# Jackie-Chou/MC-CNN-python

Measured on AMD Instinct MI355X. Metric: Mdisparities/s (HxWxD / s) end-to-end match.py timed region, images resident in HBM, higher is better.
Workload: dtype f32; 1 GPU; cfg2: 750x500 synthetic stereo pair, D=256, one pair per GPU; weights=converted reference checkpoint

## Files before the change

### include/mccnn.h

```cpp
#ifndef MCCNN_H
#define MCCNN_H

#include <stddef.h>
#include <stdint.h>

#ifdef __cplusplus
extern "C" {
#endif

typedef void *mccnn_stream_t;

#define MCCNN_ABI_VERSION 7

#define MCCNN_E_INVALID (-1)
#define MCCNN_E_UNSUPPORTED (-2)
#define MCCNN_E_SCRATCH (-3)

#define MCCNN_SIDE_LEFT 0
#define MCCNN_SIDE_RIGHT 1

int mccnn_version(void);
const char *mccnn_last_error_string(void);

#define MCCNN_CV_EXACT 0
#define MCCNN_CV_MFMA 1
int mccnn_cost_volume(const float *fl, const float *fr, int H, int W, int C, int D, float *lcv, float *rcv, int mode,
                      mccnn_stream_t stream);

int mccnn_cost_volume_hwd(const float *fl, const float *fr, int H, int W, int C, int D, float *lcv_hwd, float *rcv_hwd,
                          int mode, mccnn_stream_t stream);

size_t mccnn_decision_pack_bytes(int n_fc, int units, int mode);
int mccnn_decision_pack(const float *weights, int n_fc, int units, float weight_scale, int mode, void *packed,
                        mccnn_stream_t stream);
int mccnn_cost_volume_accurate(const float *aL, const float *aR, int H, int W, int C, int units, int n_fc, int D,
                               const void *packed, const float *biases, const float *w_final, float b_final,
                               float weight_scale, float *lcv, float *rcv, int mode, int *saturation_flag,
                               mccnn_stream_t stream);
int mccnn_cost_volume_accurate_hwd(const float *aL, const float *aR, int H, int W, int C, int units, int n_fc, int D,
                                   const void *packed, const float *biases, const float *w_final, float b_final,
                                   float weight_scale, float *lcv_hwd, float *rcv_hwd, int mode, int *saturation_flag,
                                   mccnn_stream_t stream);

int mccnn_cost_volume_fill(float *lcv, float *rcv, int D, int H, int W, int pixel_major, mccnn_stream_t stream);

typedef uint32_t mccnn_support_t;
size_t mccnn_support_bytes(int H, int W);
#define MCCNN_SUPPORT_UP(s) ((s) & 31u)
#define MCCNN_SUPPORT_DOWN(s) (((s) >> 5) & 31u)
#define MCCNN_SUPPORT_LEFT(s) (((s) >> 10) & 31u)
#define MCCNN_SUPPORT_RIGHT(s) (((s) >> 15) & 31u)
#define MCCNN_SUPPORT_COUNT(s) ((s) >> 20)
int mccnn_cross_arms(const float *image, int H, int W, float tau, int L, mccnn_support_t *support,
                     mccnn_stream_t stream);
int mccnn_cross_arms_pair(const float *image_left, const float *image_right, int H, int W, float tau, int L,
                          mccnn_support_t *support_left, mccnn_support_t *support_right, mccnn_stream_t stream);
int mccnn_cross_region_list(const mccnn_support_t *support, int H, int W, int L, int32_t *region,
                            mccnn_stream_t stream);

#define MCCNN_CBCA_SEPARABLE 0
#define MCCNN_CBCA_REFERENCE_ORDER 1
int mccnn_cbca_iter(const float *in, float *out, const mccnn_support_t *support, int D, int H, int W, int L, int order,
                    mccnn_stream_t stream);

int mccnn_cbca_iter_pair(const float *in_left, float *out_left, const mccnn_support_t *support_left,
                         const float *in_right, float *out_right, const mccnn_support_t *support_right, int D, int H,
                         int W, int L, int order, mccnn_stream_t stream);

int mccnn_cbca_iter_both(const float *in, float *out, const mccnn_support_t *support_self,
                         const mccnn_support_t *support_other, int D, int H, int W, int L, int side,
                         mccnn_stream_t stream);

int mccnn_cbca_iter_hwd(const float *in_hwd, float *out_hwd, const mccnn_support_t *support, int D, int H, int W, int L,
                        mccnn_stream_t stream);
int mccnn_cbca_iter_hwd_pair(const float *in_left, float *out_left, const mccnn_support_t *support_left,
                             const float *in_right, float *out_right, const mccnn_support_t *support_right, int D,
                             int H, int W, int L, mccnn_stream_t stream);

int mccnn_cbca_iter_hwd_pair_wta(const float *in_left, float *out_left, const mccnn_support_t *support_left,
                                 const float *in_right, float *out_right, const mccnn_support_t *support_right, int D,
                                 int H, int W, int L, float *disparity_left, float *disparity_right, int store_right,
                                 mccnn_stream_t stream);

int mccnn_cbca_iter_hwd_long(const float *in_hwd, float *out_hwd, const mccnn_support_t *support, int D, int H, int W,
                             int L, mccnn_stream_t stream);
int mccnn_cbca_iter_hwd_long_pair(const float *in_left, float *out_left, const mccnn_support_t *support_left,
                                  const float *in_right, float *out_right, const mccnn_support_t *support_right, int D,
                                  int H, int W, int L, mccnn_stream_t stream);

size_t mccnn_cbca_prog_bytes(int D, int H, int W);
int mccnn_cbca_prog_build_pair(const mccnn_support_t *support_left, const mccnn_support_t *support_right, int D, int H,
                               int W, int L, void *prog_left, void *prog_right, mccnn_stream_t stream);
int mccnn_cbca_iter_prog_pair(const float *in_left, float *out_left, const mccnn_support_t *support_left,
                              const void *prog_left, const float *in_right, float *out_right,
                              const mccnn_support_t *support_right, const void *prog_right, int D, int H, int W, int L,
                              mccnn_stream_t stream);
int mccnn_cbca_iter_prog_pair_wta(const float *in_left, float *out_left, const mccnn_support_t *support_left,
                                  const void *prog_left, const float *in_right, float *out_right,
                                  const mccnn_support_t *support_right, const void *prog_right, int D, int H, int W, int L,
                                  float *disparity_left, float *disparity_right, int store_right, mccnn_stream_t stream);

int mccnn_cbca_prog_build_skip_pair(const mccnn_support_t *support_left, const mccnn_support_t *support_right, int D,
                                    int H, int W, int L, void *prog_left, void *prog_right, mccnn_stream_t stream);
int mccnn_cbca_prog_build_both_pair(const mccnn_support_t *support_left, const mccnn_support_t *support_right, int D,
                                    int H, int W, int L, void *prog_left, void *prog_right, mccnn_stream_t stream);
int mccnn_cbca_iter_prog_pair_skip(const float *in_left, float *out_left, const mccnn_support_t *support_left,
                                   const void *prog_left, const float *in_right, float *out_right,
                                   const mccnn_support_t *support_right, const void *prog_right, int D, int H, int W,
                                   int L, mccnn_stream_t stream);

int mccnn_cbca_iter_prog(const float *in, float *out, const mccnn_support_t *support, const void *prog, int D, int H, int W,
                         int L, mccnn_stream_t stream);
int mccnn_cbca_iter_prog_skip(const float *in, float *out, const mccnn_support_t *support, const void *prog, int D, int H,
                              int W, int L, mccnn_stream_t stream);

int mccnn_cbca_iter_prog_refresh(float *in, float *out, const mccnn_support_t *support, const void *prog, int D, int H, int W,
                                 int L, mccnn_stream_t stream);
int mccnn_cbca_iter_prog_pair_refresh(float *in_left, float *out_left, const mccnn_support_t *support_left,
                                      const void *prog_left, float *in_right, float *out_right,
                                      const mccnn_support_t *support_right, const void *prog_right, int D, int H, int W,
                                      int L, mccnn_stream_t stream);

int mccnn_hwd_pitch(int D);
int mccnn_dhw_to_hwd(const float *dhw, float *hwd, int D, int H, int W, mccnn_stream_t stream);
int mccnn_hwd_to_dhw(const float *hwd, float *dhw, int D, int H, int W, mccnn_stream_t stream);

size_t mccnn_sgm_scratch_bytes(int H, int W, int D);
int mccnn_sgm_pass(const float *image_left, const float *image_right, float *const *vol_hwd, const int *side,
                   int n_jobs, int D, int H, int W, int rh, int rw, float p1, float p2, float q1, float q2, float thr,
                   void *scratch, size_t scratch_bytes, mccnn_stream_t stream);
int mccnn_sgm_flags(const float *image_left, const float *image_right, int D, int H, int W, int rh, int rw, float thr,
                    void *flags, size_t flags_bytes, mccnn_stream_t stream);
int mccnn_sgm_pass_flagged(float *const *vol_hwd, const int *side, int n_jobs, int D, int H, int W, int rh, int rw, float p1,
                           float p2, float q1, float q2, const void *flags, size_t flags_bytes, mccnn_stream_t stream);

#define MCCNN_SGM_ACC_STORE 0
#define MCCNN_SGM_ACC_ADD 1
#define MCCNN_SGM_ACC_ADD_QUARTER 2
int mccnn_sgm_pass_accumulate(const float *const *src_hwd, float *const *acc_hwd, const int *side, int n_jobs, int D, int H,
                              int W, int rh, int rw, float p1, float p2, float q1, float q2, int mode, const void *flags,
                              size_t flags_bytes, mccnn_stream_t stream);

int mccnn_sgm_first_pass(const float *image_left, const float *image_right, const float *const *vol_dhw,
                         float *const *vol_hwd, const int *side, int n_jobs, int D, int H, int W, float p1, float p2,
                         float q1, float q2, float thr, void *scratch, size_t scratch_bytes, mccnn_stream_t stream);

int mccnn_wta(const float *vol_dhw, int D, int H, int W, float *disparity, mccnn_stream_t stream);

int mccnn_wta_hwd(const float *vol_hwd, int D, int H, int W, float *disparity, mccnn_stream_t stream);

int mccnn_lr_status(const float *disp_left, const float *disp_right, int H, int W, int D, int32_t *status,
                    mccnn_stream_t stream);
int mccnn_interpolate(const float *disp_left, const int32_t *status, int H, int W, float *out,
                      mccnn_stream_t stream);
int mccnn_interpolate_ex(const float *disp_left, const int32_t *status, int H, int W, int directions,
                         int occlusion_from_left, float *out, mccnn_stream_t stream);

int mccnn_lr_status_right(const float *disp_right, const float *disp_left, int H, int W, int D, int32_t *status,
                          mccnn_stream_t stream);
int mccnn_interpolate_right(const float *disp_right, const int32_t *status, int H, int W, int directions,
                            int occlusion_from_right, float *out, mccnn_stream_t stream);

int mccnn_subpixel(const float *disp, const float *vol_dhw, int D, int H, int W, float *out, mccnn_stream_t stream);
int mccnn_subpixel_ex(const float *disp, const float *vol_dhw, int D, int H, int W, int numpy1_promotion, float *out,
                      mccnn_stream_t stream);

int mccnn_subpixel_hwd(const float *disp, const float *vol_hwd, int D, int H, int W, int numpy1_promotion, float *out,
                       mccnn_stream_t stream);

#define MCCNN_CONF_MSM 1u
#define MCCNN_CONF_MMN 2u
#define MCCNN_CONF_CUR 4u
#define MCCNN_CONF_LRC 8u
int mccnn_confidence_hwd(const float *vol_hwd , const float *disp_right , int D,
                         int H, int W, unsigned measures, float *out, mccnn_stream_t stream);
int mccnn_confidence(const float *vol_dhw , const float *disp_right , int D, int H,
                     int W, unsigned measures, float *out, mccnn_stream_t stream);

int mccnn_confidence_right_hwd(const float *vol_right_hwd , const float *disp_left ,
                               int D, int H, int W, unsigned measures, float *out, mccnn_stream_t stream);
int mccnn_confidence_right(const float *vol_right_dhw , const float *disp_left , int D,
                           int H, int W, unsigned measures, float *out, mccnn_stream_t stream);

int mccnn_median(const float *disp, int H, int W, int fh, int fw, float *out, mccnn_stream_t stream);

int mccnn_bilateral(const float *image, const float *disp, int H, int W, int fh, int fw, const float *table,
                    float thr, float *out, mccnn_stream_t stream);

size_t mccnn_ingest_scratch_bytes(int H, int W);
int mccnn_ingest_u8(const uint8_t *image_u8, int H, int W, int C, float *out, void *scratch, size_t scratch_bytes,
                    mccnn_stream_t stream);
int mccnn_ingest_u8_pair(const uint8_t *left_u8, const uint8_t *right_u8, int H, int W, int C, float *out_left,
                         float *out_right, void *scratch, size_t scratch_bytes, mccnn_stream_t stream);

typedef struct { int64_t offset; int32_t H, W; } mccnn_sample_image_t;
typedef struct { int32_t image; float cy, cx; float m[4]; float gain, bias; } mccnn_sample_t;
int mccnn_sample_patches(const float *pool, const mccnn_sample_image_t *images, int n_images,
                         const mccnn_sample_t *records, int N, int ps, float *out ,
                         mccnn_stream_t stream);

#define MCCNN_EVAL_MAX_THRESHOLDS 8
typedef struct { uint64_t n_valid, n_invalid, n_bad[MCCNN_EVAL_MAX_THRESHOLDS]; double sum_abs, sum_sq; } mccnn_eval_region_t;
typedef struct { mccnn_eval_region_t all, nonocc; } mccnn_eval_t;
size_t mccnn_evaluate_scratch_bytes(int H, int W);
int mccnn_evaluate(const float *disp, const float *gt, const uint8_t *mask , int H, int W,
                   const float *thresholds , int n_thr, int accumulate,
                   mccnn_eval_t *result , void *scratch, size_t scratch_bytes, mccnn_stream_t stream);

#define MCCNN_EVAL_MAX_QUANTILES 8
typedef struct { uint64_t n_scored; uint64_t rank[MCCNN_EVAL_MAX_QUANTILES]; float value[MCCNN_EVAL_MAX_QUANTILES]; } mccnn_quantile_region_t;
typedef struct { mccnn_quantile_region_t all, nonocc; } mccnn_eval_quantiles_t;
#define MCCNN_EVAL_POOL_BYTES (2 * 65536 * 8)
size_t mccnn_evaluate_quantiles_scratch_bytes(int H, int W);
int mccnn_evaluate_quantiles(const float *disp, const float *gt, const uint8_t *mask , int H, int W,
                             const uint32_t *q_ppm , int n_q,
                             mccnn_eval_quantiles_t *result , uint64_t *pool ,
                             void *scratch, size_t scratch_bytes, mccnn_stream_t stream);
int mccnn_evaluate_quantiles_pooled(const uint64_t *pool, const uint32_t *q_ppm , int n_q,
                                    mccnn_eval_quantiles_t *result , mccnn_stream_t stream);

int mccnn_kitti_encode_u16(const float *disp, int H, int W, uint16_t *out_u16, mccnn_stream_t stream);
int mccnn_kitti_decode_u16(const uint16_t *code_u16, int H, int W, float *out, mccnn_stream_t stream);
int mccnn_kitti_interpolate_background(const float *disp, int H, int W, float *out, mccnn_stream_t stream);
size_t mccnn_evaluate_kitti_scratch_bytes(int H, int W, int interpolate);
int mccnn_evaluate_kitti(const float *disp, const uint16_t *gt_occ_u16, const uint16_t *gt_noc_u16 ,
                         int H, int W, const float *abs_thr , const float *rel_thr , int n_thr,
                         int interpolate, int accumulate, mccnn_eval_t *result , void *scratch,
                         size_t scratch_bytes, mccnn_stream_t stream);

int mccnn_bias_act(float *x, const float *bias, int N, int C, long plane, int relu, mccnn_stream_t stream);
int mccnn_conv1_pad_bias_relu(const float *images, const float *weights, const float *bias, float *out, int N, int H,
                              int W, int pad, int C, mccnn_stream_t stream);
int mccnn_l2norm_chw_to_hwc(const float *chw, const float *bias, float *hwc, int C, int H, int W,
                            mccnn_stream_t stream);

size_t mccnn_conv3x3_split_weights_bytes(void);
int mccnn_conv3x3_split_pack(const float *weights, float weight_scale, void *packed, mccnn_stream_t stream);
int mccnn_conv1_split(const float *images, const float *weights, const float *bias, void *out, int N, int H, int W,
                      int pad, float act_scale, int *saturation_flag, mccnn_stream_t stream);
int mccnn_conv3x3_split(const void *in, const void *packed_weights, const float *bias, void *out, int N, int Hi, int Wi,
                        float weight_scale, float act_scale, int last, int *saturation_flag, mccnn_stream_t stream);

#ifdef __cplusplus
}
#endif
#endif
```

### mc-cnn-python_amd/csrc/conv_mfma.hip

```cpp
#include "common.h"

namespace mccnn {

typedef _Float16 h8 __attribute__((ext_vector_type(8)));
typedef _Float16 h4 __attribute__((ext_vector_type(4)));
typedef float f16x __attribute__((ext_vector_type(16)));
typedef uint32_t w4 __attribute__((ext_vector_type(4)));
typedef uint32_t w2 __attribute__((ext_vector_type(2)));

#ifndef CONV_STAGE_TAP
#define CONV_STAGE_TAP 0
#endif
#ifndef CONV_NBW
#define CONV_NBW 4
#endif
namespace cs {
constexpr int NBW = CONV_NBW;
constexpr int TH = 4 * NBW, TW = 32;
constexpr int IH = TH + 2, IW = TW + 2;
constexpr int NPIX = IH * IW;
constexpr int SLOT = 80;
constexpr int QBUF = NPIX * SLOT;
constexpr int NITEM = NPIX * 4;
constexpr int NST = (NITEM + 255) / 256;
constexpr int EPITCH = 272;
constexpr int EPX = NBW >= 4 ? 32 : 16;
constexpr int EPI = EPX * EPITCH;
constexpr int LDS_BYTES = 2 * QBUF + 4 * EPI;
constexpr int REC = 256;
constexpr int WFRAG = 1024;
constexpr int WLAYER = 36 * 4 * WFRAG;
}

__device__ __forceinline__ void split4(const float y[4], float scale, w2 &hi, w2 &lo)
{
    h4 a, b;
#pragma unroll
    for (int j = 0; j < 4; ++j) {
        const float v = fminf(fmaxf(y[j] * scale, -65504.f), 65504.f);
        const _Float16 h = (_Float16)v;
        a[j] = h;
        b[j] = (_Float16)(v - (float)h);
    }
    hi = __builtin_bit_cast(w2, a);
    lo = __builtin_bit_cast(w2, b);
}

__device__ __forceinline__ void split4_scaled(const float v[4], w2 &hi, w2 &lo)
{
    h4 a, b;
#pragma unroll
    for (int j = 0; j < 4; ++j) {
        const _Float16 h = (_Float16)v[j];
        a[j] = h;
        b[j] = (_Float16)(v[j] - (float)h);
    }
    hi = __builtin_bit_cast(w2, a);
    lo = __builtin_bit_cast(w2, b);
}

__global__ __launch_bounds__(256) void conv3x3_split_pack_kernel(const float *__restrict__ w, float scale,
                                                                 _Float16 *__restrict__ packed)
{
    const int i = blockIdx.x * 256 + threadIdx.x;
    if (i >= 36 * 2 * 64) return;
    const int lane = i & 63, mb = (i >> 6) & 1, ks = i >> 7;
    const int q = ks / 9, tap = ks - q * 9;
    const int oc = 32 * mb + (lane & 31), ic0 = 16 * q + 8 * (lane >> 5);
    h8 hi, lo;
#pragma unroll
    for (int j = 0; j < 8; ++j) {
        const float v = w[((size_t)oc * 64 + ic0 + j) * 9 + tap] * scale;
        const _Float16 h = (_Float16)v;
        hi[j] = h;
        lo[j] = (_Float16)(v - (float)h);
    }
    h8 *p = reinterpret_cast<h8 *>(packed);
    p[((ks * 2 + 0) * 2 + mb) * 64 + lane] = hi;
    p[((ks * 2 + 1) * 2 + mb) * 64 + lane] = lo;
}

__global__ __launch_bounds__(256) void conv1_split_kernel(const float *__restrict__ img, const float *__restrict__ w,
                                                          const float *__restrict__ bias, char *__restrict__ out, int H,
                                                          int W, int pad, int Ho, int Wo, float act_scale,
                                                          int *__restrict__ sat_flag)
{
    const int xo = blockIdx.x * 256 + threadIdx.x;
    const int yo = blockIdx.y, n = blockIdx.z;
    if (xo >= Wo) return;
    float v[9];
#pragma unroll
    for (int i = 0; i < 3; ++i)
#pragma unroll
        for (int j = 0; j < 3; ++j) {
            const int y = yo + i - pad, x = xo + j - pad;
            v[i * 3 + j] = (y >= 0 && y < H && x >= 0 && x < W) ? img[((size_t)n * H + y) * W + x] : 0.f;
        }
    char *rec = out + (((size_t)n * Ho + yo) * Wo + xo) * cs::REC;
    bool sat = false;
#pragma unroll
    for (int q = 0; q < 4; ++q) {
        w2 hi[4], lo[4];
#pragma unroll
        for (int g = 0; g < 4; ++g) {
            float y[4];
#pragma unroll
            for (int j = 0; j < 4; ++j) {
                const int c = 16 * q + 4 * g + j;
                float acc = 0.f;
#pragma unroll
                for (int k = 0; k < 9; ++k) acc += w[c * 9 + k] * v[k];
                acc += bias[c];
                y[j] = fmaxf(acc, 0.f);
                sat |= !(acc * act_scale <= 65504.f);
            }
            split4(y, act_scale, hi[g], lo[g]);
        }
        w4 *p = reinterpret_cast<w4 *>(rec + q * 64);
        p[0] = w4{hi[0].x, hi[0].y, hi[1].x, hi[1].y};
        p[1] = w4{hi[2].x, hi[2].y, hi[3].x, hi[3].y};
        p[2] = w4{lo[0].x, lo[0].y, lo[1].x, lo[1].y};
        p[3] = w4{lo[2].x, lo[2].y, lo[3].x, lo[3].y};
    }
    if (sat_flag && sat) atomicOr(sat_flag, 1);
}

__device__ __forceinline__ void pin_loads()
{
    asm volatile("" ::: "memory");
    __builtin_amdgcn_sched_barrier(0x78f);
}

template <int MODE>
__global__ __launch_bounds__(256) void conv3x3_split_kernel(const char *__restrict__ in, const char *__restrict__ wpk,
                                                            const float *__restrict__ bias, char *__restrict__ out,
                                                            int N, int Hi, int Wi, float inv_scale, float act_scale,
                                                            int tiles_x, int tiles_y, int total,
                                                            int *__restrict__ sat_flag)
{
    using namespace cs;
    extern __shared__ __attribute__((aligned(16))) char lds[];
    const int tid = threadIdx.x, lane = tid & 63;
    const int wave = __builtin_amdgcn_readfirstlane(tid >> 6);
    const int Ho = Hi - 2, Wo = Wi - 2;
    const size_t in_bytes = (size_t)N * Hi * Wi * REC, out_bytes = (size_t)N * Ho * Wo * REC;
    const __amdgpu_buffer_rsrc_t rs_in = __builtin_amdgcn_make_buffer_rsrc(
        const_cast<char *>(in), 0, (int)in_bytes, 0x00020000);
    const __amdgpu_buffer_rsrc_t rs_w =
        __builtin_amdgcn_make_buffer_rsrc(const_cast<char *>(wpk), 0, WLAYER, 0x00020000);
    const __amdgpu_buffer_rsrc_t rs_out = __builtin_amdgcn_make_buffer_rsrc(
        out, 0, (int)out_bytes, 0x00020000);

    int goff[NST], loff[NST];
#pragma unroll
    for (int r = 0; r < NST; ++r) {
        const int i = r * 256 + tid, p = min(i >> 2, NPIX - 1), part = i & 3;
        const int py = p / IW, px = p - py * IW;
        goff[r] = (py * Wi + px) * REC + part * 16;
        loff[r] = p * SLOT + part * 16;
    }
    const bool last_piece = (NST - 1) * 256 + tid < NITEM;

    auto xcd_order = [](int b, int n) {
        const int q = n >> 3, r = n & 7, x = b & 7;
        return (x < r ? x * (q + 1) : r * (q + 1) + (x - r) * q) + (b >> 3);
    };
    auto tile_base = [&](int v, int &n, int &ty0, int &tx0) {
        const int t = xcd_order(v, total);
        const int tx = t % tiles_x, r = t / tiles_x;
        const int ty = r % tiles_y;
        n = r / tiles_y;
        ty0 = ty * TH;
        tx0 = tx * TW;
    };

    w4 st[NST];
    auto fetch = [&](int n, int ty0, int tx0, int q) {
        const int so = ((n * Hi + ty0) * Wi + tx0) * REC + q * 64;
#ifdef CONV_ABL_NOSTAGE
        if (so == 0x7fffffff)
#endif
#pragma unroll
        for (int r = 0; r < NST; ++r) st[r] = __builtin_amdgcn_raw_buffer_load_b128(rs_in, goff[r], so, 0);
    };
    auto commit = [&](int buf) {
        char *b = lds + buf * QBUF;
#pragma unroll
        for (int r = 0; r < NST; ++r)
            if (r < NST - 1 || last_piece) *reinterpret_cast<w4 *>(b + loff[r]) = st[r];
    };

    int v = blockIdx.x;
    if (v >= total) return;
    int n, ty0, tx0;
    tile_base(v, n, ty0, tx0);
    fetch(n, ty0, tx0, 0);
    commit(0);
    __syncthreads();

    constexpr int NSLOT = MODE == 0 ? 3 : 4;
    w4 af[NSLOT][4];
    auto fetch_a = [&](int slot, int ks) {
#pragma unroll
        for (int f = 0; f < 4; ++f)
            af[slot][f] = __builtin_amdgcn_raw_buffer_load_b128(rs_w, lane * 16, (ks * 4 + f) * WFRAG, 0);
    };
#pragma unroll
    for (int i = 0; i < NSLOT - 1; ++i) fetch_a(i, i);

    const int bfrag = (wave * NBW * IW + (lane & 31)) * SLOT + 16 * (lane >> 5);
    char *const epi = lds + 2 * QBUF + wave * EPI;

    while (true) {
        f16x acc[NBW][2], accx[NBW][2];
#pragma unroll
        for (int nb = 0; nb < NBW; ++nb)
#pragma unroll
            for (int mb = 0; mb < 2; ++mb)
#pragma unroll
                for (int i = 0; i < 16; ++i) acc[nb][mb][i] = accx[nb][mb][i] = 0.f;
        const int vn = v + gridDim.x;
        int nn = 0, nty0 = 0, ntx0 = 0;
        if (vn < total) tile_base(vn, nn, nty0, ntx0);
        if (vn >= total) {
            nn = n;
            nty0 = ty0;
            ntx0 = tx0;
        }
#pragma unroll
        for (int q = 0; q < 4; ++q) {
            auto stage_next = [&]() {
                if (q < 3)
                    fetch(n, ty0, tx0, q + 1);
                else
                    fetch(nn, nty0, ntx0, 0);
                pin_loads();
            };
            if (CONV_STAGE_TAP < 0) stage_next();
            const char *bq = lds + (q & 1) * QBUF + bfrag;
            char *const other = lds + ((q + 1) & 1) * QBUF;
            w4 bf[2][2];
            auto read_b = [&](int slot, int step) {
                const int tap = step / NBW, nb = step % NBW;
                const int dy = tap / 3, dx = tap - dy * 3;
                const char *pb = bq + ((nb + dy) * IW + dx) * SLOT;
                bf[slot][0] = *reinterpret_cast<const w4 *>(pb);
                bf[slot][1] = *reinterpret_cast<const w4 *>(pb + 32);
            };
            read_b(0, 0);
#pragma unroll
            for (int tap = 0; tap < 9; ++tap) {
                const int ks = q * 9 + tap;
                fetch_a((ks + NSLOT - 1) % NSLOT, (ks + NSLOT - 1) % 36);
                pin_loads();
                if (tap == CONV_STAGE_TAP) stage_next();
                const int slot = ks % NSLOT;
                const h8 a_hi0 = __builtin_bit_cast(h8, af[slot][0]), a_hi1 = __builtin_bit_cast(h8, af[slot][1]);
                const h8 a_lo0 = __builtin_bit_cast(h8, af[slot][2]), a_lo1 = __builtin_bit_cast(h8, af[slot][3]);
#pragma unroll
                for (int nb = 0; nb < NBW; ++nb) {
                    const int step = tap * NBW + nb;
                    if (step + 1 < 9 * NBW) read_b((step + 1) & 1, step + 1);
                    __builtin_amdgcn_sched_barrier(0);
                    const h8 b_hi = __builtin_bit_cast(h8, bf[step & 1][0]);
                    const h8 b_lo = __builtin_bit_cast(h8, bf[step & 1][1]);
                    accx[nb][0] = __builtin_amdgcn_mfma_f32_32x32x16_f16(a_lo0, b_hi, accx[nb][0], 0, 0, 0);
                    accx[nb][1] = __builtin_amdgcn_mfma_f32_32x32x16_f16(a_lo1, b_hi, accx[nb][1], 0, 0, 0);
                    accx[nb][0] = __builtin_amdgcn_mfma_f32_32x32x16_f16(a_hi0, b_lo, accx[nb][0], 0, 0, 0);
                    accx[nb][1] = __builtin_amdgcn_mfma_f32_32x32x16_f16(a_hi1, b_lo, accx[nb][1], 0, 0, 0);
                    acc[nb][0] = __builtin_amdgcn_mfma_f32_32x32x16_f16(a_hi0, b_hi, acc[nb][0], 0, 0, 0);
                    acc[nb][1] = __builtin_amdgcn_mfma_f32_32x32x16_f16(a_hi1, b_hi, acc[nb][1], 0, 0, 0);
                }
                if (tap >= 9 - (NST + 1) / 2) {
#pragma unroll
                    for (int j = 0; j < 2; ++j) {
                        const int r = 2 * (tap - (9 - (NST + 1) / 2)) + j;
                        if (r < NST && (r < NST - 1 || last_piece)) *reinterpret_cast<w4 *>(other + loff[r]) = st[r];
                    }
                }
            }
            __syncthreads();
        }

        const int px = lane & 31, half = lane >> 5;
        bool sat = false;
#ifdef CONV_ABL_NOEPI
        {
            float t = 0.f;
#pragma unroll
            for (int nb = 0; nb < NBW; ++nb)
#pragma unroll
                for (int mb = 0; mb < 2; ++mb)
#pragma unroll
                    for (int r = 0; r < 16; ++r) t += acc[nb][mb][r] + accx[nb][mb][r];
            if (t == 123.456f) __builtin_amdgcn_raw_buffer_store_b32(__float_as_uint(t), rs_out, lane * 4, 0, 0);
        }
#else
#pragma unroll
        for (int nb = 0; nb < NBW; ++nb) {
            float y[2][16];
            float ss = 0.f;
#pragma unroll
            for (int mb = 0; mb < 2; ++mb)
#pragma unroll
                for (int r = 0; r < 16; ++r) {
                    const int ch = 32 * mb + (r & 3) + 8 * (r >> 2) + 4 * half;
                    if (MODE == 0) {
                    } else {
                        const float t = fmaf(acc[nb][mb][r] + accx[nb][mb][r], inv_scale, bias[ch]);
                        y[mb][r] = t;
                        ss = fmaf(t, t, ss);
                    }
                }
            float nrm = 1.f;
            if (MODE == 1) {
                ss += __shfl_xor(ss, 32);
                nrm = 1.f / sqrtf(fmaxf(ss, 1e-12f));
            }
            const int row = ty0 + wave * NBW + nb;
            const int so = ((n * Ho + min(row, Ho - 1)) * Wo + tx0) * REC;
            const bool stored = row < Ho && tx0 + px < Wo;
            bool over = false;
#pragma unroll
            for (int hf = 0; hf < 32 / EPX; ++hf) {
                __builtin_amdgcn_wave_barrier();
                if (EPX == 32 || (px >> 4) == hf) {
                    const int pl = px & (EPX - 1);
#pragma unroll
                    for (int mb = 0; mb < 2; ++mb)
#pragma unroll
                        for (int g = 0; g < 4; ++g) {
                            const int ch = 32 * mb + 8 * g + 4 * half;
                            if (MODE == 0) {
                                w2 hi, lo;
                                float y4[4];
#pragma unroll
                                for (int q = 0; q < 4; ++q) {
                                    const int r = 4 * g + q;
                                    const float t = fmaf(acc[nb][mb][r] + accx[nb][mb][r], inv_scale * act_scale,
                                                         bias[ch + q] * act_scale);
                                    over |= !(t <= 65504.f);
                                    y4[q] = __builtin_amdgcn_fmed3f(t, 0.f, 65504.f);
                                }
                                split4_scaled(y4, hi, lo);
                                char *p = epi + pl * EPITCH + (ch >> 4) * 64 + (ch & 15) * 2;
                                *reinterpret_cast<w2 *>(p) = hi;
                                *reinterpret_cast<w2 *>(p + 32) = lo;
                            } else {
                                w4 o;
                                o.x = __float_as_uint(y[mb][4 * g + 0] * nrm);
                                o.y = __float_as_uint(y[mb][4 * g + 1] * nrm);
                                o.z = __float_as_uint(y[mb][4 * g + 2] * nrm);
                                o.w = __float_as_uint(y[mb][4 * g + 3] * nrm);
                                *reinterpret_cast<w4 *>(epi + pl * EPITCH + ch * 4) = o;
                            }
                        }
                }
                __builtin_amdgcn_wave_barrier();
#pragma unroll
                for (int it = 0; it < EPX / 4; ++it) {
                    const int i = it * 64 + lane, pl = i >> 4, part = i & 15, p = hf * EPX + pl;
                    const w4 o = *reinterpret_cast<const w4 *>(epi + pl * EPITCH + part * 16);
                    const bool ok = row < Ho && tx0 + p < Wo;
                    buffer_store_b128<0>(o, rs_out, ok ? p * REC + part * 16 : 0x7ffffff0, so);
                }
            }
            __builtin_amdgcn_wave_barrier();
            sat |= over && stored;
        }
        if (MODE == 0 && sat_flag && __builtin_amdgcn_ballot_w64(sat) != 0 && lane == 0)
            atomicOr(sat_flag, 1);
#endif
        if (vn >= total) break;
        v = vn;
        n = nn;
        ty0 = nty0;
        tx0 = ntx0;
    }
}

}

extern "C" size_t mccnn_conv3x3_split_weights_bytes(void) { return (size_t)mccnn::cs::WLAYER; }

extern "C" int mccnn_conv3x3_split_pack(const float *weights, float weight_scale, void *packed, mccnn_stream_t stream)
{
    using namespace mccnn;
    MCCNN_REQUIRE(weights && packed, MCCNN_E_INVALID, "mccnn_conv3x3_split_pack: null pointer");
    MCCNN_REQUIRE(weight_scale > 0.f, MCCNN_E_INVALID, "mccnn_conv3x3_split_pack: scale must be positive");
    hipLaunchKernelGGL(conv3x3_split_pack_kernel, dim3(cdiv(36 * 2 * 64, 256)), dim3(256), 0, (hipStream_t)stream,
                       weights, weight_scale, reinterpret_cast<_Float16 *>(packed));
    return check_launch("mccnn_conv3x3_split_pack");
}

extern "C" int mccnn_conv1_split(const float *images, const float *weights, const float *bias, void *out, int N, int H,
                                 int W, int pad, float act_scale, int *saturation_flag, mccnn_stream_t stream)
{
    using namespace mccnn;
    MCCNN_REQUIRE(images && weights && bias && out, MCCNN_E_INVALID, "mccnn_conv1_split: null pointer");
    MCCNN_REQUIRE(N > 0 && H > 0 && W > 0 && pad >= 0, MCCNN_E_INVALID, "mccnn_conv1_split: bad size");
    MCCNN_REQUIRE(act_scale > 0.f, MCCNN_E_INVALID, "mccnn_conv1_split: scale must be positive");
    const int Ho = H + 2 * pad - 2, Wo = W + 2 * pad - 2;
    MCCNN_REQUIRE(Ho > 0 && Wo > 0 && Ho <= 65535 && N <= 65535, MCCNN_E_UNSUPPORTED,
                  "mccnn_conv1_split: output %dx%d outside the grid", Wo, Ho);
    hipLaunchKernelGGL(conv1_split_kernel, dim3(cdiv(Wo, 256), Ho, N), dim3(256), 0, (hipStream_t)stream, images,
                       weights, bias, reinterpret_cast<char *>(out), H, W, pad, Ho, Wo, act_scale, saturation_flag);
    return check_launch("mccnn_conv1_split");
}

extern "C" int mccnn_conv3x3_split(const void *in, const void *packed_weights, const float *bias, void *out, int N,
                                   int Hi, int Wi, float weight_scale, float act_scale, int last,
                                   int *saturation_flag, mccnn_stream_t stream)
{
    using namespace mccnn;
    using namespace cs;
    MCCNN_REQUIRE(in && packed_weights && bias && out, MCCNN_E_INVALID, "mccnn_conv3x3_split: null pointer");
    MCCNN_REQUIRE(N > 0 && Hi > 2 && Wi > 2, MCCNN_E_INVALID, "mccnn_conv3x3_split: input %dx%d too small", Wi, Hi);
    MCCNN_REQUIRE(weight_scale > 0.f && act_scale > 0.f, MCCNN_E_INVALID, "mccnn_conv3x3_split: scales must be positive");
    MCCNN_REQUIRE((size_t)N * Hi * Wi * REC <= 0x7ffffff0u, MCCNN_E_UNSUPPORTED,
                  "mccnn_conv3x3_split: %d x %dx%d records exceed 32-bit buffer offsets", N, Wi, Hi);
    const int Ho = Hi - 2, Wo = Wi - 2;
    const int tiles_x = cdiv(Wo, TW), tiles_y = cdiv(Ho, TH);
    const long total = (long)tiles_x * tiles_y * N;
    MCCNN_REQUIRE(total <= 0x7fffffffL, MCCNN_E_UNSUPPORTED, "mccnn_conv3x3_split: too many tiles");
    const int cus = device_cus8();
    const long slots = (long)cus * (LDS_BYTES <= 80 * 1024 ? 2 : 1);
    const int grid = (int)(total < slots ? total : slots);
    const float inv = 1.f / (weight_scale * act_scale);
    hipStream_t s = (hipStream_t)stream;
    if (last) {
        static const hipError_t attr = hipFuncSetAttribute(reinterpret_cast<const void *>(conv3x3_split_kernel<1>),
                                                           hipFuncAttributeMaxDynamicSharedMemorySize, LDS_BYTES);
        MCCNN_REQUIRE(attr == hipSuccess, MCCNN_E_UNSUPPORTED, "mccnn_conv3x3_split: %d bytes of LDS refused", LDS_BYTES);
        hipLaunchKernelGGL(conv3x3_split_kernel<1>, dim3(grid), dim3(256), LDS_BYTES, s,
                           reinterpret_cast<const char *>(in), reinterpret_cast<const char *>(packed_weights), bias,
                           reinterpret_cast<char *>(out), N, Hi, Wi, inv, act_scale, tiles_x, tiles_y, (int)total,
                           saturation_flag);
    } else {
        static const hipError_t attr = hipFuncSetAttribute(reinterpret_cast<const void *>(conv3x3_split_kernel<0>),
                                                           hipFuncAttributeMaxDynamicSharedMemorySize, LDS_BYTES);
        MCCNN_REQUIRE(attr == hipSuccess, MCCNN_E_UNSUPPORTED, "mccnn_conv3x3_split: %d bytes of LDS refused", LDS_BYTES);
        hipLaunchKernelGGL(conv3x3_split_kernel<0>, dim3(grid), dim3(256), LDS_BYTES, s,
                           reinterpret_cast<const char *>(in), reinterpret_cast<const char *>(packed_weights), bias,
                           reinterpret_cast<char *>(out), N, Hi, Wi, inv, act_scale, tiles_x, tiles_y, (int)total,
                           saturation_flag);
    }
    return check_launch("mccnn_conv3x3_split");
}
```

### mc-cnn-python_amd/src/_hipabi.py

```python
import ctypes
import os

import torch

_HERE = os.path.dirname(os.path.abspath(__file__))
LIB_PATH = os.environ.get("MCCNN_HIP_LIB") or os.path.join(os.path.dirname(_HERE), "lib", "libmccnn_hip.so")

MCCNN_ABI_VERSION = 7
MCCNN_CV_EXACT = 0
MCCNN_CV_MFMA = 1
MCCNN_CBCA_SEPARABLE = 0
MCCNN_CBCA_REFERENCE_ORDER = 1
MCCNN_SIDE_LEFT = 0
MCCNN_SIDE_RIGHT = 1
MCCNN_SGM_ACC_STORE = 0
MCCNN_SGM_ACC_ADD = 1
MCCNN_SGM_ACC_ADD_QUARTER = 2
MCCNN_E_INVALID = -1
MCCNN_E_UNSUPPORTED = -2
MCCNN_E_SCRATCH = -3

MCCNN_EVAL_MAX_THRESHOLDS = 8
MCCNN_EVAL_MAX_QUANTILES = 8
MCCNN_EVAL_POOL_BYTES = 2 * 65536 * 8
MCCNN_CONF_MSM = 1
MCCNN_CONF_MMN = 2
MCCNN_CONF_CUR = 4
MCCNN_CONF_LRC = 8

_vp = ctypes.c_void_p
_i = ctypes.c_int
_f = ctypes.c_float
_sz = ctypes.c_size_t

SIGNATURES = {
    "mccnn_version": (_i, []),
    "mccnn_last_error_string": (ctypes.c_char_p, []),
    "mccnn_cost_volume": (_i, [_vp, _vp, _i, _i, _i, _i, _vp, _vp, _i, _vp]),
    "mccnn_cost_volume_hwd": (_i, [_vp, _vp, _i, _i, _i, _i, _vp, _vp, _i, _vp]),
    "mccnn_cost_volume_fill": (_i, [_vp, _vp, _i, _i, _i, _i, _vp]),
    "mccnn_decision_pack_bytes": (_sz, [_i, _i, _i]),
    "mccnn_decision_pack": (_i, [_vp, _i, _i, _f, _i, _vp, _vp]),
    "mccnn_cost_volume_accurate": (_i, [_vp, _vp, _i, _i, _i, _i, _i, _i, _vp, _vp, _vp, _f, _f, _vp, _vp, _i, _vp, _vp]),
    "mccnn_cost_volume_accurate_hwd": (_i, [_vp, _vp, _i, _i, _i, _i, _i, _i, _vp, _vp, _vp, _f, _f, _vp, _vp, _i, _vp,
                                            _vp]),
    "mccnn_support_bytes": (_sz, [_i, _i]),
    "mccnn_cross_arms": (_i, [_vp, _i, _i, _f, _i, _vp, _vp]),
    "mccnn_cross_arms_pair": (_i, [_vp, _vp, _i, _i, _f, _i, _vp, _vp, _vp]),
    "mccnn_cross_region_list": (_i, [_vp, _i, _i, _i, _vp, _vp]),
    "mccnn_cbca_iter": (_i, [_vp, _vp, _vp, _i, _i, _i, _i, _i, _vp]),
    "mccnn_cbca_iter_pair": (_i, [_vp, _vp, _vp, _vp, _vp, _vp, _i, _i, _i, _i, _i, _vp]),
    "mccnn_cbca_iter_both": (_i, [_vp, _vp, _vp, _vp, _i, _i, _i, _i, _i, _vp]),
    "mccnn_cbca_iter_hwd": (_i, [_vp, _vp, _vp, _i, _i, _i, _i, _vp]),
    "mccnn_cbca_iter_hwd_pair": (_i, [_vp, _vp, _vp, _vp, _vp, _vp, _i, _i, _i, _i, _vp]),
    "mccnn_cbca_iter_hwd_pair_wta": (_i, [_vp, _vp, _vp, _vp, _vp, _vp, _i, _i, _i, _i, _vp, _vp, _i, _vp]),
    "mccnn_cbca_iter_hwd_long": (_i, [_vp, _vp, _vp, _i, _i, _i, _i, _vp]),
    "mccnn_cbca_iter_hwd_long_pair": (_i, [_vp, _vp, _vp, _vp, _vp, _vp, _i, _i, _i, _i, _vp]),
    "mccnn_cbca_prog_bytes": (_sz, [_i, _i, _i]),
    "mccnn_cbca_prog_build_pair": (_i, [_vp, _vp, _i, _i, _i, _i, _vp, _vp, _vp]),
    "mccnn_cbca_iter_prog_pair": (_i, [_vp, _vp, _vp, _vp, _vp, _vp, _vp, _vp, _i, _i, _i, _i, _vp]),
    "mccnn_cbca_prog_build_skip_pair": (_i, [_vp, _vp, _i, _i, _i, _i, _vp, _vp, _vp]),
    "mccnn_cbca_prog_build_both_pair": (_i, [_vp, _vp, _i, _i, _i, _i, _vp, _vp, _vp]),
    "mccnn_cbca_iter_prog_pair_skip": (_i, [_vp, _vp, _vp, _vp, _vp, _vp, _vp, _vp, _i, _i, _i, _i, _vp]),
    "mccnn_cbca_iter_prog": (_i, [_vp, _vp, _vp, _vp, _i, _i, _i, _i, _vp]),
    "mccnn_cbca_iter_prog_skip": (_i, [_vp, _vp, _vp, _vp, _i, _i, _i, _i, _vp]),
    "mccnn_cbca_iter_prog_refresh": (_i, [_vp, _vp, _vp, _vp, _i, _i, _i, _i, _vp]),
    "mccnn_cbca_iter_prog_pair_refresh": (_i, [_vp, _vp, _vp, _vp, _vp, _vp, _vp, _vp, _i, _i, _i, _i, _vp]),
    "mccnn_cbca_iter_prog_pair_wta": (_i, [_vp, _vp, _vp, _vp, _vp, _vp, _vp, _vp, _i, _i, _i, _i, _vp, _vp, _i, _vp]),
    "mccnn_wta_hwd": (_i, [_vp, _i, _i, _i, _vp, _vp]),
    "mccnn_subpixel_hwd": (_i, [_vp, _vp, _i, _i, _i, _i, _vp, _vp]),
    "mccnn_confidence_hwd": (_i, [_vp, _vp, _i, _i, _i, ctypes.c_uint, _vp, _vp]),
    "mccnn_confidence": (_i, [_vp, _vp, _i, _i, _i, ctypes.c_uint, _vp, _vp]),
    "mccnn_confidence_right_hwd": (_i, [_vp, _vp, _i, _i, _i, ctypes.c_uint, _vp, _vp]),
    "mccnn_confidence_right": (_i, [_vp, _vp, _i, _i, _i, ctypes.c_uint, _vp, _vp]),
    "mccnn_hwd_pitch": (_i, [_i]),
    "mccnn_dhw_to_hwd": (_i, [_vp, _vp, _i, _i, _i, _vp]),
    "mccnn_hwd_to_dhw": (_i, [_vp, _vp, _i, _i, _i, _vp]),
    "mccnn_sgm_scratch_bytes": (_sz, [_i, _i, _i]),
    "mccnn_sgm_pass": (_i, [_vp, _vp, ctypes.POINTER(_vp), ctypes.POINTER(_i), _i, _i, _i, _i, _i, _i,
                            _f, _f, _f, _f, _f, _vp, _sz, _vp]),
    "mccnn_sgm_flags": (_i, [_vp, _vp, _i, _i, _i, _i, _i, _f, _vp, _sz, _vp]),
    "mccnn_sgm_pass_flagged": (_i, [ctypes.POINTER(_vp), ctypes.POINTER(_i), _i, _i, _i, _i, _i, _i, _f, _f, _f, _f, _vp, _sz,
                                    _vp]),
    "mccnn_sgm_pass_accumulate": (_i, [ctypes.POINTER(_vp), ctypes.POINTER(_vp), ctypes.POINTER(_i), _i, _i, _i, _i, _i, _i,
                                       _f, _f, _f, _f, _i, _vp, _sz, _vp]),
    "mccnn_sgm_first_pass": (_i, [_vp, _vp, ctypes.POINTER(_vp), ctypes.POINTER(_vp), ctypes.POINTER(_i), _i, _i, _i,
                                  _i, _f, _f, _f, _f, _f, _vp, _sz, _vp]),
    "mccnn_wta": (_i, [_vp, _i, _i, _i, _vp, _vp]),
    "mccnn_lr_status": (_i, [_vp, _vp, _i, _i, _i, _vp, _vp]),
    "mccnn_interpolate": (_i, [_vp, _vp, _i, _i, _vp, _vp]),
    "mccnn_interpolate_ex": (_i, [_vp, _vp, _i, _i, _i, _i, _vp, _vp]),
    "mccnn_lr_status_right": (_i, [_vp, _vp, _i, _i, _i, _vp, _vp]),
    "mccnn_interpolate_right": (_i, [_vp, _vp, _i, _i, _i, _i, _vp, _vp]),
    "mccnn_subpixel": (_i, [_vp, _vp, _i, _i, _i, _vp, _vp]),
    "mccnn_subpixel_ex": (_i, [_vp, _vp, _i, _i, _i, _i, _vp, _vp]),
    "mccnn_median": (_i, [_vp, _i, _i, _i, _i, _vp, _vp]),
    "mccnn_bilateral": (_i, [_vp, _vp, _i, _i, _i, _i, _vp, _f, _vp, _vp]),
    "mccnn_bias_act": (_i, [_vp, _vp, _i, _i, ctypes.c_long, _i, _vp]),
    "mccnn_conv1_pad_bias_relu": (_i, [_vp, _vp, _vp, _vp, _i, _i, _i, _i, _i, _vp]),
    "mccnn_conv3x3_split_weights_bytes": (_sz, []),
    "mccnn_conv3x3_split_pack": (_i, [_vp, _f, _vp, _vp]),
    "mccnn_conv1_split": (_i, [_vp, _vp, _vp, _vp, _i, _i, _i, _i, _f, _vp, _vp]),
    "mccnn_conv3x3_split": (_i, [_vp, _vp, _vp, _vp, _i, _i, _i, _f, _f, _i, _vp, _vp]),
    "mccnn_l2norm_chw_to_hwc": (_i, [_vp, _vp, _vp, _i, _i, _i, _vp]),
    "mccnn_ingest_scratch_bytes": (_sz, [_i, _i]),
    "mccnn_ingest_u8": (_i, [_vp, _i, _i, _i, _vp, _vp, _sz, _vp]),
    "mccnn_ingest_u8_pair": (_i, [_vp, _vp, _i, _i, _i, _vp, _vp, _vp, _sz, _vp]),
    "mccnn_sample_patches": (_i, [_vp, _vp, _i, _vp, _i, _i, _vp, _vp]),
    "mccnn_evaluate_scratch_bytes": (_sz, [_i, _i]),
    "mccnn_evaluate": (_i, [_vp, _vp, _vp, _i, _i, ctypes.POINTER(_f), _i, _i, _vp, _vp, _sz, _vp]),
    "mccnn_evaluate_quantiles_scratch_bytes": (_sz, [_i, _i]),
    "mccnn_evaluate_quantiles": (_i, [_vp, _vp, _vp, _i, _i, ctypes.POINTER(ctypes.c_uint32), _i, _vp, _vp, _vp, _sz, _vp]),
    "mccnn_evaluate_quantiles_pooled": (_i, [_vp, ctypes.POINTER(ctypes.c_uint32), _i, _vp, _vp]),
    "mccnn_kitti_encode_u16": (_i, [_vp, _i, _i, _vp, _vp]),
    "mccnn_kitti_decode_u16": (_i, [_vp, _i, _i, _vp, _vp]),
    "mccnn_kitti_interpolate_background": (_i, [_vp, _i, _i, _vp, _vp]),
    "mccnn_evaluate_kitti_scratch_bytes": (_sz, [_i, _i, _i]),
    "mccnn_evaluate_kitti": (_i, [_vp, _vp, _vp, _i, _i, ctypes.POINTER(_f), ctypes.POINTER(_f), _i, _i, _i, _vp, _vp, _sz,
                                  _vp]),
}



class EvalRegion(ctypes.Structure):
    _fields_ = [("n_valid", ctypes.c_uint64), ("n_invalid", ctypes.c_uint64),
                ("n_bad", ctypes.c_uint64 * MCCNN_EVAL_MAX_THRESHOLDS), ("sum_abs", ctypes.c_double),
                ("sum_sq", ctypes.c_double)]


class EvalResult(ctypes.Structure):
    _fields_ = [("all", EvalRegion), ("nonocc", EvalRegion)]


class QuantileRegion(ctypes.Structure):
    _fields_ = [("n_scored", ctypes.c_uint64), ("rank", ctypes.c_uint64 * MCCNN_EVAL_MAX_QUANTILES),
                ("value", ctypes.c_uint32 * MCCNN_EVAL_MAX_QUANTILES)]


class QuantileResult(ctypes.Structure):
    _fields_ = [("all", QuantileRegion), ("nonocc", QuantileRegion)]


_lib = None


class MccnnHipError(RuntimeError):
    pass


def load():
    global _lib
    if _lib is not None:
        return _lib
    if not os.path.isfile(LIB_PATH):
        raise MccnnHipError(
            "libmccnn_hip.so not found at %s - build it with `make -C mc-cnn-python_amd` "
            "(or `python -c 'import __graft_entry__ as g; g.build()'`). There is no CPU fallback." % LIB_PATH)
    lib = ctypes.CDLL(LIB_PATH)
    for name, (res, args) in SIGNATURES.items():
        fn = getattr(lib, name)
        fn.restype = res
        fn.argtypes = args
    have = lib.mccnn_version()
    if have != MCCNN_ABI_VERSION:
        raise MccnnHipError("%s implements ABI version %d, this binding expects %d: rebuild the library "
                            "(`make -C mc-cnn-python_amd`)" % (LIB_PATH, have, MCCNN_ABI_VERSION))
    _lib = lib
    return lib


def check(rc, what):
    if rc != 0:
        msg = load().mccnn_last_error_string()
        raise MccnnHipError("%s failed (code %d): %s" % (what, rc, msg.decode() if msg else "?"))


def stream():
    return ctypes.c_void_p(torch.cuda.current_stream().cuda_stream)


def ptr(t):
    if not t.is_cuda:
        raise MccnnHipError("expected a device tensor; the HIP path never runs on host memory")
    if not t.is_contiguous():
        raise MccnnHipError("expected a contiguous tensor")
    return ctypes.c_void_p(t.data_ptr())


def require_device():
    if not torch.cuda.is_available():
        raise MccnnHipError("no HIP device visible: the MI355X path cannot run (and there is no CPU fallback)")
    load()
    return torch.device("cuda", torch.cuda.current_device())
```

### mc-cnn-python_amd/src/model.py

```python
import math
import os

os.environ.setdefault("MIOPEN_DEBUG_CONV_DIRECT_NAIVE_CONV_FWD", "0")

import numpy as np
import torch
import torch.nn.functional as F

import tf_checkpoint


SPLIT_RECORD_LIMIT = 0x7ffffff0 // 256


def split_feature_route(H, W, pad):
    padded = (H + 2 * pad - 2) * (W + 2 * pad - 2)
    if padded > SPLIT_RECORD_LIMIT:
        return "library", max(64, (SPLIT_RECORD_LIMIT // (W + 2 * pad)) // 2)
    return ("pair" if 2 * padded <= SPLIT_RECORD_LIMIT else "views"), None


class NET(object):

    def __init__(self, x=None, weights_path='DEFAULT',
                 input_patch_size=11, num_conv_layers=5, num_conv_feature_maps=64,
                 conv_kernel_size=3, batch_size=128, device=None, seed=0):
        self.X = x
        self.batch_size = batch_size
        self.input_patch_size = input_patch_size
        self.num_conv_layers = num_conv_layers
        self.num_conv_feature_maps = num_conv_feature_maps
        self.conv_kernel_size = conv_kernel_size
        self.WEIGHTS_PATH = 'pretrain.npy' if weights_path == 'DEFAULT' else weights_path
        if device is None:
            if torch.is_tensor(x):
                device = x.device
            else:
                device = torch.device("cuda") if torch.cuda.is_available() else torch.device("cpu")
        self.device = torch.device(device)
        self._init_variables(seed)
        if x is not None:
            self.create()

    def _init_variables(self, seed):
        g = torch.Generator().manual_seed(seed)
        k, nf = self.conv_kernel_size, self.num_conv_feature_maps
        self.weights = []
        self.biases = []
        cin = 1
        for _ in range(self.num_conv_layers):
            limit = math.sqrt(6.0 / (k * k * cin + k * k * nf))
            w = (torch.rand((nf, cin, k, k), generator=g) * 2 - 1) * limit
            blim = math.sqrt(6.0 / (nf + nf))
            b = (torch.rand((nf,), generator=g) * 2 - 1) * blim
            self.weights.append(w.to(self.device))
            self.biases.append(b.to(self.device))
            cin = nf

    def set_layers(self, layers):
        assert len(layers) == self.num_conv_layers, "checkpoint has %d conv layers, NET was built with %d" % (
            len(layers), self.num_conv_layers)
        self.weights = [torch.from_numpy(np.ascontiguousarray(np.transpose(w, (3, 2, 0, 1)))).to(self.device)
                        for w, _ in layers]
        self.biases = [torch.from_numpy(np.ascontiguousarray(b)).to(self.device) for _, b in layers]
        return self

    def get_layers(self):
        return [(np.ascontiguousarray(w.detach().permute(2, 3, 1, 0).cpu().numpy()), b.detach().cpu().numpy())
                for w, b in zip(self.weights, self.biases)]

    def restore(self, checkpoint):
        return self.set_layers(tf_checkpoint.load_fast_net_weights(checkpoint))

    def load_initial_weights(self, session=None):
        weights_dict = np.load(self.WEIGHTS_PATH, encoding='bytes', allow_pickle=True).item()
        layers = self.get_layers()
        for name, value in weights_dict.items():
            name = name.decode() if isinstance(name, bytes) else name
            scope, var = name.split(":")[0].split("/")
            idx = int(scope.replace("conv", "")) - 1
            w, b = layers[idx]
            layers[idx] = (np.asarray(value, np.float32), b) if var == "weights" else (w, np.asarray(value, np.float32))
        self.set_layers(layers)

    def save_weights(self, session=None, file_name='pretrain.npy'):
        weights_dict = {}
        for k, (w, b) in enumerate(self.get_layers(), start=1):
            weights_dict["conv%d/weights:0" % k] = w
            weights_dict["conv%d/biases:0" % k] = b
        np.save(file_name, weights_dict)

    def _convs_nchw(self, x):
        outs = []
        nl = self.num_conv_layers
        for k in range(nl):
            x = F.conv2d(x, self.weights[k], self.biases[k])
            if k < nl - 1:
                x = F.relu(x)
            outs.append(x)
        return outs

    def _convs_device(self, images, pad):
        import stereo_device
        nl = self.num_conv_layers
        if self.conv_kernel_size == 3 and nl >= 2:
            x = stereo_device.conv1_pad_bias_relu(images.contiguous(), self.weights[0], self.biases[0], pad)
            first = 1
        else:
            x = F.pad(images[:, None], (pad, pad, pad, pad))
            first = 0
        for k in range(first, nl):
            x = F.conv2d(x, self.weights[k], None)
            if k < nl - 1:
                x = stereo_device.bias_act_(x.contiguous(), self.biases[k], True)
        return x.contiguous()

    @staticmethod
    def _l2_normalize_last(x):
        s = torch.clamp((x * x).sum(dim=-1, keepdim=True), min=1e-12)
        return x * torch.rsqrt(s)

    def create(self):
        self(self.X)

    def __call__(self, x):
        x = torch.as_tensor(x, dtype=torch.float32).to(self.device)
        assert x.dim() == 4 and x.shape[-1] == 1, "NET expects NHWC input with one channel (model.py:36-40)"
        self.X = x
        outs = self._convs_nchw(x.permute(0, 3, 1, 2).contiguous())
        for k, o in enumerate(outs, start=1):
            setattr(self, "conv%d" % k, o.permute(0, 2, 3, 1))
        self.features = self._l2_normalize_last(outs[-1].permute(0, 2, 3, 1))
        return self.features

    def features_hwc(self, image_hw):
        import stereo_device
        pad = (self.input_patch_size - 1) // 2
        assert pad == self.num_conv_layers * (self.conv_kernel_size - 1) // 2, \
            "patch size must equal the receptive field so that features keep the image size"
        out = self._convs_device(image_hw[None], pad)[0]
        return stereo_device.l2norm_chw_to_hwc(out, self.biases[-1])

    def supports_split_features(self):
        return self.conv_kernel_size == 3 and self.num_conv_feature_maps == 64 and self.num_conv_layers >= 2

    def _split_weights(self):
        import stereo_device
        key = tuple((w.data_ptr(), w._version) for w in self.weights[1:])
        cache = getattr(self, "_split_cache", None)
        if cache is None or cache[0] != key:
            cache = (key, [stereo_device.conv3x3_split_pack(w) for w in self.weights[1:]])
            self._split_cache = cache
        return cache[1]

    def _split_flag(self):
        f = getattr(self, "_split_sat", None)
        if f is None or f.device != self.weights[0].device:
            f = torch.zeros((1,), dtype=torch.int32, device=self.weights[0].device)
            self._split_sat = f
        return f

    def split_saturated(self, reset=True):
        f = getattr(self, "_split_sat", None)
        if f is None:
            return False
        hit = bool(int(f.item()))
        if hit and reset:
            f.zero_()
        return hit

    def features_pair_hwc_split(self, left_hw, right_hw):
        import warnings
        import stereo_device
        pad = (self.input_patch_size - 1) // 2
        assert pad == self.num_conv_layers * (self.conv_kernel_size - 1) // 2
        if not self.supports_split_features():
            raise ValueError("the split-operand feature kernels are built for >= 2 layers of 64 maps, 3x3")
        packed = self._split_weights()
        flag = self._split_flag()
        H, W = left_hw.shape
        route, rows = split_feature_route(H, W, pad)
        if route == "library":
            warnings.warn("split-operand features: a %dx%d view exceeds the kernels' 32-bit record offsets; using the "
                          "float32 library convolutions in bands of %d rows instead" % (W, H, rows))
            return self.features_pair_hwc(left_hw, right_hw, tile_rows=rows)
        batches = [torch.stack((left_hw, right_hw)).contiguous()] if route == "pair" else \
            [left_hw[None].contiguous(), right_hw[None].contiguous()]
        outs = []
        nl = self.num_conv_layers
        for views in batches:
            x = stereo_device.conv1_split(views, self.weights[0].detach().contiguous(), self.biases[0].detach(), pad,
                                          sat_flag=flag)
            for k in range(1, nl):
                pk, ws = packed[k - 1]
                x = stereo_device.conv3x3_split(x, pk, ws, self.biases[k].detach(), last=(k == nl - 1), sat_flag=flag)
            outs += [x[i] for i in range(x.shape[0])]
        return outs[0], outs[1]

    def features_pair_hwc(self, left_hw, right_hw, tile_rows=None):
        import stereo_device
        pad = (self.input_patch_size - 1) // 2
        assert pad == self.num_conv_layers * (self.conv_kernel_size - 1) // 2
        pair = torch.stack((left_hw, right_hw))
        if tile_rows is None or tile_rows >= pair.shape[1]:
            out = self._convs_device(pair, pad)
            return (stereo_device.l2norm_chw_to_hwc(out[0], self.biases[-1]),
                    stereo_device.l2norm_chw_to_hwc(out[1], self.biases[-1]))
        H, W = pair.shape[1], pair.shape[2]
        x = F.pad(pair[:, None], (pad, pad, pad, pad))
        feats = [torch.empty((H, W, self.num_conv_feature_maps), dtype=torch.float32, device=pair.device)
                 for _ in range(2)]
        for y0 in range(0, H, int(tile_rows)):
            y1 = min(y0 + int(tile_rows), H)
            t = x[:, :, y0:y1 + 2 * pad, :]
            for k in range(self.num_conv_layers):
                t = F.conv2d(t, self.weights[k], None)
                if k < self.num_conv_layers - 1:
                    t = stereo_device.bias_act_(t.contiguous(), self.biases[k], True)
            t = t.contiguous()
            for v in range(2):
                stereo_device.l2norm_chw_to_hwc(t[v], self.biases[-1], out=feats[v][y0:y1])
        return feats[0], feats[1]


class ACCURATE_NET(NET):

    def __init__(self, x=None, weights_path='DEFAULT',
                 input_patch_size=11, num_conv_layers=5, num_conv_feature_maps=112,
                 conv_kernel_size=3, batch_size=128, device=None, seed=0, num_fc_layers=3, num_fc_units=384):
        self.num_fc_layers = int(num_fc_layers)
        self.num_fc_units = int(num_fc_units)
        assert self.num_fc_layers >= 1 and self.num_fc_units >= 1
        NET.__init__(self, x, weights_path, input_patch_size, num_conv_layers, num_conv_feature_maps, conv_kernel_size,
                     batch_size, device, seed)

    def _init_variables(self, seed):
        NET._init_variables(self, seed)
        g = torch.Generator().manual_seed(seed + 1)
        self.fc_weights = []
        self.fc_biases = []
        fan_in = 2 * self.num_conv_feature_maps
        for k in range(self.num_fc_layers + 1):
            fan_out = self.num_fc_units if k < self.num_fc_layers else 1
            limit = math.sqrt(6.0 / (fan_in + fan_out))
            w = (torch.rand((fan_out, fan_in), generator=g) * 2 - 1) * limit
            b = (torch.rand((fan_out,), generator=g) * 2 - 1) * limit
            self.fc_weights.append(w.to(self.device))
            self.fc_biases.append(b.to(self.device))
            fan_in = fan_out

    def set_layers(self, layers, fc_layers=None):
        NET.set_layers(self, layers)
        if fc_layers is not None:
            assert len(fc_layers) == self.num_fc_layers + 1, "checkpoint has %d fc layers, ACCURATE_NET was built with %d" % (
                len(fc_layers), self.num_fc_layers + 1)
            self.fc_weights = [torch.from_numpy(np.ascontiguousarray(np.asarray(w, np.float32).T)).to(self.device)
                               for w, _ in fc_layers]
            self.fc_biases = [torch.from_numpy(np.ascontiguousarray(b, dtype=np.float32)).to(self.device)
                              for _, b in fc_layers]
            fan_in = 2 * self.num_conv_feature_maps
            for k, w in enumerate(self.fc_weights):
                fan_out = self.num_fc_units if k < self.num_fc_layers else 1
                assert tuple(w.shape) == (fan_out, fan_in), "fc%d/weights is %s, expected [%d,%d]" % (
                    k + 1, tuple(w.shape)[::-1], fan_in, fan_out)
                fan_in = fan_out
        return self

    def get_fc_layers(self):
        return [(np.ascontiguousarray(w.detach().cpu().numpy().T), b.detach().cpu().numpy())
                for w, b in zip(self.fc_weights, self.fc_biases)]

    def restore(self, checkpoint):
        layers, fc = tf_checkpoint.load_accurate_net_weights(checkpoint)
        return self.set_layers(layers, fc)

    def save(self, path):
        tf_checkpoint.save_npz(path, self.get_layers(), self.get_fc_layers())

    def _convs_nchw(self, x):
        outs = []
        for k in range(self.num_conv_layers):
            x = F.relu(F.conv2d(x, self.weights[k], self.biases[k]))
            outs.append(x)
        return outs

    def __call__(self, x):
        x = torch.as_tensor(x, dtype=torch.float32).to(self.device)
        assert x.dim() == 4 and x.shape[-1] == 1, "ACCURATE_NET expects NHWC input with one channel"
        self.X = x
        outs = self._convs_nchw(x.permute(0, 3, 1, 2).contiguous())
        for k, o in enumerate(outs, start=1):
            setattr(self, "conv%d" % k, o.permute(0, 2, 3, 1))
        self.features = outs[-1].permute(0, 2, 3, 1)
        return self.features

    def decision_logits(self, fl, fr):
        x = torch.cat((fl, fr), dim=-1)
        for k in range(self.num_fc_layers):
            x = F.relu(F.linear(x, self.fc_weights[k], self.fc_biases[k]))
        return F.linear(x, self.fc_weights[-1], self.fc_biases[-1])[..., 0]

    def decision(self, fl, fr):
        return torch.sigmoid(self.decision_logits(fl, fr))

    def patch_logits(self, left, right):
        left = torch.as_tensor(left, dtype=torch.float32).to(self.device)
        right = torch.as_tensor(right, dtype=torch.float32).to(self.device)
        B = left.shape[0]
        f = self(torch.cat((left, right), dim=0)).reshape(2 * B, -1)
        return self.decision_logits(f[:B], f[B:])

    def scores(self, left, right):
        return torch.sigmoid(self.patch_logits(left, right))

    def first_layer_halves(self, fl, fr, out=None):
        H, W, C = fl.shape
        w1, b1 = self.fc_weights[0].detach(), self.fc_biases[0].detach()
        u = w1.shape[0]
        if out is None:
            out = (torch.empty((H, W, u), dtype=torch.float32, device=fl.device),
                   torch.empty((H, W, u), dtype=torch.float32, device=fl.device))
        torch.addmm(b1, fl.reshape(H * W, C), w1[:, :C].t(), out=out[0].view(H * W, u))
        torch.mm(fr.reshape(H * W, C), w1[:, C:].t(), out=out[1].view(H * W, u))
        return out

    def supports_split_features(self):
        return False

    def _tower_hwc(self, images):
        import stereo_device
        pad = (self.input_patch_size - 1) // 2
        assert pad == self.num_conv_layers * (self.conv_kernel_size - 1) // 2, \
            "patch size must equal the receptive field so that features keep the image size"
        x = self._convs_device(images, pad)
        x = stereo_device.bias_act_(x, self.biases[-1].detach(), True)
        return x.permute(0, 2, 3, 1).contiguous()

    def features_hwc(self, image_hw):
        return self._tower_hwc(image_hw[None].contiguous())[0]

    def features_pair_hwc(self, left_hw, right_hw, tile_rows=None):
        if tile_rows is not None:
            raise ValueError("row banding is implemented for the fast network only")
        f = self._tower_hwc(torch.stack((left_hw, right_hw)))
        return f[0], f[1]

    def features_pair_hwc_split(self, left_hw, right_hw):
        raise ValueError("the split-operand feature kernels are built for the fast network (64 maps, normalised)")

    def decision_weights_key(self):
        return tuple((w.data_ptr(), w._version) for w in self.fc_weights + self.fc_biases)

    def decision_layers(self):
        import stereo_device
        ws = [w.detach().float() for w in self.fc_weights[1:-1]]
        bs = [b.detach().float() for b in self.fc_biases[1:-1]]
        maxima = torch.stack([w.abs().max() for w in ws]).tolist()
        try:
            exps = stereo_device.decision_equalise_exponents(maxima)
        except ValueError as e:
            raise stereo_device.hip.MccnnHipError("ACCURATE_NET.decision_layers: %s" % e)
        prev = 0
        for k, c in enumerate(exps):
            if c != prev:
                ws[k] = ws[k] * 2.0 ** (c - prev)
            if c != 0:
                bs[k] = bs[k] * 2.0 ** c
            prev = c
        w_final = self.fc_weights[-1].detach().float().reshape(-1)
        if prev != 0:
            w_final = w_final * 2.0 ** (-prev)
        return (torch.stack(ws).contiguous(), torch.stack(bs).contiguous(), w_final.contiguous(),
                self.fc_biases[-1].detach().float().reshape(-1), exps)

    def decision_operands(self, mode):
        import stereo_device
        key = (int(mode),) + self.decision_weights_key()
        cache = getattr(self, "_decision_cache", None)
        if cache is None or cache[0] != key:
            mid, biases, w_final, b_final, _exps = self.decision_layers()
            packed, scale = stereo_device.decision_pack(mid, self.num_fc_layers, mode)
            cache = (key, (packed, scale, biases, w_final, float(b_final[0])))
            self._decision_cache = cache
        return cache[1]

    def _split_flag(self):
        f = getattr(self, "_split_sat", None)
        if f is None or f.device != self.fc_weights[0].device:
            f = torch.zeros((1,), dtype=torch.int32, device=self.fc_weights[0].device)
            self._split_sat = f
        return f


if __name__ == "__main__":
    net = NET(torch.zeros([128, 11, 11, 1]))
    print(net.features.shape)
```

### mc-cnn-python_amd/src/stereo_device.py

```python
import collections
import ctypes
import math

import numpy as np
import torch

import _hipabi as hip


def _f32(x):
    return float(np.float32(x))


class StageTimer(object):

    def __init__(self, enabled=False):
        self.enabled = enabled
        self.records = []
        self.spans = []
        self._open = None

    def start(self, name):
        if not self.enabled:
            return
        ev = torch.cuda.Event(enable_timing=True)
        ev.record()
        self._open = (name, ev)

    def stop(self):
        if not self.enabled or self._open is None:
            return
        ev = torch.cuda.Event(enable_timing=True)
        ev.record()
        self.records.append((self._open[0], self._open[1], ev))
        self._open = None

    def span_start(self, name):
        if self.enabled:
            ev = torch.cuda.Event(enable_timing=True)
            ev.record()
            self.spans.append([name, ev, None])

    def span_stop(self, name):
        if self.enabled:
            ev = torch.cuda.Event(enable_timing=True)
            ev.record()
            for s in reversed(self.spans):
                if s[0] == name and s[2] is None:
                    s[2] = ev
                    break

    def spans_ms(self):
        out = {}
        for name, a, b in self.spans:
            if b is not None:
                out.setdefault(name, []).append(a.elapsed_time(b))
        return out

    def summary_ms(self):
        out = {}
        for name, a, b in self.records:
            out.setdefault(name, []).append(a.elapsed_time(b))
        return out


_NO_TIMER = StageTimer(False)


def bias_act_(x, bias, relu):
    N, C, H, W = x.shape
    assert x.is_contiguous() and bias.numel() == C
    hip.check(hip.load().mccnn_bias_act(hip.ptr(x), hip.ptr(bias), N, C, H * W, 1 if relu else 0, hip.stream()),
              "mccnn_bias_act")
    return x


def conv1_pad_bias_relu(images, weight, bias, pad):
    N, H, W = images.shape
    C = weight.shape[0]
    assert tuple(weight.shape) == (C, 1, 3, 3) and images.is_contiguous() and weight.is_contiguous()
    out = torch.empty((N, C, H + 2 * pad - 2, W + 2 * pad - 2), dtype=torch.float32, device=images.device)
    hip.check(hip.load().mccnn_conv1_pad_bias_relu(hip.ptr(images), hip.ptr(weight), hip.ptr(bias), hip.ptr(out), N, H,
                                                   W, int(pad), C, hip.stream()), "mccnn_conv1_pad_bias_relu")
    return out


def l2norm_chw_to_hwc(chw, bias=None, out=None):
    C, H, W = chw.shape
    if out is None:
        out = torch.empty((H, W, C), dtype=torch.float32, device=chw.device)
    assert tuple(out.shape) == (H, W, C) and out.is_contiguous()
    hip.check(hip.load().mccnn_l2norm_chw_to_hwc(hip.ptr(chw), hip.ptr(bias) if bias is not None else None,
                                                 hip.ptr(out), C, H, W, hip.stream()), "mccnn_l2norm_chw_to_hwc")
    return out


SPLIT_ACT_SCALE = 256.0


def conv3x3_split_pack(weight):
    assert tuple(weight.shape) == (64, 64, 3, 3), "the split-operand kernel is built for 64 -> 64 maps, 3x3"
    w = weight.detach().contiguous().float()
    m = float(w.abs().max())
    scale = 2.0 ** math.floor(math.log2(1024.0 / m)) if m > 0.0 and math.isfinite(m) else 1.0
    lib = hip.load()
    packed = torch.empty((lib.mccnn_conv3x3_split_weights_bytes(),), dtype=torch.uint8, device=w.device)
    hip.check(lib.mccnn_conv3x3_split_pack(hip.ptr(w), scale, hip.ptr(packed), hip.stream()), "mccnn_conv3x3_split_pack")
    return packed, scale


def conv1_split(images, weight, bias, pad, act_scale=SPLIT_ACT_SCALE, sat_flag=None):
    N, H, W = images.shape
    assert tuple(weight.shape) == (64, 1, 3, 3) and images.is_contiguous() and weight.is_contiguous()
    out = torch.empty((N, H + 2 * pad - 2, W + 2 * pad - 2, 256), dtype=torch.uint8, device=images.device)
    hip.check(hip.load().mccnn_conv1_split(hip.ptr(images), hip.ptr(weight), hip.ptr(bias), hip.ptr(out), N, H, W,
                                           int(pad), float(act_scale), hip.ptr(sat_flag) if sat_flag is not None else None,
                                           hip.stream()), "mccnn_conv1_split")
    return out


def conv3x3_split(x, packed, weight_scale, bias, last, act_scale=SPLIT_ACT_SCALE, sat_flag=None):
    N, Hi, Wi, rec = x.shape
    assert rec == 256 and x.dtype == torch.uint8 and x.is_contiguous()
    if last:
        out = torch.empty((N, Hi - 2, Wi - 2, 64), dtype=torch.float32, device=x.device)
    else:
        out = torch.empty((N, Hi - 2, Wi - 2, 256), dtype=torch.uint8, device=x.device)
    hip.check(hip.load().mccnn_conv3x3_split(hip.ptr(x), hip.ptr(packed), hip.ptr(bias), hip.ptr(out), N, Hi, Wi,
                                             float(weight_scale), float(act_scale), 1 if last else 0,
                                             hip.ptr(sat_flag) if sat_flag is not None else None, hip.stream()),
              "mccnn_conv3x3_split")
    return out


def cost_volume(fl, fr, ndisp, mode=hip.MCCNN_CV_EXACT, out=None):
    H, W, C = fl.shape
    if out is None:
        lcv = torch.empty((ndisp, H, W), dtype=torch.float32, device=fl.device)
        rcv = torch.empty((ndisp, H, W), dtype=torch.float32, device=fl.device)
    else:
        lcv, rcv = out
    hip.check(hip.load().mccnn_cost_volume(hip.ptr(fl), hip.ptr(fr), H, W, C, int(ndisp), hip.ptr(lcv), hip.ptr(rcv),
                                           int(mode), hip.stream()), "mccnn_cost_volume")
    return lcv, rcv


def cost_volume_hwd(fl, fr, ndisp, out=None, mode=hip.MCCNN_CV_EXACT):
    H, W, C = fl.shape
    dp = hwd_pitch(ndisp)
    if out is None:
        lcv = torch.zeros((H, W, dp), dtype=torch.float32, device=fl.device)
        rcv = torch.zeros((H, W, dp), dtype=torch.float32, device=fl.device)
    else:
        lcv, rcv = out
    hip.check(hip.load().mccnn_cost_volume_hwd(hip.ptr(fl), hip.ptr(fr), H, W, C, int(ndisp), hip.ptr(lcv), hip.ptr(rcv),
                                               int(mode), hip.stream()), "mccnn_cost_volume_hwd")
    return lcv, rcv


DECISION_UNITS = 384
DECISION_MAPS = (64, 112)
DECISION_FC_LAYERS = (3, 4)
DECISION_MAX_D = 1024
DECISION_LIBRARY_BYTES = 256 << 20


def decision_kernel_refusal(net, W, D):
    if net.num_conv_feature_maps not in DECISION_MAPS:
        return "%d feature maps (the decision kernel serves %s)" % (net.num_conv_feature_maps, " or ".join(
            str(c) for c in DECISION_MAPS))
    if net.num_fc_units != DECISION_UNITS:
        return "%d units per hidden layer (the decision kernel is built for %d)" % (net.num_fc_units, DECISION_UNITS)
    if net.num_fc_layers not in DECISION_FC_LAYERS:
        return "%d fully-connected layers (the decision kernel serves 3 or 4)" % net.num_fc_layers
    if D < 2 or D > DECISION_MAX_D:
        return "ndisp=%d outside [2, %d]" % (D, DECISION_MAX_D)
    if D > W - 2:
        return "ndisp=%d needs an image at least ndisp + 2 pixels wide (W=%d)" % (D, W)
    return None


DECISION_SCALE_MAX_EXP = 118
DECISION_SCALE_MIN_EXP = -126
DECISION_EQUALISE_MAX_EXP = 64


def decision_weight_scale(m):
    m = float(m)
    if not (math.isfinite(m) and m >= 0.0):
        raise ValueError("decision_weight_scale: max |w| = %r, the decision kernel packs finite weights only" % m)
    if m == 0.0:
        return 1.0
    f, x = math.frexp(m)
    e = 10 - x + (1 if f == 0.5 else 0)
    return 2.0 ** max(DECISION_SCALE_MIN_EXP, min(DECISION_SCALE_MAX_EXP, e))


def decision_equalise_exponents(maxima):
    for k, m in enumerate(maxima):
        if not (math.isfinite(float(m)) and float(m) >= 0.0):
            raise ValueError("fc%d: max |w| = %r, the decision kernel packs finite weights only" % (k + 2, float(m)))
    exps = [math.frexp(float(m))[1] if float(m) > 0.0 else None for m in maxima]
    live = [e for e in exps if e is not None]
    if not live:
        return [0] * len(exps)
    target = int(math.floor(sum(live) / float(len(live)) + 0.5))
    out, c = [], 0
    for e in exps:
        if e is not None:
            c = max(-DECISION_EQUALISE_MAX_EXP, min(DECISION_EQUALISE_MAX_EXP, c + target - e))
        out.append(c)
    return out


def decision_pack(weights, n_fc, mode):
    lib = hip.load()
    w = weights.detach().contiguous().float()
    units = int(w.shape[-1])
    nbytes = int(lib.mccnn_decision_pack_bytes(int(n_fc), units, int(mode)))
    if nbytes == 0 or tuple(w.shape) != (n_fc - 1, units, units):
        raise hip.MccnnHipError("mccnn_decision_pack: %d fc layers of %d units are outside the decision kernel's "
                                "envelope (3 or 4 layers of %d units)" % (n_fc, units, DECISION_UNITS))
    try:
        scale = decision_weight_scale(float(w.abs().max()))
    except ValueError as e:
        raise hip.MccnnHipError("mccnn_decision_pack: %s" % e)
    packed = torch.empty((nbytes,), dtype=torch.uint8, device=w.device)
    hip.check(lib.mccnn_decision_pack(hip.ptr(w), int(n_fc), units, scale, int(mode), hip.ptr(packed), hip.stream()),
              "mccnn_decision_pack")
    return packed, scale


def cost_volume_fill(lcv, rcv, ndisp, pixel_major):
    H, W = (lcv.shape[0], lcv.shape[1]) if pixel_major else (lcv.shape[1], lcv.shape[2])
    hip.check(hip.load().mccnn_cost_volume_fill(hip.ptr(lcv), hip.ptr(rcv), int(ndisp), H, W, 1 if pixel_major else 0,
                                                hip.stream()), "mccnn_cost_volume_fill")
    return lcv, rcv


def accurate_scores_library(net, aL, aR, ndisp, lcv, rcv, pixel_major, budget=DECISION_LIBRARY_BYTES):
    H, W, U = aL.shape
    ws = [w.detach() for w in net.fc_weights]
    bs = [b.detach() for b in net.fc_biases]
    lv = lcv.permute(2, 0, 1) if pixel_major else lcv
    rv = rcv.permute(2, 0, 1) if pixel_major else rcv
    for d in range(int(ndisp)):
        n = W - d
        rows = max(1, min(H, int(budget) // (n * U * 4)))
        for h0 in range(0, H, rows):
            h1 = min(H, h0 + rows)
            x = torch.relu(aL[h0:h1, d:, :] + aR[h0:h1, :n, :]).reshape(-1, U)
            for k in range(1, net.num_fc_layers):
                x = torch.relu(torch.addmm(bs[k], x, ws[k].t()))
            z = torch.addmv(bs[-1].expand(x.shape[0]), x, ws[-1].reshape(-1))
            s = torch.sigmoid(z).neg_().reshape(h1 - h0, n)
            lv[d, h0:h1, d:] = s
            rv[d, h0:h1, :n] = s
    return lcv, rcv


def cost_volume_accurate(net, fl, fr, ndisp, mode=hip.MCCNN_CV_EXACT, decision="kernel", pixel_major=True, out=None,
                         halves=None, sat_flag=None, budget=DECISION_LIBRARY_BYTES):
    if decision not in ("kernel", "library"):
        raise ValueError("decision must be 'kernel' or 'library'")
    H, W, C = fl.shape
    D = int(ndisp)
    if out is None:
        shape = (H, W, hwd_pitch(D)) if pixel_major else (D, H, W)
        out = (torch.zeros(shape, dtype=torch.float32, device=fl.device),
               torch.zeros(shape, dtype=torch.float32, device=fl.device))
    lcv, rcv = out
    why = decision_kernel_refusal(net, W, D) if decision == "kernel" else None
    if why is not None:
        raise hip.MccnnHipError("cost_volume_accurate: %s" % why)
    aL, aR = net.first_layer_halves(fl, fr, out=halves)
    if decision == "library":
        accurate_scores_library(net, aL, aR, D, lcv, rcv, pixel_major, budget)
        return cost_volume_fill(lcv, rcv, D, pixel_major)
    lib = hip.load()
    packed, scale, biases, w_final, b_final = net.decision_operands(mode)
    fn = lib.mccnn_cost_volume_accurate_hwd if pixel_major else lib.mccnn_cost_volume_accurate
    hip.check(fn(hip.ptr(aL), hip.ptr(aR), H, W, C, net.num_fc_units, net.num_fc_layers, D, hip.ptr(packed),
                 hip.ptr(biases), hip.ptr(w_final), b_final, scale, hip.ptr(lcv), hip.ptr(rcv), int(mode),
                 hip.ptr(sat_flag) if sat_flag is not None else None, hip.stream()),
              "mccnn_cost_volume_accurate_hwd" if pixel_major else "mccnn_cost_volume_accurate")
    return lcv, rcv


def ingest_scratch(H, W, device):
    nbytes = int(hip.load().mccnn_ingest_scratch_bytes(H, W))
    return torch.empty(((nbytes + 3) // 4,), dtype=torch.float32, device=device)


def _u8_image(image_u8):
    if image_u8.dtype != torch.uint8 or image_u8.dim() not in (2, 3):
        raise ValueError("ingest: expected a uint8 image [H,W] or [H,W,C], got %s %s" % (image_u8.dtype, tuple(image_u8.shape)))
    return image_u8.shape[0], image_u8.shape[1], (image_u8.shape[2] if image_u8.dim() == 3 else 1)


def ingest_u8(image_u8, out=None, scratch=None):
    H, W, C = _u8_image(image_u8)
    out = out if out is not None else torch.empty((H, W), dtype=torch.float32, device=image_u8.device)
    scratch = scratch if scratch is not None else ingest_scratch(H, W, image_u8.device)
    hip.check(hip.load().mccnn_ingest_u8(hip.ptr(image_u8), H, W, C, hip.ptr(out), hip.ptr(scratch),
                                         scratch.numel() * 4, hip.stream()), "mccnn_ingest_u8")
    return out


def ingest_u8_pair(left_u8, right_u8, out_l=None, out_r=None, scratch=None):
    H, W, C = _u8_image(left_u8)
    if _u8_image(right_u8) != (H, W, C):
        raise ValueError("ingest_u8_pair: the two images must have the same shape")
    out_l = out_l if out_l is not None else torch.empty((H, W), dtype=torch.float32, device=left_u8.device)
    out_r = out_r if out_r is not None else torch.empty((H, W), dtype=torch.float32, device=left_u8.device)
    scratch = scratch if scratch is not None else ingest_scratch(H, W, left_u8.device)
    hip.check(hip.load().mccnn_ingest_u8_pair(hip.ptr(left_u8), hip.ptr(right_u8), H, W, C, hip.ptr(out_l), hip.ptr(out_r),
                                              hip.ptr(scratch), scratch.numel() * 4, hip.stream()),
              "mccnn_ingest_u8_pair")
    return out_l, out_r


EVAL_BYTES = 192
EVAL_THRESHOLDS = (0.5, 1.0, 2.0, 4.0)


def evaluate_scratch(H, W, device):
    nbytes = int(hip.load().mccnn_evaluate_scratch_bytes(H, W))
    return torch.empty(((nbytes + 7) // 8,), dtype=torch.float64, device=device)


def evaluate_result(device):
    return torch.zeros((EVAL_BYTES // 8,), dtype=torch.int64, device=device)


def evaluate(disp, gt, mask=None, thresholds=EVAL_THRESHOLDS, out=None, accumulate=False, scratch=None):
    if disp.dim() != 2 or disp.dtype != torch.float32 or gt.dtype != torch.float32:
        raise ValueError("evaluate: expected float32 maps [H,W], got %s %s and %s %s"
                         % (disp.dtype, tuple(disp.shape), gt.dtype, tuple(gt.shape)))
    if tuple(gt.shape) != tuple(disp.shape):
        raise ValueError("evaluate: the map is %s, the ground truth %s" % (tuple(disp.shape), tuple(gt.shape)))
    if mask is not None and (mask.dtype != torch.uint8 or tuple(mask.shape) != tuple(disp.shape)):
        raise ValueError("evaluate: expected a uint8 mask %s, got %s %s" % (tuple(disp.shape), mask.dtype, tuple(mask.shape)))
    for t in (gt, mask, out, scratch):
        if t is not None and t.device != disp.device:
            raise ValueError("evaluate: every tensor must live on the map's device")
    thr = [float(t) for t in thresholds]
    if not 1 <= len(thr) <= hip.MCCNN_EVAL_MAX_THRESHOLDS:
        raise ValueError("evaluate: %d thresholds, expected 1..%d" % (len(thr), hip.MCCNN_EVAL_MAX_THRESHOLDS))
    H, W = disp.shape
    if out is None:
        if accumulate:
            raise ValueError("evaluate: accumulate needs the `out` to accumulate into")
        out = torch.empty((EVAL_BYTES // 8,), dtype=torch.int64, device=disp.device)
    elif out.numel() * out.element_size() != EVAL_BYTES:
        raise ValueError("evaluate: `out` must hold %d bytes" % EVAL_BYTES)
    scratch = scratch if scratch is not None else evaluate_scratch(H, W, disp.device)
    hip.check(hip.load().mccnn_evaluate(hip.ptr(disp), hip.ptr(gt), hip.ptr(mask) if mask is not None else None, H, W,
                                        (ctypes.c_float * len(thr))(*thr), len(thr), 1 if accumulate else 0, hip.ptr(out),
                                        hip.ptr(scratch), scratch.numel() * scratch.element_size(), hip.stream()),
              "mccnn_evaluate")
    return out


EVAL_QUANTILES_BYTES = 208
EVAL_QUANTILES_PPM = (500000, 900000, 950000, 990000)


def evaluate_quantiles_scratch(H, W, device):
    nbytes = int(hip.load().mccnn_evaluate_quantiles_scratch_bytes(H, W))
    return torch.empty(((nbytes + 7) // 8,), dtype=torch.int64, device=device)


def evaluate_quantiles_result(device):
    return torch.zeros((EVAL_QUANTILES_BYTES // 8,), dtype=torch.int64, device=device)


def evaluate_quantiles_pool(device):
    return torch.zeros((2, 65536), dtype=torch.int64, device=device)


def _quantiles_ppm(quantiles_ppm, who):
    ppm = [int(q) for q in quantiles_ppm]
    if not 1 <= len(ppm) <= hip.MCCNN_EVAL_MAX_QUANTILES:
        raise ValueError("%s: %d quantiles, expected 1..%d" % (who, len(ppm), hip.MCCNN_EVAL_MAX_QUANTILES))
    if any(not 1 <= q <= 1000000 for q in ppm):
        raise ValueError("%s: quantiles are parts per million, 1..1000000, got %r" % (who, ppm))
    return (ctypes.c_uint32 * len(ppm))(*ppm), len(ppm)


def _quantiles_pool(pool, device, who):
    if pool.dtype != torch.int64 or pool.numel() * 8 != hip.MCCNN_EVAL_POOL_BYTES or pool.device != device:
        raise ValueError("%s: `pool` must be an evaluate_quantiles_pool() on the map's device" % who)


def evaluate_quantiles(disp, gt, mask=None, quantiles_ppm=EVAL_QUANTILES_PPM, out=None, pool=None, scratch=None):
    if disp.dim() != 2 or disp.dtype != torch.float32 or gt.dtype != torch.float32:
        raise ValueError("evaluate_quantiles: expected float32 maps [H,W], got %s %s and %s %s"
                         % (disp.dtype, tuple(disp.shape), gt.dtype, tuple(gt.shape)))
    if tuple(gt.shape) != tuple(disp.shape):
        raise ValueError("evaluate_quantiles: the map is %s, the ground truth %s" % (tuple(disp.shape), tuple(gt.shape)))
    if mask is not None and (mask.dtype != torch.uint8 or tuple(mask.shape) != tuple(disp.shape)):
        raise ValueError("evaluate_quantiles: expected a uint8 mask %s, got %s %s"
                         % (tuple(disp.shape), mask.dtype, tuple(mask.shape)))
    pool_only = out is False
    for t in (gt, mask, None if pool_only else out, pool, scratch):
        if t is not None and t.device != disp.device:
            raise ValueError("evaluate_quantiles: every tensor must live on the map's device")
    q, n_q = _quantiles_ppm(quantiles_ppm, "evaluate_quantiles")
    H, W = disp.shape
    if pool_only:
        if pool is None:
            raise ValueError("evaluate_quantiles: out=False needs the `pool` to add to")
        out = None
    elif out is None:
        out = torch.empty((EVAL_QUANTILES_BYTES // 8,), dtype=torch.int64, device=disp.device)
    elif out.numel() * out.element_size() != EVAL_QUANTILES_BYTES:
        raise ValueError("evaluate_quantiles: `out` must hold %d bytes" % EVAL_QUANTILES_BYTES)
    if pool is not None:
        _quantiles_pool(pool, disp.device, "evaluate_quantiles")
    scratch = scratch if scratch is not None else evaluate_quantiles_scratch(H, W, disp.device)
    hip.check(hip.load().mccnn_evaluate_quantiles(hip.ptr(disp), hip.ptr(gt), hip.ptr(mask) if mask is not None else None,
                                                  H, W, q, n_q, hip.ptr(out) if out is not None else None,
                                                  hip.ptr(pool) if pool is not None else None, hip.ptr(scratch),
                                                  scratch.numel() * scratch.element_size(), hip.stream()),
              "mccnn_evaluate_quantiles")
    return out


def evaluate_quantiles_pooled(pool, quantiles_ppm=EVAL_QUANTILES_PPM, out=None):
    _quantiles_pool(pool, pool.device, "evaluate_quantiles_pooled")
    q, n_q = _quantiles_ppm(quantiles_ppm, "evaluate_quantiles_pooled")
    if out is None:
        out = torch.empty((EVAL_QUANTILES_BYTES // 8,), dtype=torch.int64, device=pool.device)
    elif out.numel() * out.element_size() != EVAL_QUANTILES_BYTES or out.device != pool.device:
        raise ValueError("evaluate_quantiles_pooled: `out` must hold %d bytes on the pool's device" % EVAL_QUANTILES_BYTES)
    hip.check(hip.load().mccnn_evaluate_quantiles_pooled(hip.ptr(pool), q, n_q, hip.ptr(out), hip.stream()),
              "mccnn_evaluate_quantiles_pooled")
    return out


def _kitti_map(disp, who):
    if disp.dim() != 2 or disp.dtype != torch.float32:
        raise ValueError("%s: expected a float32 map [H,W], got %s %s" % (who, disp.dtype, tuple(disp.shape)))
    return int(disp.shape[0]), int(disp.shape[1])


def kitti_encode_u16(disp, out=None):
    H, W = _kitti_map(disp, "kitti_encode_u16")
    if out is None:
        out = torch.empty((H, W), dtype=torch.uint16, device=disp.device)
    elif out.dtype != torch.uint16 or tuple(out.shape) != (H, W) or out.device != disp.device:
        raise ValueError("kitti_encode_u16: `out` must be a uint16 %s on the map's device" % ((H, W),))
    hip.check(hip.load().mccnn_kitti_encode_u16(hip.ptr(disp), H, W, hip.ptr(out), hip.stream()), "mccnn_kitti_encode_u16")
    return out


def kitti_decode_u16(code, out=None):
    if code.dim() != 2 or code.dtype != torch.uint16:
        raise ValueError("kitti_decode_u16: expected a uint16 plane [H,W], got %s %s" % (code.dtype, tuple(code.shape)))
    H, W = int(code.shape[0]), int(code.shape[1])
    if out is None:
        out = torch.empty((H, W), dtype=torch.float32, device=code.device)
    elif out.dtype != torch.float32 or tuple(out.shape) != (H, W) or out.device != code.device:
        raise ValueError("kitti_decode_u16: `out` must be a float32 %s on the plane's device" % ((H, W),))
    hip.check(hip.load().mccnn_kitti_decode_u16(hip.ptr(code), H, W, hip.ptr(out), hip.stream()), "mccnn_kitti_decode_u16")
    return out


def kitti_interpolate_background(disp, out=None):
    H, W = _kitti_map(disp, "kitti_interpolate_background")
    if out is None:
        out = torch.empty_like(disp)
    elif out.dtype != torch.float32 or tuple(out.shape) != (H, W) or out.device != disp.device:
        raise ValueError("kitti_interpolate_background: `out` must be a float32 %s on the map's device" % ((H, W),))
    hip.check(hip.load().mccnn_kitti_interpolate_background(hip.ptr(disp), H, W, hip.ptr(out), hip.stream()),
              "mccnn_kitti_interpolate_background")
    return out


def evaluate_kitti_scratch(H, W, device, interpolate=False):
    nbytes = int(hip.load().mccnn_evaluate_kitti_scratch_bytes(H, W, 1 if interpolate else 0))
    return torch.empty(((nbytes + 7) // 8,), dtype=torch.float64, device=device)


KITTI_D1 = ((3.0, 0.05),)


def evaluate_kitti(disp, gt_occ, gt_noc=None, thresholds=KITTI_D1, interpolate=False, out=None, accumulate=False,
                   scratch=None):
    H, W = _kitti_map(disp, "evaluate_kitti")
    for name, t in (("gt_occ", gt_occ), ("gt_noc", gt_noc)):
        if t is not None and (t.dtype != torch.uint16 or tuple(t.shape) != (H, W)):
            raise ValueError("evaluate_kitti: expected a uint16 %s %s, got %s %s" % (name, (H, W), t.dtype, tuple(t.shape)))
    for t in (gt_occ, gt_noc, out, scratch):
        if t is not None and t.device != disp.device:
            raise ValueError("evaluate_kitti: every tensor must live on the map's device")
    pairs = [(float(a), float(r)) for a, r in thresholds]
    if not 1 <= len(pairs) <= hip.MCCNN_EVAL_MAX_THRESHOLDS:
        raise ValueError("evaluate_kitti: %d thresholds, expected 1..%d" % (len(pairs), hip.MCCNN_EVAL_MAX_THRESHOLDS))
    if out is None:
        if accumulate:
            raise ValueError("evaluate_kitti: accumulate needs the `out` to accumulate into")
        out = torch.empty((EVAL_BYTES // 8,), dtype=torch.int64, device=disp.device)
    elif out.numel() * out.element_size() != EVAL_BYTES:
        raise ValueError("evaluate_kitti: `out` must hold %d bytes" % EVAL_BYTES)
    scratch = scratch if scratch is not None else evaluate_kitti_scratch(H, W, disp.device, interpolate)
    floats = ctypes.c_float * len(pairs)
    hip.check(hip.load().mccnn_evaluate_kitti(hip.ptr(disp), hip.ptr(gt_occ), hip.ptr(gt_noc) if gt_noc is not None else None,
                                              H, W, floats(*[a for a, _ in pairs]), floats(*[r for _, r in pairs]),
                                              len(pairs), 1 if interpolate else 0, 1 if accumulate else 0, hip.ptr(out),
                                              hip.ptr(scratch), scratch.numel() * scratch.element_size(), hip.stream()),
              "mccnn_evaluate_kitti")
    return out


def support_buffer(H, W, device):
    nbytes = int(hip.load().mccnn_support_bytes(H, W))
    buf = torch.empty(((nbytes + 3) // 4,), dtype=torch.int32, device=device)
    return buf[:H * W].view(H, W)


def cross_arms(image, intensity_threshold, distance_threshold, out=None):
    H, W = image.shape
    support = out if out is not None else support_buffer(H, W, image.device)
    hip.check(hip.load().mccnn_cross_arms(hip.ptr(image), H, W, _f32(intensity_threshold), int(distance_threshold),
                                          hip.ptr(support), hip.stream()), "mccnn_cross_arms")
    return support


def cross_arms_pair(image_l, image_r, intensity_threshold, distance_threshold, out_l=None, out_r=None):
    H, W = image_l.shape
    if tuple(image_r.shape) != (H, W):
        raise ValueError("cross_arms_pair: the two images must have the same shape")
    sl = out_l if out_l is not None else support_buffer(H, W, image_l.device)
    sr = out_r if out_r is not None else support_buffer(H, W, image_l.device)
    hip.check(hip.load().mccnn_cross_arms_pair(hip.ptr(image_l), hip.ptr(image_r), H, W, _f32(intensity_threshold),
                                               int(distance_threshold), hip.ptr(sl), hip.ptr(sr), hip.stream()),
              "mccnn_cross_arms_pair")
    return sl, sr


def support_arms(support):
    s = support.to(torch.int64) & 0xFFFFFFFF
    return torch.stack([(s >> sh) & 31 for sh in (0, 5, 10, 15)], dim=-1).to(torch.uint8)


def support_count(support):
    return (((support.to(torch.int64) & 0xFFFFFFFF) >> 20) & 0xFFF).to(torch.int32)


def cross_region_list(support, distance_threshold):
    H, W = support.shape
    L = int(distance_threshold)
    region = torch.empty((H, W, (2 * L) ** 2, 2), dtype=torch.int32, device=support.device)
    hip.check(hip.load().mccnn_cross_region_list(hip.ptr(support), H, W, L, hip.ptr(region), hip.stream()),
              "mccnn_cross_region_list")
    return region


def _check_support(support, H, W, who):
    have = support.untyped_storage().nbytes() - support.storage_offset() * support.element_size()
    if tuple(support.shape) != (H, W) or not support.is_contiguous() or have < hip.load().mccnn_support_bytes(H, W):
        raise ValueError("%s: `support` must be the tensor cross_arms() returned (a copy drops its derived planes)" % who)


def cbca(vol, tmp, support, iterations, distance_threshold, order=hip.MCCNN_CBCA_SEPARABLE, timer=None):
    D, H, W = vol.shape
    lib = hip.load()
    _check_support(support, H, W, "cbca")
    src, dst = vol, tmp
    timer = timer or _NO_TIMER
    for _ in range(int(iterations)):
        timer.start("cbca_iter")
        hip.check(lib.mccnn_cbca_iter(hip.ptr(src), hip.ptr(dst), hip.ptr(support), D, H, W,
                                      int(distance_threshold), int(order), hip.stream()), "mccnn_cbca_iter")
        timer.stop()
        src, dst = dst, src
    return src, dst


def cbca_pair(vol_l, tmp_l, support_l, vol_r, tmp_r, support_r, iterations, distance_threshold,
              order=hip.MCCNN_CBCA_SEPARABLE, timer=None):
    D, H, W = vol_l.shape
    if tuple(vol_r.shape) != (D, H, W):
        raise ValueError("cbca_pair: the two volumes must have the same shape")
    lib = hip.load()
    _check_support(support_l, H, W, "cbca_pair")
    _check_support(support_r, H, W, "cbca_pair")
    (sl, dl), (sr, dr) = (vol_l, tmp_l), (vol_r, tmp_r)
    timer = timer or _NO_TIMER
    for _ in range(int(iterations)):
        timer.start("cbca_iter_pair")
        hip.check(lib.mccnn_cbca_iter_pair(hip.ptr(sl), hip.ptr(dl), hip.ptr(support_l), hip.ptr(sr), hip.ptr(dr),
                                           hip.ptr(support_r), D, H, W, int(distance_threshold), int(order),
                                           hip.stream()), "mccnn_cbca_iter_pair")
        timer.stop()
        sl, dl, sr, dr = dl, sl, dr, sr
    return (sl, dl), (sr, dr)


CBCA_HWD_MAX_DISTANCE = 14
CBCA_MAX_DISTANCE = 32


def aggregation_route(distance, W, D, order=hip.MCCNN_CBCA_REFERENCE_ORDER, extras=None, layout="auto",
                      cbca_kernel="auto", H=1):
    distance = int(distance)
    if distance < 1 or distance > CBCA_MAX_DISTANCE:
        raise ValueError("cbca_distance=%d outside [1, %d]: the support word holds 5-bit arms" % (distance, CBCA_MAX_DISTANCE))
    if layout not in ("auto", "plane_major"):
        raise ValueError("layout must be 'auto' or 'plane_major'")
    if layout != "auto" or order != hip.MCCNN_CBCA_REFERENCE_ORDER or (extras or {}).get("both_view_support"):
        return "plane_major"
    if distance > CBCA_HWD_MAX_DISTANCE:
        return "hwd_long"
    if cbca_kernel != "hwd" and int(hip.load().mccnn_cbca_prog_bytes(int(D), int(H), int(W))) != 0:
        return "prog"
    return "hwd"


def route_cbca_kernel(route, cbca_kernel="auto"):
    return "hwd" if route in ("hwd", "hwd_long") else cbca_kernel


def cbca_hwd(vol, tmp, support, D, iterations, distance_threshold, timer=None):
    H, W, Dp = vol.shape
    assert Dp == hwd_pitch(D) and tuple(tmp.shape) == (H, W, Dp)
    _check_support(support, H, W, "cbca_hwd")
    lib = hip.load()
    src, dst = vol, tmp
    timer = timer or _NO_TIMER
    name = "mccnn_cbca_iter_hwd" if int(distance_threshold) <= CBCA_HWD_MAX_DISTANCE else "mccnn_cbca_iter_hwd_long"
    for _ in range(int(iterations)):
        timer.start("cbca_iter_hwd")
        hip.check(getattr(lib, name)(hip.ptr(src), hip.ptr(dst), hip.ptr(support), int(D), H, W,
                                     int(distance_threshold), hip.stream()), name)
        timer.stop()
        src, dst = dst, src
    return src, dst


def _check_wta_out(wta_out, H, W, who):
    for t in wta_out:
        if tuple(t.shape) != (H, W) or t.dtype != torch.float32 or not t.is_contiguous():
            raise ValueError("%s: wta_out must be two contiguous float32 [H,W] tensors" % who)


def cbca_hwd_wta_max_d():
    return 256


def cbca_hwd_pair(vol_l, tmp_l, support_l, vol_r, tmp_r, support_r, D, iterations, distance_threshold, timer=None,
                  wta_out=None, store_right=True):
    H, W, Dp = vol_l.shape
    assert Dp == hwd_pitch(D)
    for t in (tmp_l, vol_r, tmp_r):
        if tuple(t.shape) != (H, W, Dp):
            raise ValueError("cbca_hwd_pair: the volumes must have the same shape")
    _check_support(support_l, H, W, "cbca_hwd_pair")
    _check_support(support_r, H, W, "cbca_hwd_pair")
    lib = hip.load()
    (sl, dl), (sr, dr) = (vol_l, tmp_l), (vol_r, tmp_r)
    timer = timer or _NO_TIMER
    n = int(iterations)
    long_arms = int(distance_threshold) > CBCA_HWD_MAX_DISTANCE
    if wta_out is not None:
        if n < 1 or D > cbca_hwd_wta_max_d() or long_arms:
            raise ValueError("cbca_hwd_pair: the fused WTA needs at least one iteration, D <= %d and a distance <= %d"
                             % (cbca_hwd_wta_max_d(), CBCA_HWD_MAX_DISTANCE))
        _check_wta_out(wta_out, H, W, "cbca_hwd_pair")
    pair_name = "mccnn_cbca_iter_hwd_long_pair" if long_arms else "mccnn_cbca_iter_hwd_pair"
    for it in range(n):
        timer.start("cbca_iter_hwd_pair")
        if wta_out is not None and it == n - 1:
            hip.check(lib.mccnn_cbca_iter_hwd_pair_wta(hip.ptr(sl), hip.ptr(dl), hip.ptr(support_l), hip.ptr(sr),
                                                       hip.ptr(dr), hip.ptr(support_r), int(D), H, W,
                                                       int(distance_threshold), hip.ptr(wta_out[0]), hip.ptr(wta_out[1]),
                                                       1 if store_right else 0, hip.stream()),
                      "mccnn_cbca_iter_hwd_pair_wta")
        else:
            hip.check(getattr(lib, pair_name)(hip.ptr(sl), hip.ptr(dl), hip.ptr(support_l), hip.ptr(sr), hip.ptr(dr),
                                              hip.ptr(support_r), int(D), H, W, int(distance_threshold),
                                              hip.stream()), pair_name)
        timer.stop()
        sl, dl, sr, dr = dl, sl, dr, sr
    return (sl, dl), (sr, dr)


def cbca_prog_buffers(D, H, W, device):
    n = int(hip.load().mccnn_cbca_prog_bytes(int(D), int(H), int(W)))
    if n == 0:
        return None
    return (torch.empty((n // 4,), dtype=torch.int32, device=device), torch.empty((n // 4,), dtype=torch.int32, device=device))


def cbca_prog_build_pair(support_l, support_r, D, distance_threshold, progs, which="both"):
    H, W = support_l.shape
    _check_support(support_l, H, W, "cbca_prog_build_pair")
    _check_support(support_r, H, W, "cbca_prog_build_pair")
    if which not in ("full", "skip", "both", "both_two_launches"):
        raise ValueError("cbca_prog_build_pair: which must be 'full', 'skip', 'both' or 'both_two_launches'")
    lib = hip.load()
    if which == "both":
        hip.check(lib.mccnn_cbca_prog_build_both_pair(hip.ptr(support_l), hip.ptr(support_r), int(D), H, W,
                                                      int(distance_threshold), hip.ptr(progs[0]), hip.ptr(progs[1]),
                                                      hip.stream()), "mccnn_cbca_prog_build_both_pair")
        _record_built(progs, ("full", "skip"))
        return progs
    for name, fn in (("full", lib.mccnn_cbca_prog_build_pair), ("skip", lib.mccnn_cbca_prog_build_skip_pair)):
        if which in (name, "both_two_launches"):
            hip.check(fn(hip.ptr(support_l), hip.ptr(support_r), int(D), H, W, int(distance_threshold), hip.ptr(progs[0]),
                         hip.ptr(progs[1]), hip.stream()), "mccnn_cbca_prog_build_%spair" % ("skip_" if name == "skip" else ""))
    _record_built(progs, ("full", "skip") if which == "both_two_launches" else (which,))
    return progs


def _record_built(progs, sets):
    for p in progs:
        p._cbca_prog_sets = (set(getattr(p, "_cbca_prog_sets", ())) | {"skip"}) if sets == ("skip",) else set(sets)


def _skip_set_built(progs):
    return all("skip" in getattr(p, "_cbca_prog_sets", ("skip",)) for p in progs)


_RIGHT_STREAMS = {}


def right_stream(device):
    key = (device.type, device.index)
    if key not in _RIGHT_STREAMS:
        _RIGHT_STREAMS[key] = torch.cuda.Stream(device=device)
    return _RIGHT_STREAMS[key]


_PROG_LAUNCH = {
    ("full", 1): ("mccnn_cbca_iter_prog", "cbca_iter_prog"),
    ("refresh", 1): ("mccnn_cbca_iter_prog_refresh", "cbca_iter_prog"),
    ("skip", 1): ("mccnn_cbca_iter_prog_skip", "cbca_iter_prog_skip"),
    ("full", 2): ("mccnn_cbca_iter_prog_pair", "cbca_iter_prog_pair"),
    ("refresh", 2): ("mccnn_cbca_iter_prog_pair_refresh", "cbca_iter_prog_pair"),
    ("skip", 2): ("mccnn_cbca_iter_prog_pair_skip", "cbca_iter_prog_pair_skip"),
    ("wta", 2): ("mccnn_cbca_iter_prog_pair_wta", "cbca_iter_prog_pair"),
}


def _prog_launch(kind, volumes, D, distance_threshold, timer, tail=()):
    name, timed_as = _PROG_LAUNCH[kind, len(volumes)]
    H, W, _ = volumes[0][0].shape
    timer.start(timed_as)
    hip.check(getattr(hip.load(), name)(*[hip.ptr(t) for volume in volumes for t in volume], int(D), H, W,
                                        int(distance_threshold), *tail, hip.stream()), name)
    timer.stop()


def _prog_launch_wta(left, right, D, distance_threshold, wta_out, store_right, timer):
    H, W, _ = left[0].shape
    _check_wta_out(wta_out, H, W, "cbca_prog_pair")
    _prog_launch("wta", (left, right), D, distance_threshold, timer,
                 (hip.ptr(wta_out[0]), hip.ptr(wta_out[1]), 1 if store_right else 0))


def skip_schedule(n, fused_last, skip_unit_regions=True, refresh_first=True):
    n = int(n)
    kinds = []
    for it in range(n):
        if fused_last and it == n - 1:
            kinds.append("wta")
        elif not skip_unit_regions or it == 0:
            kinds.append("full")
        elif refresh_first or not (n % 2 == 0 and it == n - 1):
            kinds.append("skip")
        else:
            kinds.append("full")
    if n >= 2 and n % 2 == 0 and kinds[-1] == "skip":
        kinds[0] = "refresh"
    return kinds


def cbca_prog_pair(vol_l, tmp_l, support_l, vol_r, tmp_r, support_r, progs, D, iterations, distance_threshold, timer=None,
                   wta_out=None, store_right=True, skip_unit_regions=True, right_stream=None, refresh_first=True):
    H, W, Dp = vol_l.shape
    assert Dp == hwd_pitch(D)
    for t in (tmp_l, vol_r, tmp_r):
        if tuple(t.shape) != (H, W, Dp):
            raise ValueError("cbca_prog_pair: the volumes must have the same shape")
    _check_support(support_l, H, W, "cbca_prog_pair")
    _check_support(support_r, H, W, "cbca_prog_pair")
    timer = timer or _NO_TIMER
    n = int(iterations)
    fused = wta_out is not None
    if fused and (n < 1 or D > cbca_hwd_wta_max_d()):
        raise ValueError("cbca_prog_pair: the fused WTA needs at least one iteration and D <= %d" % cbca_hwd_wta_max_d())
    skipping = skip_unit_regions and _skip_set_built(progs)
    (sl, dl), (sr, dr) = (vol_l, tmp_l), (vol_r, tmp_r)
    first = 0
    if right_stream is not None:
        first = n - 1 if fused else n
        main = torch.cuda.current_stream()
        right_stream.wait_stream(main)
        ends = []
        for st, vol, tmp, sup, prog in ((main, vol_l, tmp_l, support_l, progs[0]),
                                        (right_stream, vol_r, tmp_r, support_r, progs[1])):
            with torch.cuda.stream(st):
                ends.append(cbca_prog_chain(vol, tmp, sup, prog, D, first, distance_threshold, total=n, fused_last=fused,
                                            skip_unit_regions=skipping, timer=timer, refresh_first=refresh_first))
        main.wait_stream(right_stream)
        (sl, dl), (sr, dr) = ends
    kinds = skip_schedule(n, fused, skipping, refresh_first)
    for it in range(first, n):
        left, right = (sl, dl, support_l, progs[0]), (sr, dr, support_r, progs[1])
        if kinds[it] == "wta":
            _prog_launch_wta(left, right, D, distance_threshold, wta_out, store_right, timer)
        else:
            _prog_launch(kinds[it], (left, right), D, distance_threshold, timer)
        sl, dl, sr, dr = dl, sl, dr, sr
    return (sl, dl), (sr, dr)


def cbca_prog_chain(vol, tmp, support, prog, D, iterations, distance_threshold, first=0, total=None, fused_last=False,
                    skip_unit_regions=True, timer=None, refresh_first=True):
    n = int(total if total is not None else iterations)
    kinds = skip_schedule(n, fused_last, skip_unit_regions and _skip_set_built((prog,)), refresh_first)
    src, dst = vol, tmp
    timer = timer or _NO_TIMER
    for it in range(int(first), int(iterations)):
        _prog_launch("full" if kinds[it] == "wta" else kinds[it], ((src, dst, support, prog),), D, distance_threshold, timer)
        src, dst = dst, src
    return src, dst


def cbca_both_views(vol, tmp, support_self, support_other, iterations, distance_threshold, side, timer=None):
    D, H, W = vol.shape
    lib = hip.load()
    src, dst = vol, tmp
    timer = timer or _NO_TIMER
    for _ in range(int(iterations)):
        timer.start("cbca_iter_both")
        hip.check(lib.mccnn_cbca_iter_both(hip.ptr(src), hip.ptr(dst), hip.ptr(support_self), hip.ptr(support_other), D, H,
                                           W, int(distance_threshold), int(side), hip.stream()), "mccnn_cbca_iter_both")
        timer.stop()
        src, dst = dst, src
    return src, dst


def hwd_pitch(D):
    return hip.load().mccnn_hwd_pitch(int(D))


def dhw_to_hwd(dhw, hwd=None):
    D, H, W = dhw.shape
    if hwd is None:
        hwd = torch.empty((H, W, hwd_pitch(D)), dtype=torch.float32, device=dhw.device)
    hip.check(hip.load().mccnn_dhw_to_hwd(hip.ptr(dhw), hip.ptr(hwd), D, H, W, hip.stream()), "mccnn_dhw_to_hwd")
    return hwd


def hwd_to_dhw(hwd, D, dhw=None):
    H, W, _ = hwd.shape
    if dhw is None:
        dhw = torch.empty((D, H, W), dtype=torch.float32, device=hwd.device)
    hip.check(hip.load().mccnn_hwd_to_dhw(hip.ptr(hwd), hip.ptr(dhw), int(D), H, W, hip.stream()), "mccnn_hwd_to_dhw")
    return dhw


def sgm_scratch(H, W, D, device):
    n = hip.load().mccnn_sgm_scratch_bytes(H, W, int(D))
    return torch.empty((n,), dtype=torch.uint8, device=device)


def _sgm_arrays(sides, *volume_lists):
    n = len(volume_lists[0])
    return (n, (ctypes.c_int * 2)(*(list(sides) + [0] * (2 - n)))) + tuple(
        (ctypes.c_void_p * 2)(*([v.data_ptr() for v in vols] + [None] * (2 - n))) for vols in volume_lists)


def _sgm_penalties(sgm_P1, sgm_P2, sgm_Q1, sgm_Q2, sgm_D, sgm_V):
    return _f32(sgm_P1), _f32(sgm_P1 / sgm_V), _f32(sgm_P2), _f32(sgm_Q1), _f32(sgm_Q2), _f32(sgm_D)


def _sgm_p1(r, p1h, p1v):
    return p1h if r[0] == 0 else p1v


def sgm_pass_hwd(image_left, image_right, vols_hwd, sides, D, r, p1, p2, q1, q2, thr, scratch):
    H, W = image_left.shape
    n, side_arr, vol_arr = _sgm_arrays(sides, vols_hwd)
    hip.check(hip.load().mccnn_sgm_pass(hip.ptr(image_left), hip.ptr(image_right), vol_arr, side_arr, n, int(D), H, W,
                                        int(r[0]), int(r[1]), p1, p2, q1, q2, thr, hip.ptr(scratch),
                                        scratch.numel(), hip.stream()), "mccnn_sgm_pass")


SGM_DIRECTIONS = ((0, 1), (0, -1), (-1, 0), (1, 0))


def sgm_flags_hwd(image_left, image_right, D, r, thr, flags):
    H, W = image_left.shape
    hip.check(hip.load().mccnn_sgm_flags(hip.ptr(image_left), hip.ptr(image_right), int(D), H, W, int(r[0]), int(r[1]), thr,
                                         hip.ptr(flags), flags.numel(), hip.stream()), "mccnn_sgm_flags")


def sgm_flag_planes(image_left, image_right, D, sgm_D, out=None):
    H, W = image_left.shape
    planes = out if out is not None else [sgm_scratch(H, W, D, image_left.device) for _ in SGM_DIRECTIONS]
    for r, buf in zip(SGM_DIRECTIONS, planes):
        sgm_flags_hwd(image_left, image_right, D, r, _f32(sgm_D), buf)
    return planes


def sgm_pass_flagged_hwd(vols_hwd, sides, D, r, p1, p2, q1, q2, flags):
    H, W, _ = vols_hwd[0].shape
    n, side_arr, vol_arr = _sgm_arrays(sides, vols_hwd)
    hip.check(hip.load().mccnn_sgm_pass_flagged(vol_arr, side_arr, n, int(D), H, W, int(r[0]), int(r[1]), p1, p2, q1, q2,
                                                hip.ptr(flags), flags.numel(), hip.stream()), "mccnn_sgm_pass_flagged")


def sgm_average_hwd(image_left, image_right, vols_hwd, sides, D, sgm_P1, sgm_P2, sgm_Q1, sgm_Q2, sgm_D, sgm_V,
                    scratch, timer=_NO_TIMER, flags=None):
    p1h, p1v, p2, q1, q2, thr = _sgm_penalties(sgm_P1, sgm_P2, sgm_Q1, sgm_Q2, sgm_D, sgm_V)
    for i, r in enumerate(SGM_DIRECTIONS):
        timer.start("sgm_pass" if len(vols_hwd) == 2 else "sgm_pass_one_volume")
        if flags is not None:
            sgm_pass_flagged_hwd(vols_hwd, sides, D, r, _sgm_p1(r, p1h, p1v), p2, q1, q2, flags[i])
        else:
            sgm_pass_hwd(image_left, image_right, vols_hwd, sides, D, r, _sgm_p1(r, p1h, p1v), p2, q1, q2, thr, scratch)
        timer.stop()


def sgm_pass_accumulate_hwd(srcs_hwd, accs_hwd, sides, D, r, p1, p2, q1, q2, mode, flags):
    H, W, _ = srcs_hwd[0].shape
    n, side_arr, src_arr, acc_arr = _sgm_arrays(sides, srcs_hwd, accs_hwd)
    hip.check(hip.load().mccnn_sgm_pass_accumulate(src_arr, acc_arr, side_arr, n, int(D), H, W, int(r[0]), int(r[1]), p1,
                                                   p2, q1, q2, int(mode), hip.ptr(flags), flags.numel(), hip.stream()),
              "mccnn_sgm_pass_accumulate")


SGM_ACC_MODES = (hip.MCCNN_SGM_ACC_STORE, hip.MCCNN_SGM_ACC_ADD, hip.MCCNN_SGM_ACC_ADD, hip.MCCNN_SGM_ACC_ADD_QUARTER)


def sgm_average_independent_hwd(image_left, image_right, vols_hwd, spares_hwd, sides, D, sgm_P1, sgm_P2, sgm_Q1, sgm_Q2,
                                sgm_D, sgm_V, scratch, timer=_NO_TIMER, flags=None):
    p1h, p1v, p2, q1, q2, thr = _sgm_penalties(sgm_P1, sgm_P2, sgm_Q1, sgm_Q2, sgm_D, sgm_V)
    for i, (r, mode) in enumerate(zip(SGM_DIRECTIONS, SGM_ACC_MODES)):
        timer.start("sgm_pass_accumulate" if len(vols_hwd) == 2 else "sgm_pass_accumulate_one_volume")
        planes = flags[i] if flags is not None else scratch
        if flags is None:
            sgm_flags_hwd(image_left, image_right, D, r, thr, scratch)
        sgm_pass_accumulate_hwd(vols_hwd, spares_hwd, sides, D, r, _sgm_p1(r, p1h, p1v), p2, q1, q2, mode, planes)
        timer.stop()
    return list(spares_hwd), list(vols_hwd)


SGM_FIRST_PASS_MAX_D = 256


def sgm_average_from_dhw(image_left, image_right, vols_dhw, vols_hwd, sides, D, sgm_P1, sgm_P2, sgm_Q1, sgm_Q2, sgm_D,
                         sgm_V, scratch, timer=_NO_TIMER):
    H, W = image_left.shape
    p1h, p1v, p2, q1, q2, thr = _sgm_penalties(sgm_P1, sgm_P2, sgm_Q1, sgm_Q2, sgm_D, sgm_V)
    rest = SGM_DIRECTIONS
    if D <= SGM_FIRST_PASS_MAX_D:
        n, side_arr, src, dst = _sgm_arrays(sides, vols_dhw, vols_hwd)
        timer.start("sgm_first_pass")
        hip.check(hip.load().mccnn_sgm_first_pass(hip.ptr(image_left), hip.ptr(image_right), src, dst, side_arr, n,
                                                  int(D), H, W, p1h, p2, q1, q2, thr, hip.ptr(scratch),
                                                  scratch.numel(), hip.stream()), "mccnn_sgm_first_pass")
        timer.stop()
        rest = SGM_DIRECTIONS[1:]
    else:
        timer.start("dhw_to_hwd")
        for a, b in zip(vols_dhw, vols_hwd):
            dhw_to_hwd(a, b)
        timer.stop()
    for r in rest:
        timer.start("sgm_pass")
        sgm_pass_hwd(image_left, image_right, vols_hwd, sides, D, r, _sgm_p1(r, p1h, p1v), p2, q1, q2, thr, scratch)
        timer.stop()


def wta(vol, out=None):
    D, H, W = vol.shape
    disp = out if out is not None else torch.empty((H, W), dtype=torch.float32, device=vol.device)
    hip.check(hip.load().mccnn_wta(hip.ptr(vol), D, H, W, hip.ptr(disp), hip.stream()), "mccnn_wta")
    return disp


def wta_hwd(vol_hwd, D, out=None):
    H, W, Dp = vol_hwd.shape
    assert Dp == hwd_pitch(D)
    disp = out if out is not None else torch.empty((H, W), dtype=torch.float32, device=vol_hwd.device)
    hip.check(hip.load().mccnn_wta_hwd(hip.ptr(vol_hwd), int(D), H, W, hip.ptr(disp), hip.stream()), "mccnn_wta_hwd")
    return disp


def wta_any(vol, D, pixel_major, out=None):
    return wta_hwd(vol, D, out=out) if pixel_major else wta(vol, out=out)


def subpixel_hwd(dl, vol_hwd, D, out=None, numpy1_promotion=False):
    H, W, Dp = vol_hwd.shape
    assert Dp == hwd_pitch(D)
    out = out if out is not None else torch.empty_like(dl)
    hip.check(hip.load().mccnn_subpixel_hwd(hip.ptr(dl), hip.ptr(vol_hwd), int(D), H, W, 1 if numpy1_promotion else 0,
                                            hip.ptr(out), hip.stream()), "mccnn_subpixel_hwd")
    return out


CONFIDENCE_MEASURES = ("msm", "mmn", "cur", "lrc")
_CONFIDENCE_BITS = dict(msm=hip.MCCNN_CONF_MSM, mmn=hip.MCCNN_CONF_MMN, cur=hip.MCCNN_CONF_CUR, lrc=hip.MCCNN_CONF_LRC)


def confidence_mask(names):
    names = (names,) if isinstance(names, str) else tuple(names)
    mask = 0
    for name in names:
        bit = _CONFIDENCE_BITS.get(name)
        if bit is None:
            raise ValueError("unknown confidence measure %r: choose from %s" % (name, ", ".join(CONFIDENCE_MEASURES)))
        if mask & bit:
            raise ValueError("confidence measure %r named twice" % (name,))
        mask |= bit
    if not mask:
        raise ValueError("no confidence measure named: choose from %s" % ", ".join(CONFIDENCE_MEASURES))
    return mask


def confidence_names(measures):
    mask = measures if isinstance(measures, int) else confidence_mask(measures)
    return tuple(n for n in CONFIDENCE_MEASURES if mask & _CONFIDENCE_BITS[n])


VIEW_SUFFIX = {"left": "", "right": "_right"}


def _view_suffix(view):
    if view not in VIEW_SUFFIX:
        raise ValueError("view must be 'left' or 'right'")
    return VIEW_SUFFIX[view]


def _confidence(entry, vol, D, H, W, disp_other, measures, out):
    mask = confidence_mask(measures)
    k = bin(mask).count("1")
    if mask & hip.MCCNN_CONF_LRC and disp_other is None:
        raise ValueError("%s: the lrc measure needs the other view's disparity map" % entry)
    if disp_other is not None and (tuple(disp_other.shape) != (H, W) or disp_other.dtype != torch.float32):
        raise ValueError("%s: the other view's disparity must be a float32 [H,W] map" % entry)
    if vol.dtype != torch.float32:
        raise ValueError("%s: the volume must be float32" % entry)
    if out is None:
        out = torch.empty((k, H, W), dtype=torch.float32, device=vol.device)
    elif tuple(out.shape) != (k, H, W) or out.dtype != torch.float32:
        raise ValueError("%s: `out` must be a float32 [%d,%d,%d] tensor" % (entry, k, H, W))
    hip.check(getattr(hip.load(), entry)(hip.ptr(vol), hip.ptr(disp_other) if disp_other is not None else None, int(D), H,
                                         W, mask, hip.ptr(out), hip.stream()), entry)
    return out


def confidence_hwd(vol_hwd, D, disp_right=None, measures=CONFIDENCE_MEASURES, out=None, view="left"):
    H, W, Dp = vol_hwd.shape
    assert Dp == hwd_pitch(D)
    return _confidence("mccnn_confidence%s_hwd" % _view_suffix(view), vol_hwd, D, H, W, disp_right, measures, out)


def confidence(vol_dhw, disp_right=None, measures=CONFIDENCE_MEASURES, out=None, view="left"):
    D, H, W = vol_dhw.shape
    return _confidence("mccnn_confidence" + _view_suffix(view), vol_dhw, D, H, W, disp_right, measures, out)


def confidence_any(vol, D, pixel_major, disp_other=None, measures=CONFIDENCE_MEASURES, out=None, view="left"):
    if pixel_major:
        return confidence_hwd(vol, D, disp_other, measures, out=out, view=view)
    return confidence(vol, disp_other, measures, out=out, view=view)


def confidence_right_hwd(vol_right_hwd, D, disp_left=None, measures=CONFIDENCE_MEASURES, out=None):
    return confidence_hwd(vol_right_hwd, D, disp_left, measures, out=out, view="right")


def confidence_right(vol_right_dhw, disp_left=None, measures=CONFIDENCE_MEASURES, out=None):
    return confidence(vol_right_dhw, disp_left, measures, out=out, view="right")


def lr_status(dl, dr, ndisp, out=None, view="left"):
    entry = "mccnn_lr_status" + _view_suffix(view)
    H, W = dl.shape
    st = out if out is not None else torch.empty((H, W), dtype=torch.int32, device=dl.device)
    hip.check(getattr(hip.load(), entry)(hip.ptr(dl), hip.ptr(dr), H, W, int(ndisp), hip.ptr(st), hip.stream()), entry)
    return st


def lr_status_right(dr, dl, ndisp, out=None):
    return lr_status(dr, dl, ndisp, out=out, view="right")


def interpolate(dl, status, out=None, directions=4, occlusion_from_left=False, view="left"):
    H, W = dl.shape
    out = out if out is not None else torch.empty_like(dl)
    rules = (int(directions), 1 if occlusion_from_left else 0)
    if _view_suffix(view):
        entry = "mccnn_interpolate_right"
    elif rules == (4, 0):
        entry, rules = "mccnn_interpolate", ()
    else:
        entry = "mccnn_interpolate_ex"
    hip.check(getattr(hip.load(), entry)(hip.ptr(dl), hip.ptr(status), H, W, *rules, hip.ptr(out), hip.stream()), entry)
    return out


def interpolate_right(dr, status, out=None, directions=4, occlusion_from_right=False):
    return interpolate(dr, status, out=out, directions=directions, occlusion_from_left=occlusion_from_right, view="right")


def subpixel(dl, vol, out=None, numpy1_promotion=False):
    D, H, W = vol.shape
    out = out if out is not None else torch.empty_like(dl)
    if numpy1_promotion:
        hip.check(hip.load().mccnn_subpixel_ex(hip.ptr(dl), hip.ptr(vol), D, H, W, 1, hip.ptr(out), hip.stream()),
                  "mccnn_subpixel_ex")
    else:
        hip.check(hip.load().mccnn_subpixel(hip.ptr(dl), hip.ptr(vol), D, H, W, hip.ptr(out), hip.stream()),
                  "mccnn_subpixel")
    return out


def subpixel_any(dl, vol, D, pixel_major, out=None, numpy1_promotion=False):
    if pixel_major:
        return subpixel_hwd(dl, vol, D, out=out, numpy1_promotion=numpy1_promotion)
    return subpixel(dl, vol, out=out, numpy1_promotion=numpy1_promotion)


def median(dl, fh, fw, out=None):
    H, W = dl.shape
    out = out if out is not None else torch.empty_like(dl)
    hip.check(hip.load().mccnn_median(hip.ptr(dl), H, W, int(fh), int(fw), hip.ptr(out), hip.stream()),
              "mccnn_median")
    return out


def bilateral_table(filter_height, filter_width, mean, std_dev):
    constant1 = 1. / (np.sqrt(2 * np.pi) * std_dev)
    constant2 = -1. / (2 * std_dev * std_dev)
    center_h = (filter_height - 1) // 2
    center_w = (filter_width - 1) // 2
    tab = np.zeros([filter_height, filter_width], dtype=np.float32)
    for h in range(filter_height):
        for w in range(filter_width):
            x = np.sqrt((h - center_h) ** 2 + (w - center_w) ** 2)
            tab[h, w] = constant1 * np.exp(constant2 * ((x - mean) ** 2))
    return tab


_TABLES = {}


def bilateral_table_device(fh, fw, mean, std_dev, device):
    key = (int(fh), int(fw), float(mean), float(std_dev), str(device))
    tab = _TABLES.get(key)
    if tab is None:
        tab = torch.from_numpy(bilateral_table(int(fh), int(fw), mean, std_dev)).to(device)
        _TABLES[key] = tab
    return tab


def bilateral(image, dl, fh, fw, mean, std_dev, blur_threshold, out=None):
    H, W = dl.shape
    tab = bilateral_table_device(fh, fw, mean, std_dev, dl.device)
    out = out if out is not None else torch.empty_like(dl)
    hip.check(hip.load().mccnn_bilateral(hip.ptr(image), hip.ptr(dl), H, W, int(fh), int(fw), hip.ptr(tab),
                                         _f32(blur_threshold), hip.ptr(out), hip.stream()), "mccnn_bilateral")
    return out


DEFAULT_HP = dict(cbca_intensity=0.02, cbca_distance=14, cbca_num_iterations1=2, cbca_num_iterations2=16,
                  sgm_P1=2.3, sgm_P2=55.9, sgm_Q1=4, sgm_Q2=8, sgm_D=0.08, sgm_V=1.5, blur_sigma=6,
                  blur_threshold=2)


SGM_MAX_D = 1024
COST_VOLUME_HWD_MAX_D = 1024
DECISION_AUTO = "kernel"


VIEWS = ("left", "both")
PostView = collections.namedtuple("PostView", "name suffix image own other volume status maps dst planes stream")


def check_envelope(H, W, D):
    H, W, D = int(H), int(W), int(D)
    if H < 1 or W < 1:
        raise ValueError("%dx%d: empty image" % (W, H))
    if D < 2 or D > SGM_MAX_D:
        raise ValueError("ndisp=%d outside [2, %d]: SGM is built for at most %d disparities" % (D, SGM_MAX_D, SGM_MAX_D))
    if D > W - 2:
        raise ValueError("ndisp=%d needs an image at least ndisp + 2 = %d pixels wide, got W=%d" % (D, D + 2, W))


def workspace_bytes(H, W, D, pixel_major=True, cbca_kernel="auto", pairs_in_flight=1, arch="fast",
                    fc_units=DECISION_UNITS, confidence=0, views="left"):
    check_envelope(H, W, D)
    if views not in VIEWS:
        raise ValueError("views must be 'left' or 'both'")
    lib = hip.load()
    H, W, D = int(H), int(W), int(D)
    dp = (D + 3) & ~3
    n = 4 * H * W * dp * 4
    n += 5 * int(lib.mccnn_sgm_scratch_bytes(H, W, D))
    n += 2 * int(lib.mccnn_support_bytes(H, W))
    n += H * W * 4 + 6 * H * W * 4
    if pixel_major and cbca_kernel != "hwd":
        n += 2 * int(lib.mccnn_cbca_prog_bytes(D, H, W))
    if arch not in ("fast", "accurate"):
        raise ValueError("arch must be 'fast' or 'accurate'")
    if arch == "accurate":
        n += 2 * H * W * int(fc_units) * 4
    n += int(confidence) * H * W * 4
    if views == "both":
        n += (1 + 3 + 2 + int(confidence)) * H * W * 4
    return n * max(1, int(pairs_in_flight))


def _require_device_memory(nbytes, what):
    free, _total = torch.cuda.mem_get_info()
    avail = free + torch.cuda.memory_reserved() - torch.cuda.memory_allocated()
    if nbytes > avail:
        raise RuntimeError("%s needs %.2f GB of device memory, %.2f GB are available" % (what, nbytes / 1e9, avail / 1e9))


class StereoMatcher(object):

    def __init__(self, net, hp=None, cv_mode=hip.MCCNN_CV_EXACT, cbca_order=hip.MCCNN_CBCA_REFERENCE_ORDER,
                 feature_tile_rows=None, extras=None, features="auto", layout="auto", cbca_kernel="auto",
                 on_saturation="fallback", skip_unit_regions=True, two_chains=True, free_chains=True, refresh_first=True,
                 sgm_flags_once=True, decision="auto", confidence=(), views="left"):
        self.device = hip.require_device()
        self.net = net
        self.hp = dict(DEFAULT_HP)
        if hp:
            self.hp.update(hp)
        self.cv_mode = cv_mode
        self.cbca_order = cbca_order
        self.feature_tile_rows = feature_tile_rows
        if features not in ("auto", "miopen", "split_f16"):
            raise ValueError("features must be 'auto', 'miopen' or 'split_f16'")
        if features == "split_f16" and feature_tile_rows is not None:
            raise ValueError("row banding is implemented for the library convolutions only")
        if features == "auto":
            features = "split_f16" if (feature_tile_rows is None and net.supports_split_features()) else "miopen"
        self.features = features
        if decision not in ("auto", "kernel", "library"):
            raise ValueError("decision must be 'auto', 'kernel' or 'library'")
        self.accurate = hasattr(net, "fc_weights")
        self.decision = decision
        if self.accurate and features == "split_f16":
            raise ValueError("the split-operand feature kernels are built for the fast network")
        if layout not in ("auto", "plane_major"):
            raise ValueError("layout must be 'auto' or 'plane_major'")
        self.layout = layout
        if cbca_kernel not in ("auto", "prog", "hwd"):
            raise ValueError("cbca_kernel must be 'auto', 'prog' or 'hwd'")
        self.cbca_kernel = cbca_kernel
        if on_saturation not in ("fallback", "raise", "ignore"):
            raise ValueError("on_saturation must be 'fallback', 'raise' or 'ignore'")
        self.on_saturation = on_saturation
        self._library_twin = None
        self._decision_ran = None
        self.skip_unit_regions = bool(skip_unit_regions)
        self.two_chains = bool(two_chains)
        self.free_chains = bool(free_chains)
        self.refresh_first = bool(refresh_first)
        self.sgm_flags_once = bool(sgm_flags_once)
        self.extras = dict(both_view_support=False, interpolation_directions=4, occlusion_from_left=False,
                           numpy1_promotion=False, sgm_independent_directions=False)
        if extras:
            unknown = set(extras) - set(self.extras)
            if unknown:
                raise ValueError("unknown extras: %s" % sorted(unknown))
            self.extras.update(extras)
        self.confidence = confidence_names(confidence) if confidence else ()
        if views not in VIEWS:
            raise ValueError("views must be 'left' or 'both'")
        self.views = views
        self.both = views == "both"
        self._ws = {}
        self._graphs = {}
        self._side = None
        self._right = None
        self._ingest = None

    def _right_stream(self):
        if self._right is None:
            self._right = torch.cuda.Stream()
        return self._right

    def features_saturated(self, reset=True):
        return self.net.split_saturated(reset)

    def saturation_checked(self):
        return self.features == "split_f16" or (self.accurate and self._decision_ran == "kernel")

    def saturation_notice(self):
        if self.accurate:
            return "activations left the matrix-core decision kernel's range: {} repeated on the float32 library decision route"
        return ("activations left the matrix-core feature kernels' range: {} repeated with the float32 library "
                "convolutions")

    def workspace(self, H, W, D):
        key = (H, W, D)
        ws = self._ws.get(key)
        if ws is None:
            need = workspace_bytes(H, W, D, self.pixel_major(), self.workspace_cbca_kernel(H, W, D),
                                   arch="accurate" if self.accurate else "fast",
                                   fc_units=self.net.num_fc_units if self.accurate else DECISION_UNITS,
                                   confidence=len(self.confidence), views=self.views)
            self._ws, self._graphs = {}, {}
            _require_device_memory(need, "StereoMatcher: the workspace of a %dx%d pair with ndisp=%d" % (W, H, D))
            dp = hwd_pitch(D)
            n = H * W * dp
            dev = self.device
            ws = dict(
                vol=[torch.empty((n,), dtype=torch.float32, device=dev) for _ in range(4)],
                scratch=sgm_scratch(H, W, D, dev),
                sgm_flags=[sgm_scratch(H, W, D, dev) for _ in SGM_DIRECTIONS],
                sup_l=support_buffer(H, W, dev), sup_r=support_buffer(H, W, dev),
                status=torch.empty((H, W), dtype=torch.int32, device=dev),
                maps=torch.empty((6, H, W), dtype=torch.float32, device=dev),
            )
            if self.accurate:
                ws["halves"] = tuple(torch.empty((H, W, self.net.num_fc_units), dtype=torch.float32, device=dev)
                                     for _ in range(2))
            if self.confidence:
                ws["confidence"] = torch.empty(((2,) if self.both else ()) + (len(self.confidence), H, W),
                                               dtype=torch.float32, device=dev)
            if self.both:
                ws["status_right"] = torch.empty((H, W), dtype=torch.int32, device=dev)
                ws["maps_right"] = torch.empty((3, H, W), dtype=torch.float32, device=dev)
                ws["both"] = torch.empty((2, H, W), dtype=torch.float32, device=dev)
            ws["progs"] = None
            if self.route(H, W, D) == "prog":
                ws["progs"] = cbca_prog_buffers(D, H, W, dev)
            elif self.pixel_major() and self.cbca_kernel == "prog":
                raise ValueError("cbca_kernel='prog': %dx%dx%d (cbca_distance %d) is outside what the aggregation "
                                 "programs encode" % (W, H, D, int(self.hp["cbca_distance"])))
            bilateral_table_device(5, 5, 0, self.hp["blur_sigma"], dev)
            self._ws = {key: ws}
            self._graphs = {}
        return ws

    def route(self, H, W, D):
        return aggregation_route(self.hp["cbca_distance"], W, D, self.cbca_order, self.extras, self.layout,
                                 self.cbca_kernel, H)

    def workspace_cbca_kernel(self, H, W, D):
        return route_cbca_kernel(self.route(H, W, D), self.cbca_kernel)

    def pixel_major(self):
        return aggregation_route(self.hp["cbca_distance"], 1, 1, self.cbca_order, self.extras, self.layout,
                                 "hwd") != "plane_major"

    def _saturated_pair(self, left_image, right_image, ndisp, out, keep=None, confidence_out=None):
        if not self.saturation_checked() or self.on_saturation == "ignore" or torch.cuda.is_current_stream_capturing():
            return None
        if not self.features_saturated():
            return None
        if self.on_saturation == "raise":
            raise RuntimeError("StereoMatcher: an activation left the range of the split-operand %s "
                               "(|x| >= 255.9); match this pair with %s" % (
                                   ("decision kernel", "decision='library'") if self.accurate else
                                   ("feature kernels", "features='miopen'")))
        if self._library_twin is None:
            self._library_twin = StereoMatcher(self.net, hp=self.hp, cv_mode=self.cv_mode, cbca_order=self.cbca_order,
                                               extras=self.extras, features="miopen", layout=self.layout,
                                               cbca_kernel=self.cbca_kernel, on_saturation="ignore", decision="library",
                                               confidence=self.confidence, views=self.views)
        if keep is not None:
            keep.clear()
        return self._library_twin.match(left_image, right_image, ndisp, out=out, keep=keep, confidence_out=confidence_out)

    def match(self, left_image, right_image, ndisp, timer=_NO_TIMER, keep=None, _static_out=False, out=None,
              confidence_out=None):
        res = self._match(left_image, right_image, ndisp, timer=timer, keep=keep, _static_out=_static_out, out=out,
                          confidence_out=confidence_out)
        if not _static_out:
            redo = self._saturated_pair(left_image, right_image, ndisp, out, keep, confidence_out)
            if redo is not None:
                return redo
        return res

    def _side_work(self, ws, L, R, D, want_flags):
        hp = self.hp
        if self._side is None:
            self._side = torch.cuda.Stream()
        self._side.wait_stream(torch.cuda.current_stream())
        with torch.cuda.stream(self._side):
            sup_l, sup_r = cross_arms_pair(L, R, hp["cbca_intensity"], hp["cbca_distance"], ws["sup_l"], ws["sup_r"])
            if ws["progs"] is not None:
                cbca_prog_build_pair(sup_l, sup_r, D, hp["cbca_distance"], ws["progs"],
                                     "both" if self.skip_unit_regions else "full")
            flag_planes = sgm_flag_planes(L, R, D, hp["sgm_D"], out=ws["sgm_flags"]) if want_flags else None
            ready = torch.cuda.Event()
            ready.record(self._side)
        return sup_l, sup_r, flag_planes, ready

    def _side_work_timed(self, ws, L, R, D, timer):
        hp = self.hp
        timer.start("cross_arms")
        sup_l, sup_r = cross_arms_pair(L, R, hp["cbca_intensity"], hp["cbca_distance"], ws["sup_l"], ws["sup_r"])
        timer.stop()
        if ws["progs"] is not None:
            timer.start("cbca_prog_build")
            cbca_prog_build_pair(sup_l, sup_r, D, hp["cbca_distance"], ws["progs"])
            timer.stop()
        return sup_l, sup_r

    def decision_route(self, W, D):
        if self.decision == "library":
            return "library"
        why = decision_kernel_refusal(self.net, W, D)
        if why is None:
            return DECISION_AUTO if self.decision == "auto" else "kernel"
        if self.decision == "kernel":
            raise ValueError("decision='kernel': %s" % why)
        import warnings
        warnings.warn("accurate network: %s; the decision stage runs on the float32 library route" % why)
        return "library"

    def _cost_volumes_accurate(self, ws, fl, fr, D, dhw, hwd, timer):
        direct = self.pixel_major() and D <= COST_VOLUME_HWD_MAX_D
        route = self.decision_route(fl.shape[1], D)
        self._decision_ran = route
        timer.start("cost_volume")
        left, right = cost_volume_accurate(self.net, fl, fr, D, mode=self.cv_mode, decision=route, pixel_major=direct,
                                           out=(hwd[2], hwd[3]) if direct else (dhw[0], dhw[1]), halves=ws["halves"],
                                           sat_flag=self.net._split_flag() if route == "kernel" else None)
        timer.stop()
        return left, right, direct

    def _cost_volumes(self, fl, fr, D, dhw, hwd, timer, ws=None):
        if self.accurate:
            return self._cost_volumes_accurate(ws, fl, fr, D, dhw, hwd, timer)
        direct = self.pixel_major() and D <= COST_VOLUME_HWD_MAX_D
        timer.start("cost_volume")
        if direct:
            left, right = cost_volume_hwd(fl, fr, D, out=(hwd[2], hwd[3]), mode=self.cv_mode)
        else:
            left, right = cost_volume(fl, fr, D, self.cv_mode, out=(dhw[0], dhw[1]))
        timer.stop()
        return left, right, direct

    def _sgm_hp(self):
        return [self.hp[k] for k in ("sgm_P1", "sgm_P2", "sgm_Q1", "sgm_Q2", "sgm_D", "sgm_V")]

    def _wta(self, lv, rv, D, pixel_major, m, timer):
        timer.start("wta")
        dl, dr = wta_any(lv, D, pixel_major, out=m[0]), wta_any(rv, D, pixel_major, out=m[1])
        timer.stop()
        return dl, dr

    def _pixel_major_free(self, ws, L, R, D, left, right, sups, flag_planes, fuse, m, timer):
        hp, progs, dist = self.hp, ws["progs"], self.hp["cbca_distance"]
        n1, n2 = int(hp["cbca_num_iterations1"]), int(hp["cbca_num_iterations2"])
        if flag_planes is None and self.sgm_flags_once:
            timer.start("sgm_flags")
            flag_planes = sgm_flag_planes(L, R, D, hp["sgm_D"], out=ws["sgm_flags"])
            timer.stop()
        if flag_planes is None and "scratch2" not in ws:
            ws["scratch2"] = sgm_scratch(L.shape[0], L.shape[1], D, self.device)
        chain = dict(skip_unit_regions=self.skip_unit_regions, refresh_first=self.refresh_first, timer=timer)
        main_s, right_s = torch.cuda.current_stream(), self._right_stream()
        right_s.wait_stream(main_s)
        ends = []
        for st, (v, t), sup, prog, side, scr in ((main_s, left, sups[0], progs[0], hip.MCCNN_SIDE_LEFT, ws["scratch"]),
                                                 (right_s, right, sups[1], progs[1], hip.MCCNN_SIDE_RIGHT, ws.get("scratch2"))):
            with torch.cuda.stream(st):
                timer.span_start("aggregation_1")
                v, t = cbca_prog_chain(v, t, sup, prog, D, n1, dist, **chain)
                timer.span_stop("aggregation_1")
                timer.span_start("sgm")
                if self.extras["sgm_independent_directions"]:
                    (v,), (t,) = sgm_average_independent_hwd(L, R, [v], [t], [side], D, *self._sgm_hp(), scr, timer,
                                                             flags=flag_planes)
                else:
                    sgm_average_hwd(L, R, [v], [side], D, *self._sgm_hp(), scr, timer, flags=flag_planes)
                timer.span_stop("sgm")
                timer.span_start("aggregation_2")
                v, t = cbca_prog_chain(v, t, sup, prog, D, n2 - 1 if fuse else n2, dist, total=n2, fused_last=fuse, **chain)
                timer.span_stop("aggregation_2")
                ends.append((v, t))
        main_s.wait_stream(right_s)
        (lh, lt), (rh, rt) = ends
        if not fuse:
            return self._wta(lh, rh, D, True, m, timer) + (lh, rh)
        _prog_launch_wta((lh, lt, sups[0], progs[0]), (rh, rt, sups[1], progs[1]), D, dist, (m[0], m[1]), self.both,
                         timer)
        return m[0], m[1], lt, rt

    def _aggregate_hwd(self, progs, left, right, sups, D, n, timer, **kw):
        (lh, lt), (rh, rt) = left, right
        if progs is None:
            return cbca_hwd_pair(lh, lt, sups[0], rh, rt, sups[1], D, int(n), self.hp["cbca_distance"], timer, **kw)
        return cbca_prog_pair(lh, lt, sups[0], rh, rt, sups[1], progs, D, int(n), self.hp["cbca_distance"], timer,
                              skip_unit_regions=self.skip_unit_regions, refresh_first=self.refresh_first,
                              right_stream=self._right_stream() if self.two_chains else None, **kw)

    def _pixel_major_joined(self, ws, L, R, D, left, right, sups, fuse, m, timer, keep):
        hp, progs = self.hp, ws["progs"]
        sides = [hip.MCCNN_SIDE_LEFT, hip.MCCNN_SIDE_RIGHT]
        timer.span_start("aggregation_1")
        (lh, lt), (rh, rt) = self._aggregate_hwd(progs, left, right, sups, D, hp["cbca_num_iterations1"], timer)
        timer.span_stop("aggregation_1")
        if keep is not None:
            keep["cbca1"] = (hwd_to_dhw(lh, D), hwd_to_dhw(rh, D))
        timer.span_start("sgm")
        if self.extras["sgm_independent_directions"]:
            (lh, rh), (lt, rt) = sgm_average_independent_hwd(L, R, [lh, rh], [lt, rt], sides, D, *self._sgm_hp(),
                                                             ws["scratch"], timer)
        else:
            sgm_average_hwd(L, R, [lh, rh], sides, D, *self._sgm_hp(), ws["scratch"], timer)
        timer.span_stop("sgm")
        if keep is not None:
            keep["sgm"] = (hwd_to_dhw(lh, D), hwd_to_dhw(rh, D))
        timer.span_start("aggregation_2")
        (lh, lt), (rh, rt) = self._aggregate_hwd(progs, (lh, lt), (rh, rt), sups, D, hp["cbca_num_iterations2"], timer,
                                                 wta_out=(m[0], m[1]) if fuse else None,
                                                 store_right=keep is not None or self.both)
        timer.span_stop("aggregation_2")
        if keep is not None:
            keep["cbca2"] = (hwd_to_dhw(lh, D), hwd_to_dhw(rh, D))
        return ((m[0], m[1]) if fuse else self._wta(lh, rh, D, True, m, timer)) + (lh, rh)

    def _aggregate_dhw(self, left, right, sups, n, timer):
        dist, both = self.hp["cbca_distance"], self.extras["both_view_support"]
        if not both and self.cbca_order == hip.MCCNN_CBCA_SEPARABLE:
            return cbca_pair(left[0], left[1], sups[0], right[0], right[1], sups[1], n, dist, self.cbca_order, timer)
        res = []
        for (vol, tmp), own, other, side in ((left, sups[0], sups[1], hip.MCCNN_SIDE_LEFT),
                                             (right, sups[1], sups[0], hip.MCCNN_SIDE_RIGHT)):
            res.append(cbca_both_views(vol, tmp, own, other, n, dist, side, timer) if both
                       else cbca(vol, tmp, own, n, dist, self.cbca_order, timer))
        return res

    def _plane_major(self, ws, L, R, D, left, right, hwd, sups, m, timer, keep):
        hp = self.hp
        (lcv, t1d), (rcv, t2d) = self._aggregate_dhw(left, right, sups, hp["cbca_num_iterations1"], timer)
        if keep is not None:
            keep["cbca1"] = (lcv.clone(), rcv.clone())
        lh = next(h for b, h in zip(ws["vol"], hwd) if b.data_ptr() == t1d.data_ptr())
        rh = next(h for b, h in zip(ws["vol"], hwd) if b.data_ptr() == t2d.data_ptr())
        sides = [hip.MCCNN_SIDE_LEFT, hip.MCCNN_SIDE_RIGHT]
        if self.extras["sgm_independent_directions"]:
            timer.start("dhw_to_hwd")
            dhw_to_hwd(lcv, lh)
            dhw_to_hwd(rcv, rh)
            timer.stop()
            la = next(h for b, h in zip(ws["vol"], hwd) if b.data_ptr() == lcv.data_ptr())
            ra = next(h for b, h in zip(ws["vol"], hwd) if b.data_ptr() == rcv.data_ptr())
            sgm_average_independent_hwd(L, R, [lh, rh], [la, ra], sides, D, *self._sgm_hp(), ws["scratch"], timer)
            timer.start("hwd_to_dhw")
            hwd_to_dhw(la, D, t1d)
            hwd_to_dhw(ra, D, t2d)
            timer.stop()
            lcv, t1d, rcv, t2d = t1d, lcv, t2d, rcv
        else:
            sgm_average_from_dhw(L, R, [lcv, rcv], [lh, rh], sides, D, *self._sgm_hp(), ws["scratch"], timer)
            timer.start("hwd_to_dhw")
            hwd_to_dhw(lh, D, lcv)
            hwd_to_dhw(rh, D, rcv)
            timer.stop()
        if keep is not None:
            keep["sgm"] = (lcv.clone(), rcv.clone())
        (lcv, t1d), (rcv, t2d) = self._aggregate_dhw((lcv, t1d), (rcv, t2d), sups, hp["cbca_num_iterations2"], timer)
        if keep is not None:
            keep["cbca2"] = (lcv.clone(), rcv.clone())
        return self._wta(lcv, rcv, D, False, m, timer) + (lcv, rcv)

    def _post_view(self, v, D, pixel_major, timer, keep):
        hp, ex = self.hp, self.extras
        timer.start("post" + v.suffix)
        st = lr_status(v.own, v.other, D, out=v.status, view=v.name)
        di = interpolate(v.own, st, out=v.maps[0], directions=ex["interpolation_directions"],
                         occlusion_from_left=ex["occlusion_from_left"], view=v.name)
        ds = subpixel_any(di, v.volume, D, pixel_major, out=v.maps[1], numpy1_promotion=ex["numpy1_promotion"])
        dm = median(ds, 5, 5, out=v.maps[2])
        db = bilateral(v.image, dm, 5, 5, 0, hp["blur_sigma"], hp["blur_threshold"], out=v.dst)
        timer.stop()
        stages = dict(status=st, interp=di, subpixel=ds, median=dm, bilateral=db)
        if self.confidence:
            timer.start("confidence" + v.suffix)
            stages["confidence"] = confidence_any(v.volume, D, pixel_major, v.other, self.confidence, out=v.planes,
                                                  view=v.name)
            timer.stop()
        if keep is not None:
            keep.update((name + v.suffix, t) for name, t in stages.items())

    def _check_given(self, t, shape, name, dims, like):
        if t is not None and (tuple(t.shape) != shape or t.dtype != torch.float32 or not t.is_contiguous()
                              or t.device != like.device):
            raise ValueError("match: %s`%s` must be a contiguous float32 [%s%s] tensor on the images' device" % (
                "with views='both' " if self.both else "", name, "2," if self.both else "", dims))

    @staticmethod
    def _hand_out(t, given, handed):
        return t if (handed or given is not None) else t.clone()

    def _match(self, left_image, right_image, ndisp, timer=_NO_TIMER, keep=None, _static_out=False, out=None,
               confidence_out=None):
        L = left_image.reshape(left_image.shape[0], left_image.shape[1]).contiguous()
        R = right_image.reshape(right_image.shape[0], right_image.shape[1]).contiguous()
        H, W = L.shape
        D = int(ndisp)
        ws = self.workspace(H, W, D)
        dp = hwd_pitch(D)
        dhw = [b[:D * H * W].view(D, H, W) for b in ws["vol"]]
        hwd = [b[:H * W * dp].view(H, W, dp) for b in ws["vol"]]
        overlap = timer is _NO_TIMER
        free = self.free_chains and self.two_chains and keep is None and ws["progs"] is not None
        flag_planes = None

        timer.start("features")
        if self.features == "split_f16":
            fl, fr = self.net.features_pair_hwc_split(L, R)
        else:
            fl, fr = self.net.features_pair_hwc(L, R, tile_rows=self.feature_tile_rows)
        timer.stop()
        if overlap:
            sup_l, sup_r, flag_planes, ready = self._side_work(ws, L, R, D, want_flags=free and self.sgm_flags_once)
        lv, rv, pixel_major = self._cost_volumes(fl, fr, D, dhw, hwd, timer, ws)
        del fl, fr
        if keep is not None:
            keep["cv"] = (hwd_to_dhw(lv, D), hwd_to_dhw(rv, D)) if pixel_major else (lv.clone(), rv.clone())
        if overlap:
            torch.cuda.current_stream().wait_event(ready)
        else:
            sup_l, sup_r = self._side_work_timed(ws, L, R, D, timer)
        sups = (sup_l, sup_r)

        m = ws["maps"] if keep is None else torch.empty_like(ws["maps"])
        if self.pixel_major():
            if not pixel_major:
                timer.start("cv_to_pixel_major")
                lv, rv = dhw_to_hwd(lv, hwd[2]), dhw_to_hwd(rv, hwd[3])
                timer.stop()
            fuse = (int(self.hp["cbca_num_iterations2"]) >= 1 and D <= cbca_hwd_wta_max_d()
                    and int(self.hp["cbca_distance"]) <= CBCA_HWD_MAX_DISTANCE)
            if free:
                dl, dr, left_volume, right_volume = self._pixel_major_free(ws, L, R, D, (lv, hwd[0]), (rv, hwd[1]), sups,
                                                                           flag_planes, fuse, m, timer)
            else:
                dl, dr, left_volume, right_volume = self._pixel_major_joined(ws, L, R, D, (lv, hwd[0]), (rv, hwd[1]), sups,
                                                                             fuse, m, timer, keep)
        else:
            dl, dr, left_volume, right_volume = self._plane_major(ws, L, R, D, (lv, dhw[2]), (rv, dhw[3]), hwd, sups, m,
                                                                  timer, keep)

        both, k, fresh, pm = self.both, len(self.confidence), keep is not None, self.pixel_major()
        lead = (2,) if both else ()
        self._check_given(out, lead + (H, W), "out", "H,W", L)
        if k or both:
            self._check_given(confidence_out, lead + (k, H, W), "confidence_out", "K,H,W", L)

        def dest(given, spare):
            return given if given is not None else (torch.empty_like(spare) if fresh else spare)
        res = dest(out, ws["both"] if both else ws["maps"][5])
        planes = dest(confidence_out, ws["confidence"]) if k else None
        main_s = torch.cuda.current_stream()
        fork = both and timer is _NO_TIMER
        if both:
            right_s = self._right_stream() if fork else main_s
            if fork:
                right_s.wait_stream(main_s)
            view = PostView("right", "_right", R, dr, dl, right_volume, None if fresh else ws["status_right"],
                            torch.empty_like(ws["maps_right"]) if fresh else ws["maps_right"], res[1],
                            planes[1] if k else None, right_s)
            with torch.cuda.stream(view.stream):
                self._post_view(view, D, pm, timer, keep)
            if fresh:
                keep["cbca2_right"] = hwd_to_dhw(right_volume, D) if pm else right_volume.clone()
        view = PostView("left", "", L, dl, dr, left_volume, None if fresh else ws["status"], m[2:5],
                        res[0] if both else res, planes[0] if k and both else planes, main_s)
        self._post_view(view, D, pm, timer, keep)
        if fork:
            main_s.wait_stream(right_s)
        if fresh:
            keep["wta"] = (dl, dr)
        handed = _static_out or fresh
        res = self._hand_out(res, out, handed)
        return (res, self._hand_out(planes, confidence_out, handed)) if k else res

    def _ingest_buffers(self, H, W):
        b = self._ingest
        if b is None or b[0] != (H, W):
            dev = self.device
            b = ((H, W), torch.empty((H, W), dtype=torch.float32, device=dev),
                 torch.empty((H, W), dtype=torch.float32, device=dev), ingest_scratch(H, W, dev))
            self._ingest = b
        return b[1:]

    def match_u8(self, left_u8, right_u8, ndisp, out=None, confidence_out=None):
        H, W, _ = _u8_image(left_u8)
        sl, sr, scratch = self._ingest_buffers(H, W)
        left_u8 = left_u8.to(self.device, non_blocking=True).contiguous()
        right_u8 = right_u8.to(self.device, non_blocking=True).contiguous()
        ingest_u8_pair(left_u8, right_u8, sl, sr, scratch)
        return self.match(sl, sr, ndisp, out=out, confidence_out=confidence_out)

    def _graph_key(self, key):
        if not self.accurate:
            return key
        key = key + (self.net.decision_weights_key(),)
        for k in [k for k in self._graphs if k[-1] != key[-1]]:
            del self._graphs[k]
        return key

    def _capture(self, key, shape, make_static, prologue=None):
        H, W, D = shape
        self.workspace(H, W, D)
        self._side = self._right = None
        static = make_static()
        side = torch.cuda.Stream()
        side.wait_stream(torch.cuda.current_stream())
        with torch.cuda.stream(side):
            for _ in range(2):
                if prologue is not None:
                    prologue(*static)
                self._match(static[0], static[1], D)
        torch.cuda.current_stream().wait_stream(side)
        torch.cuda.synchronize()
        graph = torch.cuda.CUDAGraph()
        with torch.cuda.graph(graph):
            if prologue is not None:
                prologue(*static)
            out = self._match(static[0], static[1], D, _static_out=True)
        self._graphs[key] = (graph, static, out)
        return self._graphs[key]

    def _saturated_graph_pair(self, sl, sr, ndisp, out):
        if self.confidence:
            self._saturated_pair(sl, sr, ndisp, out[0], confidence_out=out[1])
        else:
            self._saturated_pair(sl, sr, ndisp, out)

    def _static_u8(self, left_u8, right_u8, H, W):
        bl = torch.empty(tuple(left_u8.shape), dtype=torch.uint8, device=self.device)
        br = torch.empty_like(bl)
        sl = torch.empty((H, W), dtype=torch.float32, device=self.device)
        sr = torch.empty((H, W), dtype=torch.float32, device=self.device)
        scratch = ingest_scratch(H, W, self.device)
        bl.copy_(left_u8)
        br.copy_(right_u8)
        return sl, sr, bl, br, scratch

    def match_graph_u8(self, left_u8, right_u8, ndisp):
        H, W, C = _u8_image(left_u8)
        if _u8_image(right_u8) != (H, W, C):
            raise ValueError("match_graph_u8: the two images must have the same shape")
        key = self._graph_key((H, W, int(ndisp), "u8", C))
        g = self._graphs.get(key) or self._capture(
            key, key[:3], lambda: self._static_u8(left_u8, right_u8, H, W),
            lambda sl, sr, bl, br, scratch: ingest_u8_pair(bl, br, sl, sr, scratch))
        graph, (sl, sr, bl, br, _scratch), out = g
        bl.copy_(left_u8, non_blocking=True)
        br.copy_(right_u8, non_blocking=True)
        graph.replay()
        self._saturated_graph_pair(sl, sr, ndisp, out)
        return out

    @staticmethod
    def _static_f32(L, R):
        sl, sr = torch.empty_like(L, dtype=torch.float32), torch.empty_like(R, dtype=torch.float32)
        sl.copy_(L)
        sr.copy_(R)
        return sl, sr

    def match_graph(self, left_image, right_image, ndisp):
        L = left_image.reshape(left_image.shape[0], left_image.shape[1])
        R = right_image.reshape(right_image.shape[0], right_image.shape[1])
        key = self._graph_key((L.shape[0], L.shape[1], int(ndisp)))
        graph, (sl, sr), out = self._graphs.get(key) or self._capture(key, key[:3], lambda: self._static_f32(L, R))
        sl.copy_(L)
        sr.copy_(R)
        graph.replay()
        self._saturated_graph_pair(sl, sr, ndisp, out)
        return out
```

Baseline: 11270 Mdisparities/s.

## Fuse conv1 into the first 3x3 split-MFMA conv kernel

Adds a conv12_split kernel that computes layer-1 (1→64 channel 3x3 conv, bias, ReLU, fp16 hi/lo split) on the fly from an image patch held in LDS. Those layer-1 values feed the layer-2 MFMA convolution directly, and the layer-1 ALU work is interleaved between MFMA steps. This removes the write and re-read of the 256-byte-per-pixel layer-1 intermediate in HBM, plus one kernel launch. In exchange it uses more LDS and registers, which may lower occupancy, and adds per-tile recomputation of halo pixels.

```diff
diff --git a/include/mccnn.h b/include/mccnn.h
--- a/include/mccnn.h
+++ b/include/mccnn.h
@@ -240,6 +240,9 @@
                       int pad, float act_scale, int *saturation_flag, mccnn_stream_t stream);
 int mccnn_conv3x3_split(const void *in, const void *packed_weights, const float *bias, void *out, int N, int Hi, int Wi,
                         float weight_scale, float act_scale, int last, int *saturation_flag, mccnn_stream_t stream);
+int mccnn_conv12_split(const float *left, const float *right, const float *weights1, const float *bias1,
+                       const void *packed_weights, const float *bias, void *out, int H, int W, int pad,
+                       float weight_scale, float act_scale, int last, int *saturation_flag, mccnn_stream_t stream);
 
 #ifdef __cplusplus
 }
diff --git a/mc-cnn-python_amd/csrc/conv12_mfma.hip b/mc-cnn-python_amd/csrc/conv12_mfma.hip
--- /dev/null
+++ b/mc-cnn-python_amd/csrc/conv12_mfma.hip
@@ -0,0 +1,31 @@
+#include "conv_mfma.h"
+
+extern "C" int mccnn_conv12_split(const float *left, const float *right, const float *w1, const float *b1,
+                                  const void *packed_weights, const float *bias, void *out, int H, int W, int pad,
+                                  float weight_scale, float act_scale, int last, int *saturation_flag,
+                                  mccnn_stream_t stream)
+{
+    using namespace mccnn;
+    using namespace cs;
+    const char *who = "mccnn_conv12_split";
+    MCCNN_REQUIRE(left && w1 && b1 && packed_weights && bias && out, MCCNN_E_INVALID, "mccnn_conv12_split: null pointer");
+    MCCNN_REQUIRE(H > 0 && W > 0 && pad >= 0, MCCNN_E_INVALID, "mccnn_conv12_split: bad size");
+    MCCNN_REQUIRE(weight_scale > 0.f && act_scale > 0.f, MCCNN_E_INVALID, "mccnn_conv12_split: scales must be positive");
+    const int N = right ? 2 : 1;
+    const long Hi = (long)H + 2 * pad - 2, Wi = (long)W + 2 * pad - 2;
+    MCCNN_REQUIRE(Hi > 2 && Wi > 2, MCCNN_E_INVALID, "mccnn_conv12_split: layer-1 grid %ldx%ld too small", Wi, Hi);
+    MCCNN_REQUIRE(Hi <= 0x7fffffffL && Wi <= 0x7fffffffL &&
+                      (size_t)N * (size_t)(Hi - 2) * (size_t)(Wi - 2) * REC <= 0x7ffffff0u,
+                  MCCNN_E_UNSUPPORTED, "mccnn_conv12_split: %d x %ldx%ld records exceed 32-bit buffer offsets", N,
+                  Wi - 2, Hi - 2);
+    MCCNN_REQUIRE((size_t)H * W * 4 <= 0x7ffffff0u, MCCNN_E_UNSUPPORTED,
+                  "mccnn_conv12_split: a %dx%d view exceeds 32-bit buffer offsets", W, H);
+    hipStream_t s = (hipStream_t)stream;
+    typedef const float *__restrict__ view_t;
+    return last ? launch_conv3x3_split<1, true, view_t, view_t, view_t, int, int, int>(
+                      who, left, packed_weights, bias, out, N, (int)Hi, (int)Wi, weight_scale, act_scale,
+                      saturation_flag, s, right, w1, b1, H, W, pad)
+                : launch_conv3x3_split<0, true, view_t, view_t, view_t, int, int, int>(
+                      who, left, packed_weights, bias, out, N, (int)Hi, (int)Wi, weight_scale, act_scale,
+                      saturation_flag, s, right, w1, b1, H, W, pad);
+}
diff --git a/mc-cnn-python_amd/csrc/conv_mfma.h b/mc-cnn-python_amd/csrc/conv_mfma.h
--- /dev/null
+++ b/mc-cnn-python_amd/csrc/conv_mfma.h
@@ -0,0 +1,493 @@
+#pragma once
+#include "common.h"
+
+namespace mccnn {
+
+typedef _Float16 h8 __attribute__((ext_vector_type(8)));
+typedef _Float16 h4 __attribute__((ext_vector_type(4)));
+typedef float f16x __attribute__((ext_vector_type(16)));
+typedef uint32_t w4 __attribute__((ext_vector_type(4)));
+typedef uint32_t w2 __attribute__((ext_vector_type(2)));
+
+#ifndef CONV_STAGE_TAP
+#define CONV_STAGE_TAP 0
+#endif
+#ifndef CONV_L1_SCHED
+#define CONV_L1_SCHED 1
+#endif
+#ifndef CONV_NBW
+#define CONV_NBW 4
+#endif
+namespace cs {
+constexpr int NBW = CONV_NBW;
+constexpr int TH = 4 * NBW, TW = 32;
+constexpr int IH = TH + 2, IW = TW + 2;
+constexpr int NPIX = IH * IW;
+constexpr int SLOT = 80;
+constexpr int QBUF = NPIX * SLOT;
+constexpr int NITEM = NPIX * 4;
+constexpr int NST = (NITEM + 255) / 256;
+constexpr int EPITCH = 272;
+constexpr int EPX = NBW >= 4 ? 32 : 16;
+constexpr int EPI = EPX * EPITCH;
+constexpr int LDS_BYTES = 2 * QBUF + 4 * EPI;
+constexpr int PH = IH + 2, PW = IW + 2;
+constexpr int NPATCH = PH * PW;
+constexpr int NPL = (NPATCH + 255) / 256;
+constexpr int PATCH_BYTES = NPATCH * 4;
+constexpr int LDS_BYTES_FIRST = LDS_BYTES + 2 * PATCH_BYTES;
+constexpr int UHALF = (NPIX + 127) / 128 * 128;
+constexpr int NUR = 2 * UHALF / 256;
+constexpr int NL1 = NUR * 8;
+constexpr int REC = 256;
+constexpr int WFRAG = 1024;
+constexpr int WLAYER = 36 * 4 * WFRAG;
+}
+
+__device__ __forceinline__ void split4(const float y[4], float scale, w2 &hi, w2 &lo)
+{
+    h4 a, b;
+#pragma unroll
+    for (int j = 0; j < 4; ++j) {
+        const float v = fminf(fmaxf(y[j] * scale, -65504.f), 65504.f);
+        const _Float16 h = (_Float16)v;
+        a[j] = h;
+        b[j] = (_Float16)(v - (float)h);
+    }
+    hi = __builtin_bit_cast(w2, a);
+    lo = __builtin_bit_cast(w2, b);
+}
+
+__device__ __forceinline__ void split4_scaled(const float v[4], w2 &hi, w2 &lo)
+{
+    h4 a, b;
+#pragma unroll
+    for (int j = 0; j < 4; ++j) {
+        const _Float16 h = (_Float16)v[j];
+        a[j] = h;
+        b[j] = (_Float16)(v[j] - (float)h);
+    }
+    hi = __builtin_bit_cast(w2, a);
+    lo = __builtin_bit_cast(w2, b);
+}
+
+__device__ __forceinline__ float conv1_map(const float v[9], const float w[9], float b, float act_scale, bool &sat)
+{
+    float acc = 0.f;
+#pragma unroll
+    for (int k = 0; k < 9; ++k) acc += w[k] * v[k];
+    acc += b;
+    sat |= !(acc * act_scale <= 65504.f);
+    return fmaxf(acc, 0.f);
+}
+
+__device__ __forceinline__ void pin_loads()
+{
+    asm volatile("" ::: "memory");
+    __builtin_amdgcn_sched_barrier(0x78f);
+}
+
+template <int I, typename T, typename... R>
+__device__ __forceinline__ auto pack_arg(T t, R... r)
+{
+    if constexpr (I == 0)
+        return t;
+    else
+        return pack_arg<I - 1>(r...);
+}
+
+template <int MODE, bool FIRST, typename... L1>
+__global__ __launch_bounds__(256) void conv3x3_split_kernel(const char *__restrict__ in, const char *__restrict__ wpk,
+                                                            const float *__restrict__ bias, char *__restrict__ out,
+                                                            int N, int Hi, int Wi, float inv_scale, float act_scale,
+                                                            int tiles_x, int tiles_y, int total,
+                                                            int *__restrict__ sat_flag, L1... l1)
+{
+    static_assert(sizeof...(L1) == (FIRST ? 6 : 0), "in_b, w1, b1, H, W, pad with FIRST, no further argument without");
+    const float *in_b = nullptr, *w1 = nullptr, *b1 = nullptr;
+    int H = 0, W = 0, pad = 0;
+    if constexpr (FIRST) {
+        in_b = pack_arg<0>(l1...);
+        w1 = pack_arg<1>(l1...);
+        b1 = pack_arg<2>(l1...);
+        H = pack_arg<3>(l1...);
+        W = pack_arg<4>(l1...);
+        pad = pack_arg<5>(l1...);
+    }
+    using namespace cs;
+    extern __shared__ __attribute__((aligned(16))) char lds[];
+    const int tid = threadIdx.x, lane = tid & 63;
+    const int wave = __builtin_amdgcn_readfirstlane(tid >> 6);
+    const int Ho = Hi - 2, Wo = Wi - 2;
+    const size_t in_bytes = (size_t)N * Hi * Wi * REC, out_bytes = (size_t)N * Ho * Wo * REC;
+    const __amdgpu_buffer_rsrc_t rs_in = __builtin_amdgcn_make_buffer_rsrc(
+        const_cast<char *>(in), 0, (int)in_bytes, 0x00020000);
+    const __amdgpu_buffer_rsrc_t rs_w =
+        __builtin_amdgcn_make_buffer_rsrc(const_cast<char *>(wpk), 0, WLAYER, 0x00020000);
+    const __amdgpu_buffer_rsrc_t rs_out = __builtin_amdgcn_make_buffer_rsrc(
+        out, 0, (int)out_bytes, 0x00020000);
+
+    int goff[NST], loff[NST];
+#pragma unroll
+    for (int r = 0; r < NST; ++r) {
+        const int i = r * 256 + tid, p = min(i >> 2, NPIX - 1), part = i & 3;
+        const int py = p / IW, px = p - py * IW;
+        goff[r] = (py * Wi + px) * REC + part * 16;
+        loff[r] = p * SLOT + part * 16;
+    }
+    const bool last_piece = (NST - 1) * 256 + tid < NITEM;
+
+    auto xcd_order = [](int b, int n) {
+        const int q = n >> 3, r = n & 7, x = b & 7;
+        return (x < r ? x * (q + 1) : r * (q + 1) + (x - r) * q) + (b >> 3);
+    };
+    auto tile_base = [&](int v, int &n, int &ty0, int &tx0) {
+        const int t = xcd_order(v, total);
+        const int tx = t % tiles_x, r = t / tiles_x;
+        const int ty = r % tiles_y;
+        n = r / tiles_y;
+        ty0 = ty * TH;
+        tx0 = tx * TW;
+    };
+
+    w4 st[NST];
+    auto fetch = [&](int n, int ty0, int tx0, int q) {
+        const int so = ((n * Hi + ty0) * Wi + tx0) * REC + q * 64;
+#ifdef CONV_ABL_NOSTAGE
+        if (so == 0x7fffffff)
+#endif
+#pragma unroll
+        for (int r = 0; r < NST; ++r) st[r] = __builtin_amdgcn_raw_buffer_load_b128(rs_in, goff[r], so, 0);
+    };
+    auto commit = [&](int buf) {
+        char *b = lds + buf * QBUF;
+#pragma unroll
+        for (int r = 0; r < NST; ++r)
+            if (r < NST - 1 || last_piece) *reinterpret_cast<w4 *>(b + loff[r]) = st[r];
+    };
+
+    float *const patch = reinterpret_cast<float *>(lds + 2 * QBUF + 4 * EPI);
+    float pv[NPL];
+    auto load_patch = [&](int n, int ty0, int tx0) {
+        const __amdgpu_buffer_rsrc_t rs_img = __builtin_amdgcn_make_buffer_rsrc(
+            const_cast<float *>(n ? in_b : reinterpret_cast<const float *>(in)), 0, H * W * 4, 0x00020000);
+#pragma unroll
+        for (int r = 0; r < NPL; ++r) {
+            const int i = r * 256 + tid, py = i / PW, px = i - py * PW;
+            const int y = ty0 + py - pad, x = tx0 + px - pad;
+            const bool ok = i < NPATCH && y >= 0 && y < H && x >= 0 && x < W;
+            pv[r] = __uint_as_float(__builtin_amdgcn_raw_buffer_load_b32(rs_img, ok ? (y * W + x) * 4 : 0x7ffffff0, 0, 0));
+        }
+    };
+    auto store_patch = [&](float *pt) {
+#pragma unroll
+        for (int r = 0; r < NPL; ++r)
+            if (r * 256 + tid < NPATCH) pt[r * 256 + tid] = pv[r];
+    };
+    static_assert(UHALF % 64 == 0, "the half must be wave-uniform");
+    constexpr int RMIX = UHALF / 256;
+    const int mixed = RMIX * 256 + 64 * wave >= UHALF ? 8 : 0;
+    const float *const w1m = w1 + mixed * 9, *const b1m = b1 + mixed;
+    auto l1_fetch_w = [&](int qn, int r, int m, float *w) {
+        const int c = 16 * qn + m;
+        const float *pw = r == RMIX ? w1m : r < RMIX ? w1 : w1 + 72;
+        const float *pbias = r == RMIX ? b1m : r < RMIX ? b1 : b1 + 8;
+#pragma unroll
+        for (int i = 0; i < 9; ++i) w[i] = pw[c * 9 + i];
+        w[9] = pbias[c];
+    };
+    float l1v[9], l1y[4];
+    w2 l1hi[2], l1lo[2];
+    char *l1dst = lds;
+    bool l1over = false, l1store = false, l1grid = false;
+    uint32_t sat1 = 0;
+    auto l1_item = [&](int r, int m, const float *w, char *buf, const float *pt, int ty0, int tx0) {
+        if (m == 0) {
+            const int u = r * 256 + tid, hf = u >= UHALF ? 1 : 0, p = u - hf * UHALF;
+            const int pc = min(p, NPIX - 1), py = pc / IW, px = pc - py * IW;
+            const float *s = pt + py * PW + px;
+#pragma unroll
+            for (int i = 0; i < 9; ++i) l1v[i] = s[(i / 3) * PW + i % 3];
+            l1store = p < NPIX;
+            l1dst = l1store ? buf + pc * SLOT + hf * 16 : lds + 2 * QBUF + wave * EPI + lane * 64;
+            l1grid = ty0 + py < Hi && tx0 + px < Wi;
+        }
+        l1y[m & 3] = conv1_map(l1v, w, w[9], act_scale, l1over);
+        asm volatile("" : "+v"(l1y[m & 3]));
+        if ((m & 3) == 3) split4(l1y, act_scale, l1hi[m >> 2], l1lo[m >> 2]);
+        if (m == 7) {
+            const w4 z = {0u, 0u, 0u, 0u};
+            *reinterpret_cast<w4 *>(l1dst) = l1grid ? w4{l1hi[0].x, l1hi[0].y, l1hi[1].x, l1hi[1].y} : z;
+            *reinterpret_cast<w4 *>(l1dst + 32) = l1grid ? w4{l1lo[0].x, l1lo[0].y, l1lo[1].x, l1lo[1].y} : z;
+            sat1 |= l1over && l1store && l1grid ? 1u : 0u;
+            asm volatile("" : "+v"(sat1));
+            l1over = false;
+        }
+    };
+
+    int v = blockIdx.x;
+    if (v >= total) return;
+    int n, ty0, tx0;
+    tile_base(v, n, ty0, tx0);
+    float l1w[2][10];
+    int pb = 0;
+    if constexpr (FIRST) {
+        load_patch(n, ty0, tx0);
+        store_patch(patch);
+        __syncthreads();
+#pragma unroll 1
+        for (int r = 0; r < NUR; ++r)
+#pragma unroll
+            for (int m = 0; m < 8; ++m) {
+                l1_fetch_w(0, r, m, l1w[0]);
+                l1_item(r, m, l1w[0], lds, patch, ty0, tx0);
+            }
+        l1_fetch_w(1, 0, 0, l1w[0]);
+    } else {
+        fetch(n, ty0, tx0, 0);
+        commit(0);
+    }
+    __syncthreads();
+
+    constexpr int NSLOT = MODE == 0 ? 3 : 4;
+    w4 af[NSLOT][4];
+    auto fetch_a = [&](int slot, int ks) {
+#pragma unroll
+        for (int f = 0; f < 4; ++f)
+            af[slot][f] = __builtin_amdgcn_raw_buffer_load_b128(rs_w, lane * 16, (ks * 4 + f) * WFRAG, 0);
+    };
+#pragma unroll
+    for (int i = 0; i < NSLOT - 1; ++i) fetch_a(i, i);
+
+    const int bfrag = (wave * NBW * IW + (lane & 31)) * SLOT + 16 * (lane >> 5);
+    char *const epi = lds + 2 * QBUF + wave * EPI;
+
+    while (true) {
+        f16x acc[NBW][2], accx[NBW][2];
+#pragma unroll
+        for (int nb = 0; nb < NBW; ++nb)
+#pragma unroll
+            for (int mb = 0; mb < 2; ++mb)
+#pragma unroll
+                for (int i = 0; i < 16; ++i) acc[nb][mb][i] = accx[nb][mb][i] = 0.f;
+        const int vn = v + gridDim.x;
+        int nn = 0, nty0 = 0, ntx0 = 0;
+        if (vn < total) tile_base(vn, nn, nty0, ntx0);
+        if (vn >= total) {
+            nn = n;
+            nty0 = ty0;
+            ntx0 = tx0;
+        }
+#pragma unroll
+        for (int q = 0; q < 4; ++q) {
+            auto stage_next = [&]() {
+                if constexpr (FIRST) {
+                    if (q == 0) {
+                        load_patch(nn, nty0, ntx0);
+                        pin_loads();
+                    }
+                } else {
+                    if (q < 3)
+                        fetch(n, ty0, tx0, q + 1);
+                    else
+                        fetch(nn, nty0, ntx0, 0);
+                    pin_loads();
+                }
+            };
+            auto l1_run = [&](int k) {
+                const int k1 = (k + 1) % NL1, q1 = k + 1 < NL1 ? (q + 1) & 3 : (q + 2) & 3;
+                l1_fetch_w(q1, k1 >> 3, k1 & 7, l1w[(k + 1) & 1]);
+                l1_item(k >> 3, k & 7, l1w[k & 1], lds + ((q + 1) & 1) * QBUF, patch + (q < 3 ? pb : pb ^ 1) * NPATCH,
+                        q < 3 ? ty0 : nty0, q < 3 ? tx0 : ntx0);
+            };
+            if (CONV_STAGE_TAP < 0) stage_next();
+            const char *bq = lds + (q & 1) * QBUF + bfrag;
+            char *const other = lds + ((q + 1) & 1) * QBUF;
+            w4 bf[2][2];
+            auto read_b = [&](int slot, int step) {
+                const int tap = step / NBW, nb = step % NBW;
+                const int dy = tap / 3, dx = tap - dy * 3;
+                const char *pb = bq + ((nb + dy) * IW + dx) * SLOT;
+                bf[slot][0] = *reinterpret_cast<const w4 *>(pb);
+                bf[slot][1] = *reinterpret_cast<const w4 *>(pb + 32);
+            };
+            read_b(0, 0);
+#pragma unroll
+            for (int tap = 0; tap < 9; ++tap) {
+                const int ks = q * 9 + tap;
+                fetch_a((ks + NSLOT - 1) % NSLOT, (ks + NSLOT - 1) % 36);
+                pin_loads();
+                if (tap == CONV_STAGE_TAP) stage_next();
+                const int slot = ks % NSLOT;
+                const h8 a_hi0 = __builtin_bit_cast(h8, af[slot][0]), a_hi1 = __builtin_bit_cast(h8, af[slot][1]);
+                const h8 a_lo0 = __builtin_bit_cast(h8, af[slot][2]), a_lo1 = __builtin_bit_cast(h8, af[slot][3]);
+#pragma unroll
+                for (int nb = 0; nb < NBW; ++nb) {
+                    const int step = tap * NBW + nb;
+                    if (step + 1 < 9 * NBW) read_b((step + 1) & 1, step + 1);
+                    __builtin_amdgcn_sched_barrier(0);
+                    const h8 b_hi = __builtin_bit_cast(h8, bf[step & 1][0]);
+                    const h8 b_lo = __builtin_bit_cast(h8, bf[step & 1][1]);
+                    accx[nb][0] = __builtin_amdgcn_mfma_f32_32x32x16_f16(a_lo0, b_hi, accx[nb][0], 0, 0, 0);
+                    accx[nb][1] = __builtin_amdgcn_mfma_f32_32x32x16_f16(a_lo1, b_hi, accx[nb][1], 0, 0, 0);
+                    accx[nb][0] = __builtin_amdgcn_mfma_f32_32x32x16_f16(a_hi0, b_lo, accx[nb][0], 0, 0, 0);
+                    accx[nb][1] = __builtin_amdgcn_mfma_f32_32x32x16_f16(a_hi1, b_lo, accx[nb][1], 0, 0, 0);
+                    acc[nb][0] = __builtin_amdgcn_mfma_f32_32x32x16_f16(a_hi0, b_hi, acc[nb][0], 0, 0, 0);
+                    acc[nb][1] = __builtin_amdgcn_mfma_f32_32x32x16_f16(a_hi1, b_hi, acc[nb][1], 0, 0, 0);
+                    if constexpr (FIRST) {
+                        constexpr int two = NL1 - 9 * NBW;
+                        static_assert(two >= 0 && two <= 9 * NBW, "one or two items per row step");
+#if CONV_L1_SCHED == 0
+                        if (step == 9 * NBW - 1)
+#pragma unroll
+                            for (int k = 0; k < NL1; ++k) l1_run(k);
+#else
+                        if (step < two) {
+                            l1_run(2 * step);
+                            l1_run(2 * step + 1);
+                        } else {
+                            l1_run(step + two);
+                        }
+#endif
+                    }
+                }
+                if constexpr (FIRST) {
+                    if (q == 1 && tap == 4) store_patch(patch + (pb ^ 1) * NPATCH);
+                }
+                if (!FIRST && tap >= 9 - (NST + 1) / 2) {
+#pragma unroll
+                    for (int j = 0; j < 2; ++j) {
+                        const int r = 2 * (tap - (9 - (NST + 1) / 2)) + j;
+                        if (r < NST && (r < NST - 1 || last_piece)) *reinterpret_cast<w4 *>(other + loff[r]) = st[r];
+                    }
+                }
+            }
+            __syncthreads();
+        }
+
+        const int px = lane & 31, half = lane >> 5;
+        bool sat = false;
+#ifdef CONV_ABL_NOEPI
+        {
+            float t = 0.f;
+#pragma unroll
+            for (int nb = 0; nb < NBW; ++nb)
+#pragma unroll
+                for (int mb = 0; mb < 2; ++mb)
+#pragma unroll
+                    for (int r = 0; r < 16; ++r) t += acc[nb][mb][r] + accx[nb][mb][r];
+            if (t == 123.456f) __builtin_amdgcn_raw_buffer_store_b32(__float_as_uint(t), rs_out, lane * 4, 0, 0);
+        }
+#else
+#pragma unroll
+        for (int nb = 0; nb < NBW; ++nb) {
+            float y[2][16];
+            float ss = 0.f;
+#pragma unroll
+            for (int mb = 0; mb < 2; ++mb)
+#pragma unroll
+                for (int r = 0; r < 16; ++r) {
+                    const int ch = 32 * mb + (r & 3) + 8 * (r >> 2) + 4 * half;
+                    if (MODE == 0) {
+                    } else {
+                        const float t = fmaf(acc[nb][mb][r] + accx[nb][mb][r], inv_scale, bias[ch]);
+                        y[mb][r] = t;
+                        ss = fmaf(t, t, ss);
+                    }
+                }
+            float nrm = 1.f;
+            if (MODE == 1) {
+                ss += __shfl_xor(ss, 32);
+                nrm = 1.f / sqrtf(fmaxf(ss, 1e-12f));
+            }
+            const int row = ty0 + wave * NBW + nb;
+            const int so = ((n * Ho + min(row, Ho - 1)) * Wo + tx0) * REC;
+            const bool stored = row < Ho && tx0 + px < Wo;
+            bool over = false;
+#pragma unroll
+            for (int hf = 0; hf < 32 / EPX; ++hf) {
+                __builtin_amdgcn_wave_barrier();
+                if (EPX == 32 || (px >> 4) == hf) {
+                    const int pl = px & (EPX - 1);
+#pragma unroll
+                    for (int mb = 0; mb < 2; ++mb)
+#pragma unroll
+                        for (int g = 0; g < 4; ++g) {
+                            const int ch = 32 * mb + 8 * g + 4 * half;
+                            if (MODE == 0) {
+                                w2 hi, lo;
+                                float y4[4];
+#pragma unroll
+                                for (int q = 0; q < 4; ++q) {
+                                    const int r = 4 * g + q;
+                                    const float t = fmaf(acc[nb][mb][r] + accx[nb][mb][r], inv_scale * act_scale,
+                                                         bias[ch + q] * act_scale);
+                                    over |= !(t <= 65504.f);
+                                    y4[q] = __builtin_amdgcn_fmed3f(t, 0.f, 65504.f);
+                                }
+                                split4_scaled(y4, hi, lo);
+                                char *p = epi + pl * EPITCH + (ch >> 4) * 64 + (ch & 15) * 2;
+                                *reinterpret_cast<w2 *>(p) = hi;
+                                *reinterpret_cast<w2 *>(p + 32) = lo;
+                            } else {
+                                w4 o;
+                                o.x = __float_as_uint(y[mb][4 * g + 0] * nrm);
+                                o.y = __float_as_uint(y[mb][4 * g + 1] * nrm);
+                                o.z = __float_as_uint(y[mb][4 * g + 2] * nrm);
+                                o.w = __float_as_uint(y[mb][4 * g + 3] * nrm);
+                                *reinterpret_cast<w4 *>(epi + pl * EPITCH + ch * 4) = o;
+                            }
+                        }
+                }
+                __builtin_amdgcn_wave_barrier();
+#pragma unroll
+                for (int it = 0; it < EPX / 4; ++it) {
+                    const int i = it * 64 + lane, pl = i >> 4, part = i & 15, p = hf * EPX + pl;
+                    const w4 o = *reinterpret_cast<const w4 *>(epi + pl * EPITCH + part * 16);
+                    const bool ok = row < Ho && tx0 + p < Wo;
+                    buffer_store_b128<0>(o, rs_out, ok ? p * REC + part * 16 : 0x7ffffff0, so);
+                }
+            }
+            __builtin_amdgcn_wave_barrier();
+            sat |= over && stored;
+        }
+        if (MODE == 0 && sat_flag && __builtin_amdgcn_ballot_w64(sat) != 0 && lane == 0)
+            atomicOr(sat_flag, 1);
+#endif
+        if (vn >= total) break;
+        v = vn;
+        n = nn;
+        ty0 = nty0;
+        tx0 = ntx0;
+        pb ^= 1;
+    }
+    if (FIRST && sat_flag && __builtin_amdgcn_ballot_w64(sat1 != 0) != 0 && lane == 0) atomicOr(sat_flag, 1);
+}
+
+
+template <int MODE, bool FIRST, typename... L1>
+static int launch_conv3x3_split(const char *who, const void *in, const void *packed_weights, const float *bias,
+                                void *out, int N, int Hi, int Wi, float weight_scale, float act_scale,
+                                int *saturation_flag, hipStream_t s, L1... l1)
+{
+    using namespace cs;
+    constexpr int lds_bytes = FIRST ? LDS_BYTES_FIRST : LDS_BYTES;
+    const int Ho = Hi - 2, Wo = Wi - 2;
+    const int tiles_x = cdiv(Wo, TW), tiles_y = cdiv(Ho, TH);
+    const long total = (long)tiles_x * tiles_y * N;
+    MCCNN_REQUIRE(total <= 0x7fffffffL, MCCNN_E_UNSUPPORTED, "%s: too many tiles", who);
+    const int cus = device_cus8();
+    const long slots = (long)cus * (lds_bytes <= 80 * 1024 ? 2 : 1);
+    const int grid = (int)(total < slots ? total : slots);
+    const float inv = 1.f / (weight_scale * act_scale);
+    static const hipError_t attr = hipFuncSetAttribute(reinterpret_cast<const void *>(conv3x3_split_kernel<MODE, FIRST, L1...>),
+                                                       hipFuncAttributeMaxDynamicSharedMemorySize, lds_bytes);
+    MCCNN_REQUIRE(attr == hipSuccess, MCCNN_E_UNSUPPORTED, "%s: %d bytes of LDS refused", who, lds_bytes);
+    hipLaunchKernelGGL((conv3x3_split_kernel<MODE, FIRST, L1...>), dim3(grid), dim3(256), lds_bytes, s,
+                       reinterpret_cast<const char *>(in), reinterpret_cast<const char *>(packed_weights), bias,
+                       reinterpret_cast<char *>(out), N, Hi, Wi, inv, act_scale, tiles_x, tiles_y, (int)total,
+                       saturation_flag, l1...);
+    return check_launch(who);
+}
+
+}
diff --git a/mc-cnn-python_amd/csrc/conv_mfma.hip b/mc-cnn-python_amd/csrc/conv_mfma.hip
--- a/mc-cnn-python_amd/csrc/conv_mfma.hip
+++ b/mc-cnn-python_amd/csrc/conv_mfma.hip
@@ -1,63 +1,6 @@
-#include "common.h"
+#include "conv_mfma.h"
 
 namespace mccnn {
-
-typedef _Float16 h8 __attribute__((ext_vector_type(8)));
-typedef _Float16 h4 __attribute__((ext_vector_type(4)));
-typedef float f16x __attribute__((ext_vector_type(16)));
-typedef uint32_t w4 __attribute__((ext_vector_type(4)));
-typedef uint32_t w2 __attribute__((ext_vector_type(2)));
-
-#ifndef CONV_STAGE_TAP
-#define CONV_STAGE_TAP 0
-#endif
-#ifndef CONV_NBW
-#define CONV_NBW 4
-#endif
-namespace cs {
-constexpr int NBW = CONV_NBW;
-constexpr int TH = 4 * NBW, TW = 32;
-constexpr int IH = TH + 2, IW = TW + 2;
-constexpr int NPIX = IH * IW;
-constexpr int SLOT = 80;
-constexpr int QBUF = NPIX * SLOT;
-constexpr int NITEM = NPIX * 4;
-constexpr int NST = (NITEM + 255) / 256;
-constexpr int EPITCH = 272;
-constexpr int EPX = NBW >= 4 ? 32 : 16;
-constexpr int EPI = EPX * EPITCH;
-constexpr int LDS_BYTES = 2 * QBUF + 4 * EPI;
-constexpr int REC = 256;
-constexpr int WFRAG = 1024;
-constexpr int WLAYER = 36 * 4 * WFRAG;
-}
-
-__device__ __forceinline__ void split4(const float y[4], float scale, w2 &hi, w2 &lo)
-{
-    h4 a, b;
-#pragma unroll
-    for (int j = 0; j < 4; ++j) {
-        const float v = fminf(fmaxf(y[j] * scale, -65504.f), 65504.f);
-        const _Float16 h = (_Float16)v;
-        a[j] = h;
-        b[j] = (_Float16)(v - (float)h);
-    }
-    hi = __builtin_bit_cast(w2, a);
-    lo = __builtin_bit_cast(w2, b);
-}
-
-__device__ __forceinline__ void split4_scaled(const float v[4], w2 &hi, w2 &lo)
-{
-    h4 a, b;
-#pragma unroll
-    for (int j = 0; j < 4; ++j) {
-        const _Float16 h = (_Float16)v[j];
-        a[j] = h;
-        b[j] = (_Float16)(v[j] - (float)h);
-    }
-    hi = __builtin_bit_cast(w2, a);
-    lo = __builtin_bit_cast(w2, b);
-}
 
 __global__ __launch_bounds__(256) void conv3x3_split_pack_kernel(const float *__restrict__ w, float scale,
                                                                  _Float16 *__restrict__ packed)
@@ -107,12 +50,10 @@
 #pragma unroll
             for (int j = 0; j < 4; ++j) {
                 const int c = 16 * q + 4 * g + j;
-                float acc = 0.f;
+                float wk[9];
 #pragma unroll
-                for (int k = 0; k < 9; ++k) acc += w[c * 9 + k] * v[k];
-                acc += bias[c];
-                y[j] = fmaxf(acc, 0.f);
-                sat |= !(acc * act_scale <= 65504.f);
+                for (int k = 0; k < 9; ++k) wk[k] = w[c * 9 + k];
+                y[j] = conv1_map(v, wk, bias[c], act_scale, sat);
             }
             split4(y, act_scale, hi[g], lo[g]);
         }
@@ -123,260 +64,6 @@
         p[3] = w4{lo[2].x, lo[2].y, lo[3].x, lo[3].y};
     }
     if (sat_flag && sat) atomicOr(sat_flag, 1);
-}
-
-__device__ __forceinline__ void pin_loads()
-{
-    asm volatile("" ::: "memory");
-    __builtin_amdgcn_sched_barrier(0x78f);
-}
-
-template <int MODE>
-__global__ __launch_bounds__(256) void conv3x3_split_kernel(const char *__restrict__ in, const char *__restrict__ wpk,
-                                                            const float *__restrict__ bias, char *__restrict__ out,
-                                                            int N, int Hi, int Wi, float inv_scale, float act_scale,
-                                                            int tiles_x, int tiles_y, int total,
-                                                            int *__restrict__ sat_flag)
-{
-    using namespace cs;
-    extern __shared__ __attribute__((aligned(16))) char lds[];
-    const int tid = threadIdx.x, lane = tid & 63;
-    const int wave = __builtin_amdgcn_readfirstlane(tid >> 6);
-    const int Ho = Hi - 2, Wo = Wi - 2;
-    const size_t in_bytes = (size_t)N * Hi * Wi * REC, out_bytes = (size_t)N * Ho * Wo * REC;
-    const __amdgpu_buffer_rsrc_t rs_in = __builtin_amdgcn_make_buffer_rsrc(
-        const_cast<char *>(in), 0, (int)in_bytes, 0x00020000);
-    const __amdgpu_buffer_rsrc_t rs_w =
-        __builtin_amdgcn_make_buffer_rsrc(const_cast<char *>(wpk), 0, WLAYER, 0x00020000);
-    const __amdgpu_buffer_rsrc_t rs_out = __builtin_amdgcn_make_buffer_rsrc(
-        out, 0, (int)out_bytes, 0x00020000);
-
-    int goff[NST], loff[NST];
-#pragma unroll
-    for (int r = 0; r < NST; ++r) {
-        const int i = r * 256 + tid, p = min(i >> 2, NPIX - 1), part = i & 3;
-        const int py = p / IW, px = p - py * IW;
-        goff[r] = (py * Wi + px) * REC + part * 16;
-        loff[r] = p * SLOT + part * 16;
-    }
-    const bool last_piece = (NST - 1) * 256 + tid < NITEM;
-
-    auto xcd_order = [](int b, int n) {
-        const int q = n >> 3, r = n & 7, x = b & 7;
-        return (x < r ? x * (q + 1) : r * (q + 1) + (x - r) * q) + (b >> 3);
-    };
-    auto tile_base = [&](int v, int &n, int &ty0, int &tx0) {
-        const int t = xcd_order(v, total);
-        const int tx = t % tiles_x, r = t / tiles_x;
-        const int ty = r % tiles_y;
-        n = r / tiles_y;
-        ty0 = ty * TH;
-        tx0 = tx * TW;
-    };
-
-    w4 st[NST];
-    auto fetch = [&](int n, int ty0, int tx0, int q) {
-        const int so = ((n * Hi + ty0) * Wi + tx0) * REC + q * 64;
-#ifdef CONV_ABL_NOSTAGE
-        if (so == 0x7fffffff)
-#endif
-#pragma unroll
-        for (int r = 0; r < NST; ++r) st[r] = __builtin_amdgcn_raw_buffer_load_b128(rs_in, goff[r], so, 0);
-    };
-    auto commit = [&](int buf) {
-        char *b = lds + buf * QBUF;
-#pragma unroll
-        for (int r = 0; r < NST; ++r)
-            if (r < NST - 1 || last_piece) *reinterpret_cast<w4 *>(b + loff[r]) = st[r];
-    };
-
-    int v = blockIdx.x;
-    if (v >= total) return;
-    int n, ty0, tx0;
-    tile_base(v, n, ty0, tx0);
-    fetch(n, ty0, tx0, 0);
-    commit(0);
-    __syncthreads();
-
-    constexpr int NSLOT = MODE == 0 ? 3 : 4;
-    w4 af[NSLOT][4];
-    auto fetch_a = [&](int slot, int ks) {
-#pragma unroll
-        for (int f = 0; f < 4; ++f)
-            af[slot][f] = __builtin_amdgcn_raw_buffer_load_b128(rs_w, lane * 16, (ks * 4 + f) * WFRAG, 0);
-    };
-#pragma unroll
-    for (int i = 0; i < NSLOT - 1; ++i) fetch_a(i, i);
-
-    const int bfrag = (wave * NBW * IW + (lane & 31)) * SLOT + 16 * (lane >> 5);
-    char *const epi = lds + 2 * QBUF + wave * EPI;
-
-    while (true) {
-        f16x acc[NBW][2], accx[NBW][2];
-#pragma unroll
-        for (int nb = 0; nb < NBW; ++nb)
-#pragma unroll
-            for (int mb = 0; mb < 2; ++mb)
-#pragma unroll
-                for (int i = 0; i < 16; ++i) acc[nb][mb][i] = accx[nb][mb][i] = 0.f;
-        const int vn = v + gridDim.x;
-        int nn = 0, nty0 = 0, ntx0 = 0;
-        if (vn < total) tile_base(vn, nn, nty0, ntx0);
-        if (vn >= total) {
-            nn = n;
-            nty0 = ty0;
-            ntx0 = tx0;
-        }
-#pragma unroll
-        for (int q = 0; q < 4; ++q) {
-            auto stage_next = [&]() {
-                if (q < 3)
-                    fetch(n, ty0, tx0, q + 1);
-                else
-                    fetch(nn, nty0, ntx0, 0);
-                pin_loads();
-            };
-            if (CONV_STAGE_TAP < 0) stage_next();
-            const char *bq = lds + (q & 1) * QBUF + bfrag;
-            char *const other = lds + ((q + 1) & 1) * QBUF;
-            w4 bf[2][2];
-            auto read_b = [&](int slot, int step) {
-                const int tap = step / NBW, nb = step % NBW;
-                const int dy = tap / 3, dx = tap - dy * 3;
-                const char *pb = bq + ((nb + dy) * IW + dx) * SLOT;
-                bf[slot][0] = *reinterpret_cast<const w4 *>(pb);
-                bf[slot][1] = *reinterpret_cast<const w4 *>(pb + 32);
-            };
-            read_b(0, 0);
-#pragma unroll
-            for (int tap = 0; tap < 9; ++tap) {
-                const int ks = q * 9 + tap;
-                fetch_a((ks + NSLOT - 1) % NSLOT, (ks + NSLOT - 1) % 36);
-                pin_loads();
-                if (tap == CONV_STAGE_TAP) stage_next();
-                const int slot = ks % NSLOT;
-                const h8 a_hi0 = __builtin_bit_cast(h8, af[slot][0]), a_hi1 = __builtin_bit_cast(h8, af[slot][1]);
-                const h8 a_lo0 = __builtin_bit_cast(h8, af[slot][2]), a_lo1 = __builtin_bit_cast(h8, af[slot][3]);
-#pragma unroll
-                for (int nb = 0; nb < NBW; ++nb) {
-                    const int step = tap * NBW + nb;
-                    if (step + 1 < 9 * NBW) read_b((step + 1) & 1, step + 1);
-                    __builtin_amdgcn_sched_barrier(0);
-                    const h8 b_hi = __builtin_bit_cast(h8, bf[step & 1][0]);
-                    const h8 b_lo = __builtin_bit_cast(h8, bf[step & 1][1]);
-                    accx[nb][0] = __builtin_amdgcn_mfma_f32_32x32x16_f16(a_lo0, b_hi, accx[nb][0], 0, 0, 0);
-                    accx[nb][1] = __builtin_amdgcn_mfma_f32_32x32x16_f16(a_lo1, b_hi, accx[nb][1], 0, 0, 0);
-                    accx[nb][0] = __builtin_amdgcn_mfma_f32_32x32x16_f16(a_hi0, b_lo, accx[nb][0], 0, 0, 0);
-                    accx[nb][1] = __builtin_amdgcn_mfma_f32_32x32x16_f16(a_hi1, b_lo, accx[nb][1], 0, 0, 0);
-                    acc[nb][0] = __builtin_amdgcn_mfma_f32_32x32x16_f16(a_hi0, b_hi, acc[nb][0], 0, 0, 0);
-                    acc[nb][1] = __builtin_amdgcn_mfma_f32_32x32x16_f16(a_hi1, b_hi, acc[nb][1], 0, 0, 0);
-                }
-                if (tap >= 9 - (NST + 1) / 2) {
-#pragma unroll
-                    for (int j = 0; j < 2; ++j) {
-                        const int r = 2 * (tap - (9 - (NST + 1) / 2)) + j;
-                        if (r < NST && (r < NST - 1 || last_piece)) *reinterpret_cast<w4 *>(other + loff[r]) = st[r];
-                    }
-                }
-            }
-            __syncthreads();
-        }
-
-        const int px = lane & 31, half = lane >> 5;
-        bool sat = false;
-#ifdef CONV_ABL_NOEPI
-        {
-            float t = 0.f;
-#pragma unroll
-            for (int nb = 0; nb < NBW; ++nb)
-#pragma unroll
-                for (int mb = 0; mb < 2; ++mb)
-#pragma unroll
-                    for (int r = 0; r < 16; ++r) t += acc[nb][mb][r] + accx[nb][mb][r];
-            if (t == 123.456f) __builtin_amdgcn_raw_buffer_store_b32(__float_as_uint(t), rs_out, lane * 4, 0, 0);
-        }
-#else
-#pragma unroll
-        for (int nb = 0; nb < NBW; ++nb) {
-            float y[2][16];
-            float ss = 0.f;
-#pragma unroll
-            for (int mb = 0; mb < 2; ++mb)
-#pragma unroll
-                for (int r = 0; r < 16; ++r) {
-                    const int ch = 32 * mb + (r & 3) + 8 * (r >> 2) + 4 * half;
-                    if (MODE == 0) {
-                    } else {
-                        const float t = fmaf(acc[nb][mb][r] + accx[nb][mb][r], inv_scale, bias[ch]);
-                        y[mb][r] = t;
-                        ss = fmaf(t, t, ss);
-                    }
-                }
-            float nrm = 1.f;
-            if (MODE == 1) {
-                ss += __shfl_xor(ss, 32);
-                nrm = 1.f / sqrtf(fmaxf(ss, 1e-12f));
-            }
-            const int row = ty0 + wave * NBW + nb;
-            const int so = ((n * Ho + min(row, Ho - 1)) * Wo + tx0) * REC;
-            const bool stored = row < Ho && tx0 + px < Wo;
-            bool over = false;
-#pragma unroll
-            for (int hf = 0; hf < 32 / EPX; ++hf) {
-                __builtin_amdgcn_wave_barrier();
-                if (EPX == 32 || (px >> 4) == hf) {
-                    const int pl = px & (EPX - 1);
-#pragma unroll
-                    for (int mb = 0; mb < 2; ++mb)
-#pragma unroll
-                        for (int g = 0; g < 4; ++g) {
-                            const int ch = 32 * mb + 8 * g + 4 * half;
-                            if (MODE == 0) {
-                                w2 hi, lo;
-                                float y4[4];
-#pragma unroll
-                                for (int q = 0; q < 4; ++q) {
-                                    const int r = 4 * g + q;
-                                    const float t = fmaf(acc[nb][mb][r] + accx[nb][mb][r], inv_scale * act_scale,
-                                                         bias[ch + q] * act_scale);
-                                    over |= !(t <= 65504.f);
-                                    y4[q] = __builtin_amdgcn_fmed3f(t, 0.f, 65504.f);
-                                }
-                                split4_scaled(y4, hi, lo);
-                                char *p = epi + pl * EPITCH + (ch >> 4) * 64 + (ch & 15) * 2;
-                                *reinterpret_cast<w2 *>(p) = hi;
-                                *reinterpret_cast<w2 *>(p + 32) = lo;
-                            } else {
-                                w4 o;
-                                o.x = __float_as_uint(y[mb][4 * g + 0] * nrm);
-                                o.y = __float_as_uint(y[mb][4 * g + 1] * nrm);
-                                o.z = __float_as_uint(y[mb][4 * g + 2] * nrm);
-                                o.w = __float_as_uint(y[mb][4 * g + 3] * nrm);
-                                *reinterpret_cast<w4 *>(epi + pl * EPITCH + ch * 4) = o;
-                            }
-                        }
-                }
-                __builtin_amdgcn_wave_barrier();
-#pragma unroll
-                for (int it = 0; it < EPX / 4; ++it) {
-                    const int i = it * 64 + lane, pl = i >> 4, part = i & 15, p = hf * EPX + pl;
-                    const w4 o = *reinterpret_cast<const w4 *>(epi + pl * EPITCH + part * 16);
-                    const bool ok = row < Ho && tx0 + p < Wo;
-                    buffer_store_b128<0>(o, rs_out, ok ? p * REC + part * 16 : 0x7ffffff0, so);
-                }
-            }
-            __builtin_amdgcn_wave_barrier();
-            sat |= over && stored;
-        }
-        if (MODE == 0 && sat_flag && __builtin_amdgcn_ballot_w64(sat) != 0 && lane == 0)
-            atomicOr(sat_flag, 1);
-#endif
-        if (vn >= total) break;
-        v = vn;
-        n = nn;
-        ty0 = nty0;
-        tx0 = ntx0;
-    }
 }
 
 }
@@ -414,36 +101,15 @@
 {
     using namespace mccnn;
     using namespace cs;
+    const char *who = "mccnn_conv3x3_split";
     MCCNN_REQUIRE(in && packed_weights && bias && out, MCCNN_E_INVALID, "mccnn_conv3x3_split: null pointer");
     MCCNN_REQUIRE(N > 0 && Hi > 2 && Wi > 2, MCCNN_E_INVALID, "mccnn_conv3x3_split: input %dx%d too small", Wi, Hi);
     MCCNN_REQUIRE(weight_scale > 0.f && act_scale > 0.f, MCCNN_E_INVALID, "mccnn_conv3x3_split: scales must be positive");
     MCCNN_REQUIRE((size_t)N * Hi * Wi * REC <= 0x7ffffff0u, MCCNN_E_UNSUPPORTED,
                   "mccnn_conv3x3_split: %d x %dx%d records exceed 32-bit buffer offsets", N, Wi, Hi);
-    const int Ho = Hi - 2, Wo = Wi - 2;
-    const int tiles_x = cdiv(Wo, TW), tiles_y = cdiv(Ho, TH);
-    const long total = (long)tiles_x * tiles_y * N;
-    MCCNN_REQUIRE(total <= 0x7fffffffL, MCCNN_E_UNSUPPORTED, "mccnn_conv3x3_split: too many tiles");
-    const int cus = device_cus8();
-    const long slots = (long)cus * (LDS_BYTES <= 80 * 1024 ? 2 : 1);
-    const int grid = (int)(total < slots ? total : slots);
-    const float inv = 1.f / (weight_scale * act_scale);
     hipStream_t s = (hipStream_t)stream;
-    if (last) {
-        static const hipError_t attr = hipFuncSetAttribute(reinterpret_cast<const void *>(conv3x3_split_kernel<1>),
-                                                           hipFuncAttributeMaxDynamicSharedMemorySize, LDS_BYTES);
-        MCCNN_REQUIRE(attr == hipSuccess, MCCNN_E_UNSUPPORTED, "mccnn_conv3x3_split: %d bytes of LDS refused", LDS_BYTES);
-        hipLaunchKernelGGL(conv3x3_split_kernel<1>, dim3(grid), dim3(256), LDS_BYTES, s,
-                           reinterpret_cast<const char *>(in), reinterpret_cast<const char *>(packed_weights), bias,
-                           reinterpret_cast<char *>(out), N, Hi, Wi, inv, act_scale, tiles_x, tiles_y, (int)total,
-                           saturation_flag);
-    } else {
-        static const hipError_t attr = hipFuncSetAttribute(reinterpret_cast<const void *>(conv3x3_split_kernel<0>),
-                                                           hipFuncAttributeMaxDynamicSharedMemorySize, LDS_BYTES);
-        MCCNN_REQUIRE(attr == hipSuccess, MCCNN_E_UNSUPPORTED, "mccnn_conv3x3_split: %d bytes of LDS refused", LDS_BYTES);
-        hipLaunchKernelGGL(conv3x3_split_kernel<0>, dim3(grid), dim3(256), LDS_BYTES, s,
-                           reinterpret_cast<const char *>(in), reinterpret_cast<const char *>(packed_weights), bias,
-                           reinterpret_cast<char *>(out), N, Hi, Wi, inv, act_scale, tiles_x, tiles_y, (int)total,
-                           saturation_flag);
-    }
-    return check_launch("mccnn_conv3x3_split");
+    return last ? launch_conv3x3_split<1, false>(who, in, packed_weights, bias, out, N, Hi, Wi, weight_scale,
+                                                 act_scale, saturation_flag, s)
+                : launch_conv3x3_split<0, false>(who, in, packed_weights, bias, out, N, Hi, Wi, weight_scale,
+                                                 act_scale, saturation_flag, s);
 }
diff --git a/mc-cnn-python_amd/src/_hipabi.py b/mc-cnn-python_amd/src/_hipabi.py
--- a/mc-cnn-python_amd/src/_hipabi.py
+++ b/mc-cnn-python_amd/src/_hipabi.py
@@ -102,6 +102,7 @@
     "mccnn_conv3x3_split_pack": (_i, [_vp, _f, _vp, _vp]),
     "mccnn_conv1_split": (_i, [_vp, _vp, _vp, _vp, _i, _i, _i, _i, _f, _vp, _vp]),
     "mccnn_conv3x3_split": (_i, [_vp, _vp, _vp, _vp, _i, _i, _i, _f, _f, _i, _vp, _vp]),
+    "mccnn_conv12_split": (_i, [_vp, _vp, _vp, _vp, _vp, _vp, _vp, _i, _i, _i, _f, _f, _i, _vp, _vp]),
     "mccnn_l2norm_chw_to_hwc": (_i, [_vp, _vp, _vp, _i, _i, _i, _vp]),
     "mccnn_ingest_scratch_bytes": (_sz, [_i, _i]),
     "mccnn_ingest_u8": (_i, [_vp, _i, _i, _i, _vp, _vp, _sz, _vp]),
diff --git a/mc-cnn-python_amd/src/model.py b/mc-cnn-python_amd/src/model.py
--- a/mc-cnn-python_amd/src/model.py
+++ b/mc-cnn-python_amd/src/model.py
@@ -184,14 +184,16 @@
             warnings.warn("split-operand features: a %dx%d view exceeds the kernels' 32-bit record offsets; using the "
                           "float32 library convolutions in bands of %d rows instead" % (W, H, rows))
             return self.features_pair_hwc(left_hw, right_hw, tile_rows=rows)
-        batches = [torch.stack((left_hw, right_hw)).contiguous()] if route == "pair" else \
-            [left_hw[None].contiguous(), right_hw[None].contiguous()]
+        left_hw, right_hw = left_hw.contiguous(), right_hw.contiguous()
+        batches = [(left_hw, right_hw)] if route == "pair" else [(left_hw, None), (right_hw, None)]
         outs = []
         nl = self.num_conv_layers
-        for views in batches:
-            x = stereo_device.conv1_split(views, self.weights[0].detach().contiguous(), self.biases[0].detach(), pad,
-                                          sat_flag=flag)
-            for k in range(1, nl):
+        w1, b1 = self.weights[0].detach().contiguous(), self.biases[0].detach()
+        for a, b in batches:
+            pk, ws = packed[0]
+            x = stereo_device.conv12_split(a, b, w1, b1, pk, ws, self.biases[1].detach(), pad, last=(nl == 2),
+                                           sat_flag=flag)
+            for k in range(2, nl):
                 pk, ws = packed[k - 1]
                 x = stereo_device.conv3x3_split(x, pk, ws, self.biases[k].detach(), last=(k == nl - 1), sat_flag=flag)
             outs += [x[i] for i in range(x.shape[0])]
diff --git a/mc-cnn-python_amd/src/stereo_device.py b/mc-cnn-python_amd/src/stereo_device.py
--- a/mc-cnn-python_amd/src/stereo_device.py
+++ b/mc-cnn-python_amd/src/stereo_device.py
@@ -130,6 +130,25 @@
                                              float(weight_scale), float(act_scale), 1 if last else 0,
                                              hip.ptr(sat_flag) if sat_flag is not None else None, hip.stream()),
               "mccnn_conv3x3_split")
+    return out
+
+
+def conv12_split(left, right, weight1, bias1, packed, weight_scale, bias, pad, last=False, act_scale=SPLIT_ACT_SCALE,
+                 sat_flag=None):
+    H, W = left.shape
+    assert tuple(weight1.shape) == (64, 1, 3, 3) and weight1.is_contiguous() and weight1.dtype == torch.float32
+    assert left.is_contiguous() and left.dtype == torch.float32
+    assert right is None or (right.shape == left.shape and right.is_contiguous() and right.dtype == torch.float32
+                             and right.device == left.device)
+    N = 1 if right is None else 2
+    Ho, Wo = H + 2 * pad - 4, W + 2 * pad - 4
+    out = torch.empty((N, Ho, Wo, 64), dtype=torch.float32, device=left.device) if last else \
+        torch.empty((N, Ho, Wo, 256), dtype=torch.uint8, device=left.device)
+    hip.check(hip.load().mccnn_conv12_split(hip.ptr(left), hip.ptr(right) if right is not None else None,
+                                            hip.ptr(weight1), hip.ptr(bias1), hip.ptr(packed), hip.ptr(bias),
+                                            hip.ptr(out), H, W, int(pad), float(weight_scale), float(act_scale),
+                                            1 if last else 0, hip.ptr(sat_flag) if sat_flag is not None else None,
+                                            hip.stream()), "mccnn_conv12_split")
     return out
 
 
```

New measurement: 11290 Mdisparities/s (median of 6 runs). Within noise of the previous version (+0.2%).
